# multimodallearning/DG-TTA

Hardware: AMD Instinct MI355X
Metric: TTA-epochs/sec per GPU on 128^3 patch; Dice delta vs reference (higher is better)
Workload: dtype fp16

## Files before the change

dg_tta_amd/_lib.py:

```python
import ctypes as C
import os
from pathlib import Path

LIB_PATH = Path(__file__).resolve().parent / "libdgtta_hip.so"

_c_float_p = C.POINTER(C.c_float)
P, I, I64, U64, F, SZ = C.c_void_p, C.c_int, C.c_int64, C.c_uint64, C.c_float, C.c_size_t

SIGNATURES = {
    "dgtta_version": (I, []),
    "dgtta_last_error": (C.c_char_p, []),
    "dgtta_reload_env": (I, []),
    "dgtta_mind3d_ws_bytes": (SZ, [I, I, I, I]),
    "dgtta_mind3d_fwd": (I, [P, P, F, I, C.POINTER(F), I, P, I, I, I, P, SZ, I, I, I, I, P]),
    "dgtta_mind3d_noise_fill": (I, [P, U64, U64, I, I, I, I, I, P]),
    "dgtta_mind3d_fwd_seeded": (I, [P, U64, U64, I, F, I, C.POINTER(F), I, P, I, I, I, P, SZ, I, I, I, I, P]),
    "dgtta_gin_ws_bytes": (SZ, [I, I, I, I]),
    "dgtta_gin_chain_fwd": (I, [P, P, C.POINTER(I), C.POINTER(P), C.POINTER(P), P, P, SZ, I, I, I, I, P]),
    "dgtta_affine_warp3d_fwd": (I, [P, P, P, I, I, I, I, I, I, I, I, I, I, I, I, I, I, P, P]),
    "dgtta_affine_warp3d_bwd": (I, [P, P, P, I, I, I, I, I, I, I, I, I, I, I, I, I, P]),
    "dgtta_rf_field_ws_bytes": (SZ, [I, I, I, I]),
    "dgtta_rf_field_fwd": (I, [P, P, P, SZ, I, I, I, I, I, I, I, I, P]),
    "dgtta_diffeo_fields_ws_bytes": (SZ, [I, I, I, I]),
    "dgtta_diffeo_fields": (I, [P, F, P, P, P, SZ, I, I, I, I, I, P]),
    "dgtta_dense_warp3d_fwd": (I, [P, P, P, I, I, I, I, I, I, I, I, I, P]),
    "dgtta_dense_warp3d_bwd": (I, [P, P, P, I, I, I, I, I, I, I, I, I, P]),
    "dgtta_softdice_ws_bytes": (SZ, [I, I, I64]),
    "dgtta_softdice_fwd": (I, [P, P, P, P, P, SZ, I, I, I64, I, I, I, P]),
    "dgtta_softdice_bwd": (I, [P, P, P, P, P, F, P, I, I, I64, I, I, P]),
    "dgtta_softdice_bwd_t": (I, [P, P, P, P, P, F, P, I, I, I64, I, I, I, P]),
    "dgtta_softdice_probs_fwd": (I, [P, P, P, P, SZ, I, I, I64, I64, I64, I64, P]),
    "dgtta_softdice_probs_bwd": (I, [P, P, P, P, P, P, I, I, I64, I64, I64, I64, P]),
    "dgtta_dice_ce_ws_bytes": (SZ, [I, I, I64]),
    "dgtta_dice_ce_fwd": (I, [P, I, P, P, P, P, SZ, I, I, I64, F, I, P]),
    "dgtta_dice_ce_bwd": (I, [P, I, P, P, F, P, P, I, I, I, I64, P]),
    "dgtta_dice_ce_ds_ws_bytes": (SZ, [I, I, I, I, I]),
    "dgtta_dice_ce_ds_fwd": (I, [P, I, P, P, P, P, SZ, I, I, I, I, I, I, I, I, F, I, P]),
    "dgtta_dice_ce_ds_bwd": (I, [P, I, P, P, F, P, P, I, I, I, I, I, I, I, I, I, P]),
    "dgtta_adamw_step": (I, [C.POINTER(P), C.POINTER(P), C.POINTER(P), C.POINTER(P), C.POINTER(I64), I, F, F, F, F, F,
                             I, F, P, P]),
    "dgtta_grads_nonfinite": (I, [C.POINTER(P), C.POINTER(I64), I, P, P]),
    "dgtta_grad_sumsq_ws_bytes": (SZ, [I64, I]),
    "dgtta_grad_sumsq": (I, [C.POINTER(P), C.POINTER(I64), I, P, P, SZ, P]),
    "dgtta_sgd_step": (I, [C.POINTER(P), C.POINTER(P), C.POINTER(P), C.POINTER(I64), I, F, F, F, I, I, F, P, F, P, P]),
    "dgtta_conv3d_packed_bytes": (SZ, [I, I, I]),
    "dgtta_conv3d_pack_weights": (I, [P, P, I, I, I, I, I, P]),
    "dgtta_conv3d_stats_bytes": (SZ, [I, I, I, I, I]),
    "dgtta_conv3d_k3_fwd": (I, [P, I, P, P, P, I, P, I, I, I, I, I, I, I, I, I, I, I, P]),
    "dgtta_conv3d_k3_dgrad": (I, [P, I, P, P, I, I, I, I, I, I, I, I, I, I, I, I, I, P]),
    "dgtta_conv3d_wgrad_ws_bytes": (SZ, [I, I, I, I, I, I]),
    "dgtta_conv3d_wgrad_split_ws_bytes": (SZ, [I, I, I, I, I, I, I]),
    "dgtta_conv3d_k3_wgrad": (I, [P, I, P, I, P, P, P, SZ, I, I, I, I, I, I, I, I, I, I, P]),
    "dgtta_conv3d_k3_blocked_supported": (I, [I, I, I, I, I, I, I]),
    "dgtta_conv3d_k3_fwd_blocked": (I, [P, I64, P, P, P, I, P, I, I, I, I, I, I, I, I, I, P]),
    "dgtta_conv3d_k3_wgrad_blocked": (I, [P, I64, P, I, P, P, P, SZ, I, I, I, I, I, I, I, I, P]),
    "dgtta_instnorm_ws_bytes": (SZ, [I, I, I64]),
    "dgtta_instnorm_lrelu_fwd": (I, [P, I, P, P, P, P, P, I, P, SZ, I, I, I64, F, F, I, P]),
    "dgtta_instnorm_lrelu_bwd": (I, [P, I, P, I, P, P, P, P, I, P, P, P, SZ, I, I, I64, F, I, I, P]),
    "dgtta_conv3d_k3_dgrad_gstats": (I, [P, I, P, P, I, I, I, I, I, I, I, I, I, P, I, P, P, P, F, P, SZ, C.POINTER(I), I, I, P]),
    "dgtta_instnorm_lrelu_bwd_gstats": (I, [P, I, P, I, P, P, P, P, I, P, P, P, P, SZ, I, I, I64, F, I, I, P]),
    "dgtta_convT3d_fwd_ws_bytes": (SZ, [I, I, I]),
    "dgtta_convT3d_k2s2_fwd": (I, [P, I, P, P, P, I, P, SZ, I, I, I, I, I, I, I, I, P]),
    "dgtta_convT3d_bwd_ws_bytes": (SZ, [I, I, I, I, I, I]),
    "dgtta_convT3d_bwd_split_ws_bytes": (SZ, [I, I, I, I, I, I]),
    "dgtta_convT3d_k2s2_bwd": (I, [P, I, P, I, P, P, I, P, P, P, SZ, I, I, I, I, I, I, I, I, I, P]),
    "dgtta_conv3d_kpacked_bytes": (SZ, [I, I, I, I]),
    "dgtta_conv3d_kpack_weights": (I, [P, P, I, I, I, I, I, I, I, I, P]),
    "dgtta_conv3d_fwd": (I, [P, I, P, P, P, I, P, I, I, I, I, I, I, I, I, I, I, I, I, I, P]),
    "dgtta_conv3d_dgrad": (I, [P, I, P, P, I, I, I, I, I, I, I, I, I, I, I, I, I, I, I, P]),
    "dgtta_conv3d_kwgrad_ws_bytes": (SZ, [I, I, I, I, I, I, I, I, I, I]),
    "dgtta_conv3d_wgrad": (I, [P, I, P, I, P, P, P, SZ, I, I, I, I, I, I, I, I, I, I, I, I, P]),
    "dgtta_convT3d_s_fwd_ws_bytes": (SZ, [I, I, I, I, I, I]),
    "dgtta_convT3d_s_fwd": (I, [P, I, P, P, P, I, P, SZ, I, I, I, I, I, I, I, I, I, I, P]),
    "dgtta_convT3d_s_bwd_ws_bytes": (SZ, [I, I, I, I, I, I, I, I, I]),
    "dgtta_convT3d_s_bwd": (I, [P, I, P, I, P, P, I, P, P, P, SZ, I, I, I, I, I, I, I, I, I, I, I, P]),
    "dgtta_seghead_fwd": (I, [P, I, P, P, P, I, P, I, I, I, I, I64, I, P]),
    "dgtta_seghead_bwd_ws_bytes": (SZ, [I, I, I, I64]),
    "dgtta_seghead_bwd": (I, [P, I, P, I, P, P, I, P, I, P, P, P, SZ, I, I, I64, I, I, P]),
    "dgtta_seghead_bwd_acc": (I, [P, I, P, I, P, P, I, P, I, P, P, P, SZ, I, I, I64, I, I, I, P]),
    "dgtta_seghead_warp_supported": (I, [P, I, I, I, I, I, I, I]),
    "dgtta_seghead_warp_bwd_ws_bytes": (SZ, [I, I, I, I, I, I]),
    "dgtta_seghead_warp_fwd": (I, [P, P, P, P, I, P, P, I, I, I, I, I, I, I, P]),
    "dgtta_seghead_warp_bwd": (I, [P, P, P, P, P, P, I, P, P, P, P, SZ, I, I, I, I, I, I, I, I, P]),
    "dgtta_seghead_warp_bwd_g16": (I, [P, P, P, P, P, P, I, P, P, P, P, SZ, I, I, I, I, I, I, I, I, P]),
    "dgtta_ncdhw_to_ndhwc": (I, [P, P, I, I, I64, I, I, P]),
    "dgtta_ndhwc_to_ncdhw": (I, [P, P, I, I, I64, I, I, P]),
    "dgtta_argmax_dice": (I, [P, I, I, P, P, P, I, I64, P]),
    "dgtta_resample_axis_ws_bytes": (SZ, [I64, I, I64, I]),
    "dgtta_resample_axis": (I, [P, P, P, SZ, I64, I, I, I64, I, P]),
    "dgtta_window_accumulate": (I, [P, P, P, P, I, I, I, I, I, I, I, I, I, I, P]),
    "dgtta_seghead_window_accumulate": (I, [P, P, P, P, P, P, I, I, I, I, I, I, I, I, I, I, I, I, P]),
    "dgtta_logits_chunk_f64": (I, [P, P, P, I, I, I, I, I, I, I, I, I, I, I, I, P]),
    "dgtta_window_accumulate_t": (I, [P, P, P, P, I, I, I, I, I, I, I, I, I, I, I, P]),
    "dgtta_seghead_window_accumulate_t": (I, [P, P, P, P, P, P, I, I, I, I, I, I, I, I, I, I, I, I, I, P]),
    "dgtta_argmax_rows": (I, [P, I, I, I64, P, P]),
    "dgtta_feature_window_accumulate": (I, [P, P, P, P, I, I, I, I, I, I, I, I, I, I, I, P]),
    "dgtta_feature_window_accumulate_norm": (I, [P, P, P, P, F, P, P, P, I, I, I, I, I, I, I, I, I, I, I, P]),
    "dgtta_feature_window_accumulate_multi": (I, [P, P, P, I, P, P, F, P, P, P, I, I, I, I, I, I, I, I, I, I, I, I, P]),
    "dgtta_feature_head_argmax": (I, [P, I64, P, P, P, I, I, I, I64, P, P]),
    "dgtta_feature_logits_chunk_f64": (I, [P, I64, P, P, P, P, I, I, I, I, I, I, I, I, I, I, I, I, I, I, P]),
    "dgtta_logits_chunk_f64_t": (I, [P, P, P, I, I, I, I, I, I, I, I, I, I, I, I, I, P]),
    "dgtta_argmax_merge_f64": (I, [P, I64, I, I, P, P, I, P]),
    "dgtta_feature_head_softmax": (I, [P, I64, P, P, P, I, I, I, I64, C.POINTER(I), I, I, P, P, P, P, P]),
    "dgtta_softmax_merge_f64": (I, [P, I64, I, I, C.c_double, P, P, P, C.POINTER(I), I, P, I, P]),
    "dgtta_softmax_finalize_f64": (I, [P, P, P, P, I64, I, I, P, P, P, P]),
    "dgtta_label_bboxes": (I, [P, P, I, I, I, I, P, P]),
    "dgtta_label_surface": (I, [P, I, I, I, I64, I, I, I, I, I, I, P, P]),
    "dgtta_edt_ws_bytes": (SZ, [I, I, I]),
    "dgtta_edt_sq": (I, [P, P, P, SZ, I, I, I, F, F, F, P]),
    "dgtta_cc_ws_bytes": (SZ, [I, I, I]),
    "dgtta_cc_label": (I, [P, P, I, I, I, I, I, P, P, SZ, P]),
    "dgtta_cc_sizes": (I, [P, I64, P, P]),
    "dgtta_cc_filter": (I, [P, P, I, P, P, I64, I, I, I64, P, P, P, SZ, P]),
    "dgtta_holes_ws_bytes": (SZ, [I, I, I]),
    "dgtta_holes_fill": (I, [P, I, I, I, I, P, P, P, P, SZ, P]),
    "dgtta_holes_member": (I, [P, I, I, I, P, I, I, I, I, I, I, I, P, P]),
    "dgtta_holes_apply": (I, [P, I, I, I, P, P, I, I, I, I, I, I, I64, I64, P, P]),
    "dgtta_nonzero_mask": (I, [P, I, I64, P, P]),
    "dgtta_bspline3_prefilter": (I, [P, P, I, I, I, P]),
    "dgtta_patch_sample_aug": (I, [P, I, I, I, I, I, P, P, P]),
    "dgtta_intensity_stats_ws_bytes": (SZ, [I, I64]),
    "dgtta_intensity_stats": (I, [P, I, I64, C.POINTER(I), I, P, P, SZ, P]),
    "dgtta_intensity_map": (I, [P, P, I, I64, P, I, P, P, P]),
    "dgtta_gauss_blur3": (I, [P, P, P, I, I, I, I, P, I, P]),
}



class PatchItem(C.Structure):
    _fields_ = [("image", P), ("label", P), ("D", I), ("H", I), ("W", I), ("map", F * 12)]


PATCH_MAX_ITEMS = 16


class IntensityItem(C.Structure):
    _fields_ = [("item", I), ("mode", I), ("negate", I), ("noise_b", I), ("a", F), ("s", F), ("seed_lo", C.c_uint32),
                ("seed_hi", C.c_uint32), ("off_lo", C.c_uint32), ("off_hi", C.c_uint32)]


class BlurItem(C.Structure):
    _fields_ = [("item", I), ("radius", I), ("taps", F * 9)]


INTENSITY_MAX_ITEMS = 16
IMAP_LINEAR, IMAP_CONTRAST, IMAP_GAMMA, IMAP_RESTORE = 0, 1, 2, 3

_lib = None
_load_error = None


class DgttaError(RuntimeError):
    pass


def load():
    global _lib, _load_error
    if _lib is not None:
        return _lib
    if _load_error is not None:
        raise DgttaError(_load_error)
    path = os.environ.get("DGTTA_LIB", str(LIB_PATH))
    import torch
    try:
        lib = C.CDLL(path)
    except OSError as e:
        _load_error = (f"libdgtta_hip.so could not be loaded from {path} ({e}). Build it with "
                       f"`python dg_tta_amd/build.py`; dg_tta_amd has no CPU fallback.")
        raise DgttaError(_load_error) from e
    for name, (res, args) in SIGNATURES.items():
        fn = getattr(lib, name)
        fn.restype = res
        fn.argtypes = args
    _lib = lib
    return lib


def check(rc, what):
    if rc != 0:
        msg = load().dgtta_last_error().decode(errors="replace")
        raise DgttaError(f"{what} failed (code {rc}): {msg}")


def ptr(t):
    return None if t is None else t.data_ptr()


def stream_of(device=None):
    import torch
    return torch.cuda.current_stream(device).cuda_stream


def require_cuda(*tensors):
    for t in tensors:
        if t is not None and not t.is_cuda:
            raise DgttaError("dg_tta_amd ops run on the MI355X only: got a CPU tensor (there is no CPU fallback)")
```

dg_tta_amd/csrc/common.h:

```cpp
#pragma once
#include <hip/hip_runtime.h>
#include <hip/hip_bf16.h>
#include <hip/hip_fp16.h>
#include <stdint.h>
#include <stdio.h>
#include <stdarg.h>

#include "../../include/dgtta.h"

#define WAVE 64

#include <atomic>

void dgtta_set_error(const char *fmt, ...);

struct DgttaSwitches {
  int conv_rows, conv_s2, dgrad_s2_allcls, wgrad_tr, wgrad_tr8, wgrad_s2_onepass, convt_wgrad_onepass;
  int convt_gemm, rows_order, in_nt, wgrad_upw, wgrad_xcd, in_gstats, softdice16, conv_ring, wgrad_ring, ha_mfma, wgrad_f32_split, feature_head_mfma, headwarp_mfma, wgrad_flat, wgrad_reduce_taps;
};
const DgttaSwitches &dgtta_switches();

struct DynLdsOnce {
  std::atomic<unsigned long long> mask{0};
};
static inline hipError_t ensure_dyn_lds(DynLdsOnce &o, const void *fn, int bytes) {
  int dev = 0;
  (void)hipGetDevice(&dev);
  const unsigned long long bit = 1ull << (dev & 63);
  if (o.mask.load(std::memory_order_acquire) & bit) return hipSuccess;
  const hipError_t e = hipFuncSetAttribute(fn, hipFuncAttributeMaxDynamicSharedMemorySize, bytes);
  if (e == hipSuccess) o.mask.fetch_or(bit, std::memory_order_release);
  return e;
}

struct RowsGstCtx {
  const void *y;
  long long ldy;
  const float *mr, *gamma, *beta;
  float slope;
  double *out;
  int produced;
};

#define DG_REQUIRE(cond, code, ...)      \
  do {                                   \
    if (!(cond)) {                       \
      dgtta_set_error(__VA_ARGS__);      \
      return (code);                     \
    }                                    \
  } while (0)

#define DG_CHECK_LAUNCH(name)                                                     \
  do {                                                                            \
    hipError_t e__ = hipGetLastError();                                           \
    if (e__ != hipSuccess) {                                                      \
      dgtta_set_error("%s: launch failed: %s", name, hipGetErrorString(e__));     \
      return DGTTA_ERR_LAUNCH;                                                    \
    }                                                                             \
  } while (0)

__host__ __device__ static inline int64_t cdiv64(int64_t a, int64_t b) { return (a + b - 1) / b; }
__host__ __device__ static inline int cdiv(int a, int b) { return (a + b - 1) / b; }
static inline size_t align_up(size_t x, size_t a) { return (x + a - 1) / a * a; }
static inline int grid_for(int64_t total) {
  const int64_t b = (total + 255) / 256;
  return (int)(b < 8192 ? b : 8192);
}

typedef unsigned short bf16_t;

__device__ __forceinline__ float bf16_to_f32(bf16_t h) { return __uint_as_float(((unsigned)h) << 16); }
__device__ __forceinline__ bf16_t f32_to_bf16(float f) {
  __hip_bfloat16 b = __float2bfloat16(f);
  return *reinterpret_cast<bf16_t *>(&b);
}

struct f16_t {
  unsigned short v;
};
__device__ __forceinline__ float f16_to_f32(unsigned short h) {
  return __half2float(__ushort_as_half(h));
}
__device__ __forceinline__ unsigned short f32_to_f16(float f) { return __half_as_ushort(__float2half_rn(f)); }

template <typename T>
__device__ __forceinline__ unsigned short f32_to_16(float f);
template <>
__device__ __forceinline__ unsigned short f32_to_16<bf16_t>(float f) { return f32_to_bf16(f); }
template <>
__device__ __forceinline__ unsigned short f32_to_16<f16_t>(float f) { return f32_to_f16(f); }
template <typename T>
__device__ __forceinline__ float from16(unsigned short h);
template <>
__device__ __forceinline__ float from16<bf16_t>(unsigned short h) { return bf16_to_f32(h); }
template <>
__device__ __forceinline__ float from16<f16_t>(unsigned short h) { return f16_to_f32(h); }
template <typename T>
__device__ __forceinline__ unsigned pack2_16(float lo, float hi) {
  return (unsigned)f32_to_16<T>(lo) | ((unsigned)f32_to_16<T>(hi) << 16);
}
template <typename T>
__device__ __forceinline__ void unpack2_16(unsigned w, float &lo, float &hi);
template <>
__device__ __forceinline__ void unpack2_16<bf16_t>(unsigned w, float &lo, float &hi) {
  lo = __uint_as_float(w << 16);
  hi = __uint_as_float(w & 0xffff0000u);
}
template <>
__device__ __forceinline__ void unpack2_16<f16_t>(unsigned w, float &lo, float &hi) {
  lo = f16_to_f32((unsigned short)(w & 0xffffu));
  hi = f16_to_f32((unsigned short)(w >> 16));
}

template <typename T>
__device__ __forceinline__ float ld_f(const T *p);
template <>
__device__ __forceinline__ float ld_f<float>(const float *p) { return *p; }
template <>
__device__ __forceinline__ float ld_f<bf16_t>(const bf16_t *p) { return bf16_to_f32(*p); }
template <>
__device__ __forceinline__ float ld_f<f16_t>(const f16_t *p) { return f16_to_f32(p->v); }

template <typename T>
__device__ __forceinline__ void st_f(T *p, float v);
template <>
__device__ __forceinline__ void st_f<float>(float *p, float v) { *p = v; }
template <>
__device__ __forceinline__ void st_f<bf16_t>(bf16_t *p, float v) { *p = f32_to_bf16(v); }
template <>
__device__ __forceinline__ void st_f<f16_t>(f16_t *p, float v) { p->v = f32_to_f16(v); }

template <typename T>
__device__ __forceinline__ void unpack16(const uint4 &v, float *f);
template <>
__device__ __forceinline__ void unpack16<float>(const uint4 &v, float *f) {
  f[0] = __uint_as_float(v.x);
  f[1] = __uint_as_float(v.y);
  f[2] = __uint_as_float(v.z);
  f[3] = __uint_as_float(v.w);
}
template <>
__device__ __forceinline__ void unpack16<bf16_t>(const uint4 &v, float *f) {
  const unsigned w[4] = {v.x, v.y, v.z, v.w};
#pragma unroll
  for (int i = 0; i < 4; ++i) {
    f[2 * i] = __uint_as_float(w[i] << 16);
    f[2 * i + 1] = __uint_as_float(w[i] & 0xffff0000u);
  }
}
template <>
__device__ __forceinline__ void unpack16<f16_t>(const uint4 &v, float *f) {
  const unsigned w[4] = {v.x, v.y, v.z, v.w};
#pragma unroll
  for (int i = 0; i < 4; ++i) unpack2_16<f16_t>(w[i], f[2 * i], f[2 * i + 1]);
}

template <typename T>
__device__ __forceinline__ uint4 pack16(const float *f);
template <>
__device__ __forceinline__ uint4 pack16<float>(const float *f) {
  return make_uint4(__float_as_uint(f[0]), __float_as_uint(f[1]), __float_as_uint(f[2]), __float_as_uint(f[3]));
}
template <>
__device__ __forceinline__ uint4 pack16<bf16_t>(const float *f) {
  unsigned w[4];
#pragma unroll
  for (int i = 0; i < 4; ++i) w[i] = (unsigned)f32_to_bf16(f[2 * i]) | ((unsigned)f32_to_bf16(f[2 * i + 1]) << 16);
  return make_uint4(w[0], w[1], w[2], w[3]);
}
template <>
__device__ __forceinline__ uint4 pack16<f16_t>(const float *f) {
  return make_uint4(pack2_16<f16_t>(f[0], f[1]), pack2_16<f16_t>(f[2], f[3]), pack2_16<f16_t>(f[4], f[5]),
                    pack2_16<f16_t>(f[6], f[7]));
}

__device__ __forceinline__ float wave_sum(float v) {
#pragma unroll
  for (int o = 32; o > 0; o >>= 1) v += __shfl_xor(v, o, 64);
  return v;
}
__device__ __forceinline__ double wave_sum_d(double v) {
#pragma unroll
  for (int o = 32; o > 0; o >>= 1) v += __shfl_xor(v, o, 64);
  return v;
}
__device__ __forceinline__ float wave_min(float v) {
#pragma unroll
  for (int o = 32; o > 0; o >>= 1) v = fminf(v, __shfl_xor(v, o, 64));
  return v;
}

__device__ __forceinline__ float block_sum(float v, float *red) {
  v = wave_sum(v);
  const int lane = threadIdx.x & 63, w = threadIdx.x >> 6, nw = (blockDim.x + 63) >> 6;
  __syncthreads();
  if (lane == 0) red[w] = v;
  __syncthreads();
  float r = 0.f;
  for (int i = 0; i < nw; ++i) r += red[i];
  return r;
}

__device__ __forceinline__ float lrelu(float a, float slope) { return a > 0.f ? a : a * slope; }
```

dg_tta_amd/csrc/conv_dispatch.hip:

```cpp
#include "conv_api.h"

static int wgrad_splits(int64_t nvox) {
  int64_t s = cdiv64(nvox, 4096);
  return (int)(s < 64 ? (s > 0 ? s : 1) : 64);
}

static const void *wb_of(const void *wpack, int CinP, int CoutP, int dtype) {
  return (const char *)wpack + (size_t)27 * CinP * CoutP * esize(dtype);
}

static const void *img_of(const void *wpack, int CinP, int CoutP, int dtype) {
  return (const char *)wpack + (size_t)2 * 27 * CinP * CoutP * esize(dtype);
}
static const void *imgB_of(const void *wpack, int CinP, int CoutP, int dtype) {
  return (const char *)img_of(wpack, CinP, CoutP, dtype) + conv_imgB_offset_bytes(CinP, CoutP, dtype);
}

extern "C" size_t dgtta_conv3d_packed_bytes(int CinP, int CoutP, int dtype) {
  if (CinP <= 0 || CoutP <= 0) return 0;
  return (size_t)2 * 27 * CinP * CoutP * esize(dtype) + conv_image_bytes(CinP, CoutP, dtype);
}

extern "C" int dgtta_conv3d_pack_weights(const float *w_t, void *wpack, int Cin, int Cout, int CinP, int CoutP,
                                         int dtype, void *stream) {
  DG_REQUIRE(w_t && wpack, DGTTA_ERR_BADARG, "pack_weights: null pointer");
  void *wf = wpack;
  void *wb = const_cast<void *>(wb_of(wpack, CinP, CoutP, dtype));
  DG_REQUIRE(Cin > 0 && Cout > 0 && CinP >= Cin && CoutP >= Cout, DGTTA_ERR_BADARG, "pack_weights: bad channel counts");
  const int rc = conv3_pack_weights_ref(w_t, wf, wb, Cin, Cout, CinP, CoutP, dtype, (hipStream_t)stream);
  if (rc != DGTTA_OK) return rc;
  if (CinP % conv_granule(dtype) == 0 && CoutP % conv_granule(dtype) == 0)
    return conv_pack_images(w_t, const_cast<void *>(img_of(wpack, CinP, CoutP, dtype)), 27, Cin, Cout, CinP, CoutP, dtype,
                            (hipStream_t)stream);
  return DGTTA_OK;
}

extern "C" size_t dgtta_conv3d_stats_bytes(int B, int Cout, int Do, int Ho, int Wo) {
  if (B <= 0 || Cout <= 0 || Do <= 0 || Ho <= 0 || Wo <= 0) return 0;
  int64_t nb = conv3_mfma_max_tiles(Do, Ho, Wo);
  const int64_t rb = reduce_blocks((int64_t)Do * Ho * Wo, B);
  if (rb > nb) nb = rb;
  return 256 + (size_t)B * nb * Cout * 2 * sizeof(double);
}

static int k3_fwd(const void *x, int ldx, long long x_block_stride, const void *wpack, const float *bias, void *y, int ldy,
                  void *stats, int B, int Cin, int Cout, int CinP, int CoutP, int Di, int Hi, int Wi, int stride, int dtype, int impl,
                  void *stream) {
  DG_REQUIRE(x && wpack && y, DGTTA_ERR_BADARG, "conv3d_k3_fwd: null pointer");
  const void *wf = wpack;
  DG_REQUIRE(B > 0 && Cin > 0 && Cout > 0 && CinP >= Cin && CoutP >= Cout && Di > 0 && Hi > 0 && Wi > 0,
             DGTTA_ERR_BADARG, "conv3d_k3_fwd: bad dims");
  DG_REQUIRE(stride == 1 || stride == 2, DGTTA_ERR_UNSUPPORTED, "conv3d_k3_fwd: stride %d", stride);
  DG_REQUIRE((x_block_stride ? 2 * ldx : ldx) >= Cin && ldy >= Cout, DGTTA_ERR_BADARG, "conv3d_k3_fwd: ld < C");
  hipStream_t st = (hipStream_t)stream;
  if (impl != 1) {
    int rc = conv3_fwd_mfma(x, ldx, img_of(wpack, CinP, CoutP, dtype), 0, bias, y, ldy, B, Cin, Cout, CinP, CoutP, Di, Hi,
                            Wi, stride, dtype, st, (double *)stats, nullptr, x_block_stride, false);
    if (rc != DGTTA_ERR_UNSUPPORTED) return rc;
    DG_REQUIRE(x_block_stride == 0, DGTTA_ERR_UNSUPPORTED,
               "conv3d_k3_fwd_blocked: only the D-ring kernel reads x as 32-channel planes (ask dgtta_conv3d_k3_blocked_supported)");
    DG_REQUIRE(impl == 0, DGTTA_ERR_UNSUPPORTED, "conv3d_k3_fwd: shape not covered by the MFMA kernel");
  }
  int rc = conv3_fwd_ref(x, ldx, wf, bias, y, ldy, B, Cin, Cout, CinP, CoutP, Di, Hi, Wi, stride, dtype, st);
  if (rc != DGTTA_OK) return rc;
  if (stats) {
    const int64_t V = (int64_t)out_dim(Di, stride) * out_dim(Hi, stride) * out_dim(Wi, stride);
    return conv_stats_ref(y, ldy, stats, B, Cout, V, dtype, st);
  }
  return DGTTA_OK;
}

extern "C" int dgtta_conv3d_k3_fwd(const void *x, int ldx, const void *wpack, const float *bias, void *y, int ldy,
                                   void *stats, int B, int Cin, int Cout, int CinP, int CoutP, int Di, int Hi, int Wi,
                                   int stride, int dtype, int impl, void *stream) {
  return k3_fwd(x, ldx, 0, wpack, bias, y, ldy, stats, B, Cin, Cout, CinP, CoutP, Di, Hi, Wi, stride, dtype, impl, stream);
}

extern "C" int dgtta_conv3d_k3_blocked_supported(int B, int Cin, int Cout, int D, int H, int W, int dtype) {
  if (B <= 0 || Cin != 64 || Cout <= 0 || Cout % 32 || D <= 0 || H <= 0 || W <= 0) return 0;
  if (dtype != DGTTA_BF16 && dtype != DGTTA_F16) return 0;
  const int rc = conv3_fwd_mfma((const void *)16, 32, (const void *)16, 0, nullptr, (void *)16, Cout, B, Cin, Cout, Cin, Cout, D, H, W, 1,
                                dtype, nullptr, nullptr, nullptr, (long long)B * D * H * W * 32, true);
  return rc == DGTTA_OK && conv3_wgrad_blocked_ok(B, Cin, Cout, D, H, W, dtype);
}

extern "C" int dgtta_conv3d_k3_fwd_blocked(const void *x, long long x_block_stride, const void *wpack, const float *bias, void *y,
                                           int ldy, void *stats, int B, int Cin, int Cout, int CinP, int CoutP, int Di, int Hi,
                                           int Wi, int dtype, void *stream) {
  DG_REQUIRE(x_block_stride > 0 && x_block_stride % 8 == 0, DGTTA_ERR_BADARG, "conv3d_k3_fwd_blocked: block stride must be a positive multiple of 8 elements");
  return k3_fwd(x, 32, x_block_stride, wpack, bias, y, ldy, stats, B, Cin, Cout, CinP, CoutP, Di, Hi, Wi, 1, dtype, 0, stream);
}

static int k3_dgrad(const void *dy, int lddy, const void *wpack, void *dx, int lddx, int B, int Cin, int Cout, int CinP, int CoutP,
                    int Di, int Hi, int Wi, int stride, int accumulate, int dtype, int impl, void *stream, RowsGstCtx *gst) {
  DG_REQUIRE(dy && wpack && dx, DGTTA_ERR_BADARG, "conv3d_k3_dgrad: null pointer");
  const void *wb = wb_of(wpack, CinP, CoutP, dtype);
  DG_REQUIRE(B > 0 && Cin > 0 && Cout > 0 && CinP >= Cin && CoutP >= Cout && Di > 0 && Hi > 0 && Wi > 0,
             DGTTA_ERR_BADARG, "conv3d_k3_dgrad: bad dims");
  DG_REQUIRE(stride == 1 || stride == 2, DGTTA_ERR_UNSUPPORTED, "conv3d_k3_dgrad: stride %d", stride);
  DG_REQUIRE(lddx >= Cin && lddy >= Cout, DGTTA_ERR_BADARG, "conv3d_k3_dgrad: ld < C");
  hipStream_t st = (hipStream_t)stream;
  if (impl != 1 && stride == 1 && !accumulate) {
    int rc = conv3_fwd_mfma(dy, lddy, imgB_of(wpack, CinP, CoutP, dtype), 1, nullptr, dx, lddx, B, Cout, Cin, CoutP, CinP, Di,
                            Hi, Wi, 1, dtype, st, nullptr, gst, 0, false);
    if (rc != DGTTA_ERR_UNSUPPORTED) return rc;
    DG_REQUIRE(impl == 0, DGTTA_ERR_UNSUPPORTED, "conv3d_k3_dgrad: shape not covered by the MFMA kernel");
  }
  if (impl != 1 && stride == 2 && !((Di | Hi | Wi) & 1)) {
    int rc = conv3_dgrad_s2_mfma(dy, lddy, imgB_of(wpack, CinP, CoutP, dtype), dx, lddx, B, Cin, Cout, CinP, CoutP, Di, Hi, Wi,
                                 accumulate, dtype, st);
    if (rc != DGTTA_ERR_UNSUPPORTED) return rc;
    DG_REQUIRE(impl == 0, DGTTA_ERR_UNSUPPORTED, "conv3d_k3_dgrad: shape not covered by the MFMA kernel");
  }
  return conv3_dgrad_ref(dy, lddy, wb, dx, lddx, B, Cin, Cout, CinP, CoutP, Di, Hi, Wi, stride, accumulate, dtype, st);
}

extern "C" int dgtta_conv3d_k3_dgrad(const void *dy, int lddy, const void *wpack, void *dx, int lddx, int B, int Cin,
                                     int Cout, int CinP, int CoutP, int Di, int Hi, int Wi, int stride, int accumulate,
                                     int dtype, int impl, void *stream) {
  return k3_dgrad(dy, lddy, wpack, dx, lddx, B, Cin, Cout, CinP, CoutP, Di, Hi, Wi, stride, accumulate, dtype, impl, stream, nullptr);
}

extern "C" int dgtta_conv3d_k3_dgrad_gstats(const void *dy, int lddy, const void *wpack, void *dx, int lddx, int B, int Cin,
                                            int Cout, int CinP, int CoutP, int Di, int Hi, int Wi, const void *y_prev,
                                            int ldy_prev, const float *mean_rstd_prev, const float *gamma_prev,
                                            const float *beta_prev, float slope, void *gstats, size_t gstats_bytes,
                                            int *h_produced, int dtype, int impl, void *stream) {
  DG_REQUIRE(y_prev && mean_rstd_prev && gamma_prev && beta_prev && gstats && h_produced, DGTTA_ERR_BADARG,
             "conv3d_k3_dgrad_gstats: null pointer");
  DG_REQUIRE(ldy_prev >= Cin, DGTTA_ERR_BADARG, "conv3d_k3_dgrad_gstats: ldy_prev < Cin");
  DG_REQUIRE(B > 0 && Cin > 0 && Di > 0 && Hi > 0 && Wi > 0 && gstats_bytes >= dgtta_conv3d_stats_bytes(B, Cin, Di, Hi, Wi),
             DGTTA_ERR_WORKSPACE, "conv3d_k3_dgrad_gstats: statistics buffer too small");
  RowsGstCtx ctx{y_prev, ldy_prev, mean_rstd_prev, gamma_prev, beta_prev, slope, (double *)gstats, 0};
  const bool fuse = dtype != DGTTA_F32 && impl != 1 && dgtta_switches().in_gstats != '0';
  const int rc = k3_dgrad(dy, lddy, wpack, dx, lddx, B, Cin, Cout, CinP, CoutP, Di, Hi, Wi, 1, 0, dtype, impl, stream,
                          fuse ? &ctx : nullptr);
  *h_produced = rc == DGTTA_OK ? ctx.produced : 0;
  return rc;
}

static size_t wgrad_bias_bytes(int B, int Cout, int Do, int Ho, int Wo) {
  return align_up((size_t)B * reduce_blocks((int64_t)Do * Ho * Wo, B) * Cout * 2 * sizeof(double), 256);
}

extern "C" size_t dgtta_conv3d_wgrad_ws_bytes(int B, int Cin, int Cout, int Do, int Ho, int Wo) {
  if (B <= 0 || Cin <= 0 || Cout <= 0 || Do <= 0 || Ho <= 0 || Wo <= 0) return 0;
  const int64_t nvox = (int64_t)B * Do * Ho * Wo;
  size_t a = align_up((size_t)wgrad_splits(nvox) * Cout * Cin * 27 * sizeof(float), 256);
  size_t c = align_up(conv3_wgrad_mfma_ws_bytes(B, Cin, Cout, Do, Ho, Wo), 256);
  return wgrad_bias_bytes(B, Cout, Do, Ho, Wo) + (a > c ? a : c);
}

extern "C" size_t dgtta_conv3d_wgrad_split_ws_bytes(int B, int Cin, int Cout, int Do, int Ho, int Wo, int stride) {
  if (B <= 0 || Cin <= 0 || Cout <= 0 || Do <= 0 || Ho <= 0 || Wo <= 0 || (stride != 1 && stride != 2)) return 0;
  const size_t base = dgtta_conv3d_wgrad_ws_bytes(B, Cin, Cout, Do, Ho, Wo);
  return base + 256 + conv3_wgrad_split_extra_bytes(B, Cin, Cout, Do, Ho, Wo, stride);
}

static int k3_wgrad(const void *x, int ldx, long long x_block_stride, const void *dy, int lddy, float *dw_t, float *db, void *ws,
                    size_t ws_bytes, int B, int Cin, int Cout, int Di, int Hi, int Wi, int stride, int accumulate, int dtype, int impl,
                    void *stream) {
  DG_REQUIRE(x && dy && dw_t && ws, DGTTA_ERR_BADARG, "conv3d_k3_wgrad: null pointer");
  DG_REQUIRE(B > 0 && Cin > 0 && Cout > 0 && Di > 0 && Hi > 0 && Wi > 0, DGTTA_ERR_BADARG, "conv3d_k3_wgrad: bad dims");
  DG_REQUIRE(stride == 1 || stride == 2, DGTTA_ERR_UNSUPPORTED, "conv3d_k3_wgrad: stride %d", stride);
  const int Do = out_dim(Di, stride), Ho = out_dim(Hi, stride), Wo = out_dim(Wi, stride);
  DG_REQUIRE(ws_bytes >= dgtta_conv3d_wgrad_ws_bytes(B, Cin, Cout, Do, Ho, Wo), DGTTA_ERR_WORKSPACE,
             "conv3d_k3_wgrad: workspace too small");
  hipStream_t st = (hipStream_t)stream;
  const int64_t nvox = (int64_t)B * Do * Ho * Wo;
  const int nsplit = wgrad_splits(nvox);
  const size_t bias_bytes = wgrad_bias_bytes(B, Cout, Do, Ho, Wo);
  void *ws2 = ws;
  float *part = (float *)((char *)ws + bias_bytes);
  bool done = false;
  if (impl != 1) {
    int rc = conv3_wgrad_mfma(x, ldx, dy, lddy, dw_t, part, ws_bytes - bias_bytes, B, Cin, Cout, Di, Hi, Wi,
                              stride, accumulate, dtype, st, x_block_stride);
    if (rc == DGTTA_OK) done = true;
    else if (rc != DGTTA_ERR_UNSUPPORTED) return rc;
    else DG_REQUIRE(impl == 0 && x_block_stride == 0, DGTTA_ERR_UNSUPPORTED,
                    "conv3d_k3_wgrad: shape not covered by the MFMA kernel (x as 32-channel planes: only the ring sweep, ask dgtta_conv3d_k3_blocked_supported)");
  }
  if (!done) {
    const int rc = conv3_wgrad_ref(x, ldx, dy, lddy, part, nsplit, dw_t, B, Cin, Cout, Di, Hi, Wi, stride, accumulate, dtype, st);
    if (rc != DGTTA_OK) return rc;
  }
  if (db) return conv_bias_grad(dy, lddy, db, ws2, B, Cout, (int64_t)Do * Ho * Wo, accumulate, dtype, st);
  return DGTTA_OK;
}

extern "C" int dgtta_conv3d_k3_wgrad(const void *x, int ldx, const void *dy, int lddy, float *dw_t, float *db, void *ws,
                                     size_t ws_bytes, int B, int Cin, int Cout, int Di, int Hi, int Wi, int stride,
                                     int accumulate, int dtype, int impl, void *stream) {
  return k3_wgrad(x, ldx, 0, dy, lddy, dw_t, db, ws, ws_bytes, B, Cin, Cout, Di, Hi, Wi, stride, accumulate, dtype, impl, stream);
}

extern "C" int dgtta_conv3d_k3_wgrad_blocked(const void *x, long long x_block_stride, const void *dy, int lddy, float *dw_t, float *db,
                                             void *ws, size_t ws_bytes, int B, int Cin, int Cout, int Di, int Hi, int Wi,
                                             int accumulate, int dtype, void *stream) {
  DG_REQUIRE(x_block_stride > 0 && x_block_stride % 8 == 0, DGTTA_ERR_BADARG, "conv3d_k3_wgrad_blocked: block stride must be a positive multiple of 8 elements");
  return k3_wgrad(x, 32, x_block_stride, dy, lddy, dw_t, db, ws, ws_bytes, B, Cin, Cout, Di, Hi, Wi, 1, accumulate, dtype, 0, stream);
}

extern "C" size_t dgtta_convT3d_fwd_ws_bytes(int Cin, int Cout, int dtype) {
  if (Cin <= 0 || Cout <= 0) return 0;
  return convT_pack_region(Cin, Cout, dtype);
}

extern "C" int dgtta_convT3d_k2s2_fwd(const void *x, int ldx, const float *w_t, const float *bias, void *out, int ldo,
                                      void *ws, size_t ws_bytes, int B, int Cin, int Cout, int Di, int Hi, int Wi,
                                      int dtype, int impl, void *stream) {
  DG_REQUIRE(x && w_t && out, DGTTA_ERR_BADARG, "convT3d_k2s2_fwd: null pointer");
  DG_REQUIRE(B > 0 && Cin > 0 && Cout > 0 && Di > 0 && Hi > 0 && Wi > 0 && ldx >= Cin && ldo >= Cout, DGTTA_ERR_BADARG,
             "convT3d_k2s2_fwd: bad dims");
  hipStream_t st = (hipStream_t)stream;
  if (impl != 1 && ws && ws_bytes >= convT_pack_region(Cin, Cout, dtype)) {
    int rc = convT_fwd_mfma(x, ldx, w_t, bias, out, ldo, ws, B, Cin, Cout, Di, Hi, Wi, dtype, st);
    if (rc != DGTTA_ERR_UNSUPPORTED) return rc;
  }
  DG_REQUIRE(impl != 2, DGTTA_ERR_UNSUPPORTED, "convT3d_k2s2_fwd: shape not covered by the MFMA kernel");
  return convT_fwd_ref(x, ldx, w_t, bias, out, ldo, B, Cin, Cout, Di, Hi, Wi, dtype, st);
}

static size_t convT_bias_region(int B, int Cout, int Di, int Hi, int Wi) {
  return align_up((size_t)B * reduce_blocks((int64_t)Di * Hi * Wi * 8, B) * Cout * 2 * sizeof(double), 256);
}

extern "C" size_t dgtta_convT3d_bwd_ws_bytes(int B, int Cin, int Cout, int Di, int Hi, int Wi) {
  if (B <= 0 || Cin <= 0 || Cout <= 0 || Di <= 0 || Hi <= 0 || Wi <= 0) return 0;
  const int64_t nvox = (int64_t)B * Di * Hi * Wi;
  size_t a = align_up((size_t)wgrad_splits(nvox) * Cin * Cout * 8 * sizeof(float), 256);
  size_t c = align_up(conv3_wgrad_mfma_ws_bytes(B, Cin, Cout, Di, Hi, Wi), 256);
  return convT_bias_region(B, Cout, Di, Hi, Wi) + convT_pack_region(Cin, Cout, DGTTA_F32) + (a > c ? a : c);
}

extern "C" size_t dgtta_convT3d_bwd_split_ws_bytes(int B, int Cin, int Cout, int Di, int Hi, int Wi) {
  if (B <= 0 || Cin <= 0 || Cout <= 0 || Di <= 0 || Hi <= 0 || Wi <= 0) return 0;
  const int64_t nvox = (int64_t)B * Di * Hi * Wi;
  size_t a = align_up((size_t)wgrad_splits(nvox) * Cin * Cout * 8 * sizeof(float), 256);
  size_t c = align_up(conv3_wgrad_mfma_ws_bytes(B, Cin, Cout, Di, Hi, Wi), 256) + convT_wgrad_split_extra_bytes(B, Cin, Cout, Di, Hi, Wi);
  return convT_bias_region(B, Cout, Di, Hi, Wi) + convT_pack_region(Cin, Cout, DGTTA_F32) + (a > c ? a : c);
}

extern "C" int dgtta_convT3d_k2s2_bwd(const void *x, int ldx, const void *dout, int lddo, const float *w_t, void *dx,
                                      int lddx, float *dw_t, float *db, void *ws, size_t ws_bytes, int B, int Cin,
                                      int Cout, int Di, int Hi, int Wi, int accumulate, int dtype, int impl,
                                      void *stream) {
  DG_REQUIRE(x && dout && w_t && ws, DGTTA_ERR_BADARG, "convT3d_k2s2_bwd: null pointer");
  DG_REQUIRE(B > 0 && Cin > 0 && Cout > 0 && Di > 0 && Hi > 0 && Wi > 0 && ldx >= Cin && lddo >= Cout,
             DGTTA_ERR_BADARG, "convT3d_k2s2_bwd: bad dims");
  DG_REQUIRE(ws_bytes >= dgtta_convT3d_bwd_ws_bytes(B, Cin, Cout, Di, Hi, Wi), DGTTA_ERR_WORKSPACE,
             "convT3d_k2s2_bwd: workspace too small");
  hipStream_t st = (hipStream_t)stream;
  const int64_t nvox = (int64_t)B * Di * Hi * Wi;
  void *ws_bias = ws;
  void *ws_pack = (char *)ws + convT_bias_region(B, Cout, Di, Hi, Wi);
  void *ws_main = (char *)ws_pack + convT_pack_region(Cin, Cout, DGTTA_F32);
  const size_t main_bytes = ws_bytes - ((char *)ws_main - (char *)ws);
  int bias_units = 0;
  if (dx) {
    DG_REQUIRE(lddx >= Cin, DGTTA_ERR_BADARG, "convT3d_k2s2_bwd: lddx < Cin");
    int rc = DGTTA_ERR_UNSUPPORTED;
    if (impl != 1) rc = convT_dgrad_mfma(dout, lddo, w_t, dx, lddx, ws_pack, B, Cin, Cout, Di, Hi, Wi, dtype, st);
    if (rc == DGTTA_ERR_UNSUPPORTED) {
      DG_REQUIRE(impl != 2, DGTTA_ERR_UNSUPPORTED, "convT3d_k2s2_bwd: dgrad shape not covered by the MFMA kernel");
      rc = convT_dgrad_ref(dout, lddo, w_t, dx, lddx, B, Cin, Cout, Di, Hi, Wi, dtype, st);
      if (rc != DGTTA_OK) return rc;
    } else if (rc != DGTTA_OK) {
      return rc;
    }
  }
  if (dw_t) {
    int rc = DGTTA_ERR_UNSUPPORTED;
    if (impl != 1)
      rc = convT_wgrad_mfma(x, ldx, dout, lddo, dw_t, ws_main, main_bytes, B, Cin, Cout, Di, Hi, Wi, accumulate, dtype, st,
                            db ? (float *)ws_bias : nullptr, convT_bias_region(B, Cout, Di, Hi, Wi), &bias_units);
    if (rc == DGTTA_ERR_UNSUPPORTED) {
      DG_REQUIRE(impl != 2, DGTTA_ERR_UNSUPPORTED, "convT3d_k2s2_bwd: wgrad shape not covered by the MFMA kernel");
      rc = convT_wgrad_ref(x, ldx, dout, lddo, (float *)ws_main, wgrad_splits(nvox), dw_t, B, Cin, Cout, Di, Hi, Wi, accumulate,
                           dtype, st);
      if (rc != DGTTA_OK) return rc;
    } else if (rc != DGTTA_OK) {
      return rc;
    }
  }
  if (db && bias_units > 0) {
    DG_REQUIRE(convT_bias_finalize((const float *)ws_bias, bias_units, Cout, db, accumulate, st) == DGTTA_OK, DGTTA_ERR_LAUNCH,
               "convT3d_k2s2_bwd: bias finalize launch failed");
    return DGTTA_OK;
  }
  if (db) return conv_bias_grad(dout, lddo, db, ws_bias, B, Cout, (int64_t)Di * Hi * Wi * 8, accumulate, dtype, st);
  return DGTTA_OK;
}
```

dg_tta_amd/csrc/conv_mfma.hip:

```cpp
#include "conv_common.h"
#include <stdlib.h>
#include <type_traits>

namespace {

template <typename T, int MBW, int MBH, int MBD, int S, int NB, int KSPC, int NW = 4, bool AC = false>
__global__ __launch_bounds__(NW * 64) void conv3_mfma_kernel(const T *__restrict__ x, View xv, const T *__restrict__ w,
                                                         ConvClasses cs, const float *__restrict__ bias,
                                                         T *__restrict__ y, View yv, int Cin, int Cout, int CinP,
                                                         int CoutP, int tilesW, int tilesH, int tilesD,
                                                         double *__restrict__ stats, int ntaps_src) {
  const int cls = blockIdx.z;
  x += cs.xoff[cls];
  if (!AC) y += cs.yoff[cls];
  const Taps &taps = cs.taps[cls];
  const int accumulate = cs.acc[cls];
  const int Di = xv.D, Hi = xv.H, Wi = xv.W, Do = yv.D, Ho = yv.H, Wo = yv.W;
  typedef ConvCfg<T, MBW, MBH, MBD, S, NB, KSPC> Cfg;
  typedef typename Cfg::G G;
  constexpr int EPV = Cfg::EPV, NG = Cfg::NG, CK = Cfg::CK, NC = Cfg::NC, NV = G::NV, MPW = G::MB / NW, NT = NW * 64;
  extern __shared__ __attribute__((aligned(16))) unsigned char smem[];
  uint4 *sA = reinterpret_cast<uint4 *>(smem);
  uint4 *sB = reinterpret_cast<uint4 *>(smem + Cfg::A_BYTES);

  const int tid = threadIdx.x, lane = tid & 63, wave = tid >> 6;
  const int r = lane & 31, h = lane >> 5;

  int tlin = blockIdx.x;
  if ((gridDim.x & 7) == 0) tlin = (tlin & 7) * (int)(gridDim.x >> 3) + (tlin >> 3);
  int t = tlin;
  const int tw = t % tilesW;
  t /= tilesW;
  const int th = t % tilesH;
  t /= tilesH;
  const int td = t % tilesD;
  const int b = t / tilesD;
  const int n0 = blockIdx.y * NC;
  constexpr int SE = G::SE, NTAP = G::NTAP;
  const int od0 = td * G::TD, oh0 = th * G::TH, ow0 = tw * G::TW;
  const int id0 = od0 * SE - G::HALO, ih0 = oh0 * SE - G::HALO, iw0 = ow0 * SE - G::HALO;

  int a_off[MPW];
#pragma unroll
  for (int i = 0; i < MPW; ++i) {
    const int mb = wave * MPW + i;
    const int mbd = mb / MBH, mbh = mb % MBH;
    const int row = mbh * G::RPM + r / MBW, col = r % MBW;
    a_off[i] = ((mbd * SE) * G::IH + row * SE) * G::ROW + col;
  }

  constexpr int NACC = AC ? 8 : NB;
  f32x16_t acc[MPW][NACC];
#pragma unroll
  for (int i = 0; i < MPW; ++i)
#pragma unroll
    for (int j = 0; j < NACC; ++j)
#pragma unroll
      for (int q = 0; q < 16; ++q) acc[i][j][q] = 0.f;

  const T *xbp = x + (int64_t)b * xv.sb;
  const int cin_lim = (Cin + EPV - 1) / EPV * EPV;

  constexpr int NA = (NV * NG + NT - 1) / NT, NBL = (NTAP * NC * NG + NT - 1) / NT;
  uint4 ra[NA], rb[NBL];
  __shared__ signed char s_wt[32];
  if (tid < 27) s_wt[tid] = AC ? (signed char)tid : taps.wt[tid];
  __syncthreads();
  int wslot[NBL];
#pragma unroll
  for (int i = 0; i < NBL; ++i) {
    const int idx = tid + i * NT;
    const int n = idx % NC, g = (idx / NC) % NG, tap = (S == 0) ? 13 : (idx / (NG * NC)) % 27;
    const int wt = s_wt[tap];
    const bool ok = idx < NTAP * NC * NG && wt >= 0;
    const int off = ((((n0 + n) / 32) * (CinP / (2 * EPV)) + g / 2) * ntaps_src + wt) * 64 + (g & 1) * 32 + (n0 + n) % 32;
    wslot[i] = ok ? off : -1;
  }
  auto load_chunk = [&](int kc) {
#pragma unroll
    for (int i = 0; i < NA; ++i) {
      const int idx = tid + i * NT;
      const int g = idx % NG, v = idx / NG;
      const int wx_l = v % G::ROW, hy = (v / G::ROW) % G::IH, dz = v / (G::ROW * G::IH);
      int wx = wx_l;
      if (S == 2) wx = (wx_l >= G::IWH) ? 2 * (wx_l - G::IWH) + 1 : 2 * wx_l;
      const int gd = id0 + dz, gh = ih0 + hy, gw = iw0 + wx;
      int c = kc + g * EPV;
      long long soff = 0;
      if (S == 0 && cs.kseg > 0) {
        const int seg = c / cs.kseg;
        c -= seg * cs.kseg;
        soff = cs.segoff[seg];
      }
      const bool ok = idx < NV * NG && (S != 2 || wx < G::IW) && (unsigned)gd < (unsigned)Di &&
                      (unsigned)gh < (unsigned)Hi && (unsigned)gw < (unsigned)Wi && c < cin_lim;
      const T *p = ok ? xbp + soff + gd * xv.sd + gh * xv.sh + gw * xv.sw + c : x;
      const uint4 val = *reinterpret_cast<const uint4 *>(p);
      ra[i] = ok ? val : make_uint4(0, 0, 0, 0);
    }
    const int kterm = (kc / (2 * EPV)) * ntaps_src * 64;
#pragma unroll
    for (int i = 0; i < NBL; ++i) {
      const bool ok = wslot[i] >= 0;
      const T *p = w + (int64_t)(ok ? wslot[i] + kterm : 0) * EPV;
      const uint4 val = *reinterpret_cast<const uint4 *>(p);
      rb[i] = ok ? val : make_uint4(0, 0, 0, 0);
    }
  };
  auto store_chunk = [&]() {
#pragma unroll
    for (int i = 0; i < NA; ++i) {
      const int idx = tid + i * NT;
      if (idx < NV * NG) sA[(idx % NG) * NV + idx / NG] = ra[i];
    }
#pragma unroll
    for (int i = 0; i < NBL; ++i) {
      const int idx = tid + i * NT;
      if (idx < NTAP * NC * NG) sB[idx] = rb[i];
    }
  };

  load_chunk(0);
  for (int kc = 0; kc < CinP; kc += CK) {
    __syncthreads();
    store_chunk();
    __syncthreads();
    if (kc + CK < CinP) load_chunk(kc + CK);
    if (AC) {
#pragma unroll
      for (int ks = 0; ks < KSPC; ++ks) {
        const int g = 2 * ks + h;
#pragma unroll
        for (int sh8 = 0; sh8 < 8; ++sh8) {
          const int sd = sh8 >> 2, shh = (sh8 >> 1) & 1, sw = sh8 & 1;
          const int tap_off = ((1 + sd) * G::IH + (1 + shh)) * G::ROW + G::lds_col(1 + sw);
          uint4 af[MPW];
#pragma unroll
          for (int i = 0; i < MPW; ++i) af[i] = sA[g * NV + a_off[i] + tap_off];
#pragma unroll
          for (int od = 0; od < 2 - sd; ++od)
#pragma unroll
            for (int oh = 0; oh < 2 - shh; ++oh)
#pragma unroll
              for (int ow = 0; ow < 2 - sw; ++ow) {
                const int pd = sd ? 1 : od, ph = shh ? 1 : oh, pw = sw ? 1 : ow;
                const int td = sd ? 0 : 1 + od, th = shh ? 0 : 1 + oh, tw = sw ? 0 : 1 + ow;
                const int tap = td * 9 + th * 3 + tw, c8 = pd * 4 + ph * 2 + pw;
                const uint4 bfr = sB[(tap * NG + g) * NC + r];
#pragma unroll
                for (int i = 0; i < MPW; ++i) mfma_step<T>(af[i], bfr, acc[i][c8]);
              }
        }
      }
    } else
#pragma unroll
    for (int tap = (S == 0 ? 13 : 0); tap < (S == 0 ? 14 : 27); ++tap) {
      if (taps.wt[tap] < 0) continue;
      const int kd = tap / 9, kh = (tap / 3) % 3, kw = tap % 3;
      const int tap_off = (S == 0) ? 0 : (kd * G::IH + kh) * G::ROW + G::lds_col(kw);
      const int tb = (S == 0) ? 0 : tap;
#pragma unroll
      for (int ks = 0; ks < KSPC; ++ks) {
        const int g = 2 * ks + h;
        uint4 bf[NB];
#pragma unroll
        for (int j = 0; j < NB; ++j) bf[j] = uint4(sB[(tb * NG + g) * NC + j * 32 + r]);
#pragma unroll
        for (int i = 0; i < MPW; ++i) {
          const uint4 af = sA[g * NV + a_off[i] + tap_off];
#pragma unroll
          for (int j = 0; j < NB; ++j) mfma_step<T>(af, bf[j], acc[i][j]);
        }
      }
    }
  }

  float st1[NB], st2[NB];
#pragma unroll
  for (int j = 0; j < NB; ++j) st1[j] = st2[j] = 0.f;
  if (AC) {
    const bool vec = Cout % 8 == 0 && (reinterpret_cast<uintptr_t>(y) & 15) == 0 && yv.sw % 8 == 0 && yv.sh % 8 == 0 &&
                     yv.sd % 8 == 0 && yv.sb % 8 == 0;
    __syncthreads();
    float *slab = reinterpret_cast<float *>(smem) + wave * (32 * 36);
#pragma unroll
    for (int i = 0; i < MPW; ++i) {
      const int mb = wave * MPW + i;
      const int mbd = mb / MBH, mbh = mb % MBH;
      const int co = n0 + r;
      uint4 olds[8][2];
      if constexpr (sizeof(T) == 2) {
        if (vec && accumulate) {
#pragma unroll
          for (int c8 = 0; c8 < 8; ++c8)
#pragma unroll
            for (int t = 0; t < 2; ++t) {
              const int m = t * 16 + (lane >> 2), cq = (lane & 3) * 8;
              const int od = od0 + mbd, oh = oh0 + mbh * G::RPM + m / MBW, ow = ow0 + m % MBW;
              olds[c8][t] = make_uint4(0u, 0u, 0u, 0u);
              if (n0 + cq < Cout && od < Do && oh < Ho && ow < Wo)
                olds[c8][t] = *reinterpret_cast<const uint4 *>(y + cs.yoff[c8] + b * yv.sb + od * yv.sd + oh * yv.sh + ow * yv.sw + n0 + cq);
            }
        }
      }
#pragma unroll
      for (int c8 = 0; c8 < 8; ++c8) {
        if (!vec) {
#pragma unroll
          for (int q = 0; q < 16; ++q) {
            const int m = (q & 3) + 8 * (q >> 2) + 4 * h;
            const int od = od0 + mbd, oh = oh0 + mbh * G::RPM + m / MBW, ow = ow0 + m % MBW;
            if (co < Cout && od < Do && oh < Ho && ow < Wo) {
              T *o = y + cs.yoff[c8] + b * yv.sb + od * yv.sd + oh * yv.sh + ow * yv.sw + co;
              float v = acc[i][c8][q];
              if (accumulate) v += ld_f<T>(o);
              st_f<T>(o, v);
            }
          }
          continue;
        }
#pragma unroll
        for (int q = 0; q < 16; ++q) slab[((q & 3) + 8 * (q >> 2) + 4 * h) * 36 + r] = acc[i][c8][q];
#pragma unroll
        for (int t = 0; t < 2; ++t) {
          const int m = t * 16 + (lane >> 2), cq = (lane & 3) * 8;
          const float4 v0 = *reinterpret_cast<const float4 *>(slab + m * 36 + cq);
          const float4 v1 = *reinterpret_cast<const float4 *>(slab + m * 36 + cq + 4);
          float v[8] = {v0.x, v0.y, v0.z, v0.w, v1.x, v1.y, v1.z, v1.w};
          const int od = od0 + mbd, oh = oh0 + mbh * G::RPM + m / MBW, ow = ow0 + m % MBW;
          if (n0 + cq < Cout && od < Do && oh < Ho && ow < Wo) {
            T *o = y + cs.yoff[c8] + b * yv.sb + od * yv.sd + oh * yv.sh + ow * yv.sw + n0 + cq;
            if constexpr (sizeof(T) == 2) {
              uint4 *o4 = reinterpret_cast<uint4 *>(o);
              if (accumulate) {
                const uint4 old = olds[c8][t];
                const unsigned wv[4] = {old.x, old.y, old.z, old.w};
#pragma unroll
                for (int e = 0; e < 4; ++e) {
                  float lo, hi;
                  unpack2_16<T>(wv[e], lo, hi);
                  v[2 * e] += lo;
                  v[2 * e + 1] += hi;
                }
              }
              uint4 pk;
              pk.x = pack2_16<T>(v[0], v[1]);
              pk.y = pack2_16<T>(v[2], v[3]);
              pk.z = pack2_16<T>(v[4], v[5]);
              pk.w = pack2_16<T>(v[6], v[7]);
              *o4 = pk;
            } else {
              float4 *o4 = reinterpret_cast<float4 *>(o);
              if (accumulate) {
                const float4 a0 = o4[0], a1 = o4[1];
                v[0] += a0.x; v[1] += a0.y; v[2] += a0.z; v[3] += a0.w;
                v[4] += a1.x; v[5] += a1.y; v[6] += a1.z; v[7] += a1.w;
              }
              o4[0] = make_float4(v[0], v[1], v[2], v[3]);
              o4[1] = make_float4(v[4], v[5], v[6], v[7]);
            }
          }
        }
      }
    }
    return;
  }
#pragma unroll
  for (int i = 0; i < MPW; ++i) {
    const int mb = wave * MPW + i;
    const int mbd = mb / MBH, mbh = mb % MBH;
#pragma unroll
    for (int j = 0; j < NB; ++j) {
      const int co = n0 + j * 32 + r;
      const float bv = (bias && co < Cout) ? bias[co] : 0.f;
#pragma unroll
      for (int q = 0; q < 16; ++q) {
        const int m = (q & 3) + 8 * (q >> 2) + 4 * h;
        const int od = od0 + mbd, oh = oh0 + mbh * G::RPM + m / MBW, ow = ow0 + m % MBW;
        if (co < Cout && od < Do && oh < Ho && ow < Wo) {
          T *o = y + b * yv.sb + od * yv.sd + oh * yv.sh + ow * yv.sw + co;
          float v = acc[i][j][q] + bv;
          if (accumulate) v += ld_f<T>(o);
          st_f<T>(o, v);
          st1[j] += v;
          st2[j] += v * v;
        }
      }
    }
  }
  if (stats) {
    __syncthreads();
    float *red = reinterpret_cast<float *>(smem);
#pragma unroll
    for (int j = 0; j < NB; ++j) {
      const float a = st1[j] + __shfl_xor(st1[j], 32, 64), c = st2[j] + __shfl_xor(st2[j], 32, 64);
      if (h == 0) {
        red[(wave * NC + j * 32 + r) * 2 + 0] = a;
        red[(wave * NC + j * 32 + r) * 2 + 1] = c;
      }
    }
    __syncthreads();
    const int tiles_per_b = tilesW * tilesH * tilesD;
    if (tid < NC && n0 + tid < Cout) {
      double s = 0.0, ss = 0.0;
#pragma unroll
      for (int wv = 0; wv < NW; ++wv) {
        s += (double)red[(wv * NC + tid) * 2 + 0];
        ss += (double)red[(wv * NC + tid) * 2 + 1];
      }
      double *p = stats + 32 + (((int64_t)b * tiles_per_b + (tlin % tiles_per_b)) * Cout + n0 + tid) * 2;
      p[0] = s;
      p[1] = ss;
    }
    if (blockIdx.x == 0 && blockIdx.y == 0 && tid == 0) reinterpret_cast<long long *>(stats)[0] = tiles_per_b;
  }
}

template <typename T, int MBW, int MBH, int MBD, int S, int NB, int KSPC, int NW = 4, bool AC = false>
int launch_conv(const ConvLaunch &L, const ConvClasses &cs) {
  typedef ConvCfg<T, MBW, MBH, MBD, S, NB, KSPC> Cfg;
  typedef typename Cfg::G G;
  auto kern = conv3_mfma_kernel<T, MBW, MBH, MBD, S, NB, KSPC, NW, AC>;
  static DynLdsOnce lds_once;
  DG_REQUIRE(ensure_dyn_lds(lds_once, reinterpret_cast<const void *>(kern), (int)Cfg::LDS_BYTES) == hipSuccess,
             DGTTA_ERR_LAUNCH, "conv3_mfma: cannot raise the dynamic LDS limit to %zu", (size_t)Cfg::LDS_BYTES);
  const int tW = cdiv(L.yv.W, G::TW), tH = cdiv(L.yv.H, G::TH), tD = cdiv(L.yv.D, G::TD);
  const int64_t tiles = (int64_t)tW * tH * tD * L.B;
  DG_REQUIRE(tiles < (1ll << 31), DGTTA_ERR_UNSUPPORTED, "conv3_mfma: too many tiles");
  dim3 grid((unsigned)tiles, (unsigned)cdiv(L.CoutP, Cfg::NC), AC ? 1u : (unsigned)cs.n);
  hipLaunchKernelGGL(kern, grid, dim3(NW * 64), Cfg::LDS_BYTES, L.st, (const T *)L.x, L.xv, (const T *)L.w, cs, L.bias, (T *)L.y,
                     L.yv, L.Cin, L.Cout, L.CinP, L.CoutP, tW, tH, tD, L.stats, L.ntaps_src);
  DG_CHECK_LAUNCH(AC ? "conv3_mfma_kernel<all classes>" : "conv3_mfma_kernel");
  return DGTTA_OK;
}

template <typename T>
int dispatch_conv_classes(const ConvLaunch &L, const ConvClasses &cs, int stride) {
  const View &yv = L.yv;
  const bool ring_only = L.xkh || L.dry;
  const long long vox = (long long)yv.D * yv.H * yv.W * L.B;
  if (ring_only && stride != 1) return DGTTA_ERR_UNSUPPORTED;
  if (stride == 0) {
    if (yv.W >= 32) return launch_conv<T, 32, 4, 4, 0, 1, 1, 8>(L, cs);
    if (yv.W >= 16) return launch_conv<T, 16, 4, 4, 0, 1, 1, 8>(L, cs);
    if (vox <= 4096) return launch_conv<T, 8, 2, 2, 0, 1, 1>(L, cs);
    return launch_conv<T, 8, 2, 8, 0, 1, 1, 8>(L, cs);
  }
  if (stride == 1 && sizeof(T) == 2 && yv.W >= 32 && cs.n == 1 && cs.acc[0] == 0 && cs.kseg == 0 && cs.xoff[0] == 0 &&
      cs.yoff[0] == 0) {
    const int rows = dgtta_switches().conv_rows;
    const int is_f16 = (int)std::is_same<T, f16_t>::value;
    bool all_taps = true;
    for (int t = 0; t < 27; ++t) all_taps = all_taps && cs.taps[0].wt[t] >= 0;
    const bool vec_out = L.Cout % 8 == 0 && ((uintptr_t)L.y & 15) == 0 && yv.sw % 8 == 0 && yv.sh % 8 == 0 &&
                         yv.sd % 8 == 0 && yv.sb % 8 == 0;
    const long long njobs = (long long)cdiv(yv.W, 32) * cdiv(yv.H, 8) * cdiv(yv.D, 4) * cdiv(L.CoutP, 32) * L.B;
    if (all_taps && vec_out && ((L.Cin == 32 && L.CinP == 32) || (L.Cin == 64 && L.CinP == 64)) &&
        (njobs >= 512 || dgtta_switches().conv_ring == '1') && dgtta_switches().conv_ring != '0' && rows != '1') {
      const int rc = conv3_ring_launch(L, cs.taps[0], conv3_mfma_max_tiles(yv.D, yv.H, yv.W), is_f16);
      if (rc != DGTTA_ERR_UNSUPPORTED || ring_only) return rc;
    }
    if (ring_only) return DGTTA_ERR_UNSUPPORTED;
    if (all_taps && vec_out && (njobs >= 256 || rows == '1') && rows != '0') return conv3_rows_launch(L, cs.taps[0], is_f16);
  }
  if (ring_only) return DGTTA_ERR_UNSUPPORTED;
  if (stride == 1) {
    if (yv.W >= 32) return launch_conv<T, 32, 4, 4, 1, 1, 1, 8>(L, cs);
    const bool k2 = L.CinP % (4 * Elem<T>::EPV) == 0;
    if (yv.W >= 16) return launch_conv<T, 16, 4, 4, 1, 1, 1, 8>(L, cs);
    if (vox <= 4096 && k2) return launch_conv<T, 8, 2, 2, 1, 1, 2>(L, cs);
    if (vox <= 4096) return launch_conv<T, 8, 2, 2, 1, 1, 1>(L, cs);
    return launch_conv<T, 8, 2, 8, 1, 1, 1, 8>(L, cs);
  }
  if (stride == 2) {
    if (dgtta_switches().conv_s2 == '4') {
      if (yv.W >= 16) return launch_conv<T, 16, 2, 4, 2, 1, 1>(L, cs);
      return launch_conv<T, 8, 2, 4, 2, 1, 1>(L, cs);
    }
    if (dgtta_switches().conv_s2 != '1' && yv.W >= 32 && L.CoutP % 64 == 0) return launch_conv<T, 32, 4, 2, 2, 2, 1, 8>(L, cs);
    if (yv.W >= 32) return launch_conv<T, 32, 4, 2, 2, 1, 1, 8>(L, cs);
    if (yv.W >= 16) return launch_conv<T, 16, 2, 4, 2, 1, 1, 8>(L, cs);
    return launch_conv<T, 8, 2, 4, 2, 1, 1, 8>(L, cs);
  }
  return DGTTA_ERR_UNSUPPORTED;
}

template <typename T>
int dispatch_conv(const ConvLaunch &L, const Taps &taps, int stride, int accumulate) {
  return dispatch_conv_classes<T>(L, single_class(taps, accumulate), stride);
}

template <typename T>
int dgrad_s2_allcls(const ConvLaunch &L, const ConvClasses &cs) {
  if (L.yv.W >= 32) return launch_conv<T, 32, 4, 2, 1, 1, 1, 8, true>(L, cs);
  if (L.yv.W >= 16) return launch_conv<T, 16, 2, 4, 1, 1, 1, 8, true>(L, cs);
  return launch_conv<T, 8, 2, 4, 1, 1, 1, 8, true>(L, cs);
}

template <typename T>
__global__ void conva_pack_kernel(const float *__restrict__ w, T *__restrict__ imgF, T *__restrict__ imgB, int Cin, int Cout,
                                  int CinP, int CoutP, int ntaps) {
  constexpr int EPV = Elem<T>::EPV;
  const int CoutN = (CoutP + 31) / 32 * 32, CinN = (CinP + 31) / 32 * 32;
  const int64_t nf = (int64_t)ntaps * CinP * CoutN, nb = (int64_t)ntaps * CoutP * CinN;
  for (int64_t i = (int64_t)blockIdx.x * blockDim.x + threadIdx.x; i < (nf > nb ? nf : nb); i += (int64_t)gridDim.x * blockDim.x) {
    if (i < nf) {
      const int ci = (int)(i % CinP), co = (int)((i / CinP) % CoutN), tap = (int)(i / ((int64_t)CinP * CoutN));
      st_f<T>(imgF + conv_weight_image_index(co, ci, tap, CinP, ntaps, EPV),
              (ci < Cin && co < Cout) ? w[((int64_t)co * Cin + ci) * ntaps + tap] : 0.f);
    }
    if (i < nb) {
      const int co = (int)(i % CoutP), ci = (int)((i / CoutP) % CinN), tap = (int)(i / ((int64_t)CoutP * CinN));
      st_f<T>(imgB + conv_weight_image_index(ci, co, tap, CoutP, ntaps, EPV),
              (ci < Cin && co < Cout) ? w[((int64_t)co * Cin + ci) * ntaps + tap] : 0.f);
    }
  }
}

}

int64_t conv3_mfma_max_tiles(int Do, int Ho, int Wo) {
  const int shapes[6][3] = {{4, 4, 32}, {4, 8, 16}, {2, 8, 8}, {8, 8, 8}, {4, 4, 16}, {4, 8, 8}};
  int64_t best = 0;
  for (auto &t : shapes) {
    int64_t n = (int64_t)cdiv(Do, t[0]) * cdiv(Ho, t[1]) * cdiv(Wo, t[2]);
    best = n > best ? n : best;
  }
  return best;
}

int conv3_fwd_mfma(const void *x, int ldx, const void *w_kmajor, int mirror, const float *bias, void *y, int ldy, int B,
                   int Cin, int Cout, int CinP, int CoutP, int Di, int Hi, int Wi, int stride, int dtype,
                   hipStream_t st, double *stats, RowsGstCtx *gst, long long xkh, bool dry) {
  if ((xkh || dry) && (stride != 1 || dtype == DGTTA_F32)) return DGTTA_ERR_UNSUPPORTED;
  const int Do = (Di - 1) / stride + 1, Ho = (Hi - 1) / stride + 1, Wo = (Wi - 1) / stride + 1;
  const ConvLaunch L{x, dense_view(B, Di, Hi, Wi, ldx), w_kmajor, bias, y, dense_view(B, Do, Ho, Wo, ldy), B, Cin, Cout, CinP, CoutP,
                     stats, 27, st, gst, xkh, dry};
  if (stride == 2 && !mirror && dtype != DGTTA_F32 && dgtta_switches().conv_s2 != '1' && dgtta_switches().conv_s2 != '4') {
    const int rc = conv3_s2_regs(L, conv3_mfma_max_tiles(Do, Ho, Wo), dtype);
    if (rc != DGTTA_ERR_UNSUPPORTED) return rc;
  }
  if (!dtype_ok(dtype) || !operand_ok(epv_of(dtype), x, xkh ? 2 * ldx : ldx, Cin, CinP)) return DGTTA_ERR_UNSUPPORTED;
  DISPATCH_T(dtype, return dispatch_conv<T>(L, identity_taps(mirror), stride, 0));
}

int conv3_dgrad_s2_mfma(const void *dy, int lddy, const void *w_kmajor, void *dx, int lddx, int B, int Cin, int Cout,
                        int CinP, int CoutP, int Di, int Hi, int Wi, int accumulate, int dtype, hipStream_t st) {
  if (!dtype_ok(dtype) || !operand_ok(epv_of(dtype), dy, lddy, Cout, CoutP)) return DGTTA_ERR_UNSUPPORTED;
  const int Do = (Di - 1) / 2 + 1, Ho = (Hi - 1) / 2 + 1, Wo = (Wi - 1) / 2 + 1;
  View yv;
  const ConvClasses cs = dgrad_parity_classes(3, 2, 2, 2, Di, Hi, Wi, lddx, accumulate, &yv);
  const ConvLaunch L{dy, dense_view(B, Do, Ho, Wo, lddy), w_kmajor, nullptr, dx, yv, B, Cout, Cin, CoutP, CinP, nullptr, 27, st};
  const bool allcls = dgtta_switches().dgrad_s2_allcls != '0' && CinP % 8 == 0;
  DISPATCH_T(dtype, return allcls ? dgrad_s2_allcls<T>(L, cs) : dispatch_conv_classes<T>(L, cs, 1));
}

size_t convT_packed_bytes(int CinP, int CoutP, int dtype) {
  return (size_t)8 * (CinP * n32(CoutP) + CoutP * n32(CinP)) * esize(dtype);
}
size_t conv_image_bytes(int CinP, int CoutP, int dtype) {
  return (size_t)27 * (CinP * n32(CoutP) + CoutP * n32(CinP)) * esize(dtype);
}
size_t conv_imgB_offset_bytes(int CinP, int CoutP, int dtype) {
  return (size_t)27 * CinP * n32(CoutP) * esize(dtype);
}
int conv_pack_images(const float *w_t, void *img, int ntaps, int Cin, int Cout, int CinP, int CoutP, int dtype, hipStream_t st) {
  const int cmax = CinP > CoutP ? CinP : CoutP;
  const int64_t n = (int64_t)ntaps * cmax * n32(cmax);
  const unsigned blocks = (unsigned)((n + 255) / 256 < 2048 ? (n + 255) / 256 : 2048);
  void *imgB = (char *)img + (size_t)ntaps * CinP * n32(CoutP) * esize(dtype);
  DISPATCH_T(dtype, hipLaunchKernelGGL((conva_pack_kernel<T>), dim3(blocks), dim3(256), 0, st, w_t, (T *)img, (T *)imgB, Cin, Cout,
                                       CinP, CoutP, ntaps));
  DG_CHECK_LAUNCH("conva_pack_kernel");
  return DGTTA_OK;
}

namespace {
template <typename T>
__global__ void convTa_pack_kernel(const float *__restrict__ w, T *__restrict__ wf, T *__restrict__ wb, int Cin, int Cout, int CinP,
                                   int CoutP, int no) {
  constexpr int EPV = Elem<T>::EPV;
  const int CoutN = (CoutP + 31) / 32 * 32, CinN = (CinP + 31) / 32 * 32;
  const int64_t nf = (int64_t)no * CinP * CoutN, nb = (int64_t)no * CoutP * CinN;
  for (int64_t i = (int64_t)blockIdx.x * blockDim.x + threadIdx.x; i < (nf > nb ? nf : nb); i += (int64_t)gridDim.x * blockDim.x) {
    if (i < nf) {
      int ci = (int)(i % CinP), co = (int)((i / CinP) % CoutN), o = (int)(i / ((int64_t)CinP * CoutN));
      st_f<T>(wf + conv_weight_image_index(co, ci, o, CinP, no, EPV), (ci < Cin && co < Cout) ? w[((int64_t)ci * Cout + co) * no + o] : 0.f);
    }
    if (i < nb) {
      int co = (int)(i % CoutP), ci = (int)((i / CoutP) % CinN), o = (int)(i / ((int64_t)CoutP * CinN));
      st_f<T>(wb + conv_weight_image_index(ci, o * CoutP + co, 0, no * CoutP, 1, EPV),
              (ci < Cin && co < Cout) ? w[((int64_t)ci * Cout + co) * no + o] : 0.f);
    }
  }
}

template <typename T>
int convTa_run_t(int mode, const void *in, int ldin, const float *w_t, const float *bias, void *out, int ldout, void *ws, int B, int Cin,
                 int Cout, int Di, int Hi, int Wi, int sd, int sh, int sw, hipStream_t st) {
  constexpr int EPV = Elem<T>::EPV;
  const int CinP = (Cin + 2 * EPV - 1) / (2 * EPV) * (2 * EPV), CoutP = (Cout + 2 * EPV - 1) / (2 * EPV) * (2 * EPV);
  const int no = sd * sh * sw;
  if (mode == 0 ? !operand_ok(EPV, in, ldin, Cin, CinP) : !operand_ok(EPV, in, ldin, Cout, CoutP)) return DGTTA_ERR_UNSUPPORTED;
  T *wf = (T *)ws, *wb = wf + (size_t)no * CinP * n32(CoutP);
  const int64_t n = (int64_t)no * (CinP > CoutP ? CinP : CoutP) * n32(CinP > CoutP ? CinP : CoutP);
  hipLaunchKernelGGL((convTa_pack_kernel<T>), dim3((unsigned)((n + 255) / 256 < 1024 ? (n + 255) / 256 : 1024)), dim3(256), 0, st,
                     w_t, wf, wb, Cin, Cout, CinP, CoutP, no);
  DG_CHECK_LAUNCH("convTa_pack_kernel");
  const int Do = sd * Di, Ho = sh * Hi, Wo = sw * Wi;
  Taps taps;
  for (int t = 0; t < 27; ++t) taps.wt[t] = -1;
  taps.wt[13] = 0;
  if (mode == 0) {
    ConvClasses cs{};
    cs.n = no;
    View yv{};
    for (int o = 0; o < no; ++o) {
      yv = lattice_view(Do, Ho, Wo, ldout, sd, sh, sw, sd == 2 ? (o / (sh * sw)) % 2 : 0, sh == 2 ? (o / sw) % 2 : 0,
                        sw == 2 ? o % 2 : 0, &cs.yoff[o]);
      cs.taps[o] = taps;
      cs.taps[o].wt[13] = (signed char)o;
    }
    const ConvLaunch L{in, dense_view(B, Di, Hi, Wi, ldin), wf, bias, out, yv, B, Cin, Cout, CinP, CoutP, nullptr, no, st};
    return dispatch_conv_classes<T>(L, cs, 0);
  }
  ConvClasses cs = single_class(taps, 0);
  cs.kseg = CoutP;
  View xv{};
  for (int o = 0; o < no; ++o)
    xv = lattice_view(Do, Ho, Wo, ldin, sd, sh, sw, sd == 2 ? (o / (sh * sw)) % 2 : 0, sh == 2 ? (o / sw) % 2 : 0, sw == 2 ? o % 2 : 0,
                      &cs.segoff[o]);
  const ConvLaunch L{in, xv, wb, nullptr, out, dense_view(B, Di, Hi, Wi, ldout), B, Cout, Cin, no * CoutP, CinP, nullptr, 1, st};
  return dispatch_conv_classes<T>(L, cs, 0);
}
}

int convTa_run(int mode, const void *in, int ldin, const float *w_t, const float *bias, void *out, int ldout, void *ws, int B, int Cin,
               int Cout, int Di, int Hi, int Wi, int sd, int sh, int sw, int dtype, hipStream_t st) {
  if (!dtype_ok(dtype)) return DGTTA_ERR_UNSUPPORTED;
  DISPATCH_T(dtype, return convTa_run_t<T>(mode, in, ldin, w_t, bias, out, ldout, ws, B, Cin, Cout, Di, Hi, Wi, sd, sh, sw, st));
}

int convT_fwd_mfma(const void *x, int ldx, const float *w_t, const float *bias, void *out, int ldo, void *ws, int B, int Cin,
                   int Cout, int Di, int Hi, int Wi, int dtype, hipStream_t st) {
  if (ldx >= Cin && ldo >= Cout && convT_gemm_eligible(0, x, ldx, out, ldo, Cin, Cout, Wi, dtype))
    return convT_gemm_run(0, x, ldx, w_t, bias, out, ldo, ws, B, Cin, Cout, Di, Hi, Wi, dtype, st);
  return convTa_run(0, x, ldx, w_t, bias, out, ldo, ws, B, Cin, Cout, Di, Hi, Wi, 2, 2, 2, dtype, st);
}
int convT_dgrad_mfma(const void *dout, int lddo, const float *w_t, void *dx, int lddx, void *ws, int B, int Cin, int Cout,
                     int Di, int Hi, int Wi, int dtype, hipStream_t st) {
  if (lddo >= Cout && lddx >= Cin && convT_gemm_eligible(1, dout, lddo, dx, lddx, Cin, Cout, Wi, dtype))
    return convT_gemm_run(1, dout, lddo, w_t, nullptr, dx, lddx, ws, B, Cin, Cout, Di, Hi, Wi, dtype, st);
  return convTa_run(1, dout, lddo, w_t, nullptr, dx, lddx, ws, B, Cin, Cout, Di, Hi, Wi, 2, 2, 2, dtype, st);
}
```

dg_tta_amd/csrc/conv_ring.hip:

```cpp
#include "conv_common.h"
#include <stdlib.h>
#include <type_traits>

namespace {

template <int KH>
struct RingCfgT {
  static constexpr int TH = 8 / KH, TW = 32;
  static constexpr int IH = TH + 2, IW = TW + 2;
  static constexpr int VB = 64;
  static constexpr int ROWB = IW * VB;
  static constexpr int SUB_PIECES = (IH * ROWB + 1023) / 1024;
  static constexpr int SUB = SUB_PIECES * 1024;
  static constexpr int PIECES = KH * SUB_PIECES, PLANE = PIECES * 1024;
  static constexpr int NVOX = IH * IW;
  static constexpr int NSLOT = 6;
  static constexpr int NW = 8 / KH, NT = NW * 64;
  static constexpr int NPW = (2 * PIECES + NW - 1) / NW;
  static constexpr int RED_BYTES = NW * 16 * 2 * (int)sizeof(float) + 32 * 2 * (int)sizeof(float);
  static constexpr int LDS_BYTES = NSLOT * PLANE + RED_BYTES;
};
typedef RingCfgT<1> RingCfg;
static_assert(RingCfgT<2>::LDS_BYTES <= 160 * 1024 && RingCfgT<1>::LDS_BYTES <= 160 * 1024, "ring does not fit the LDS");

template <int NM, int NR>
__device__ __forceinline__ void ring_sched_interleave() {
  if constexpr (NM > 0) {
    __builtin_amdgcn_sched_group_barrier(0x008, 1, 0);
    constexpr int r = NR > 0 ? 1 : 0;
    if constexpr (r > 0) __builtin_amdgcn_sched_group_barrier(0x100, 1, 0);
    ring_sched_interleave<NM - 1, NR - r>();
  }
}

template <typename T16>
__device__ __forceinline__ unsigned pack2_pk(float lo, float hi);
template <>
__device__ __forceinline__ unsigned pack2_pk<f16_t>(float lo, float hi) {
  return __builtin_bit_cast(unsigned, __builtin_convertvector(f32x2_t{lo, hi}, f16x2_t));
}
template <>
__device__ __forceinline__ unsigned pack2_pk<bf16_t>(float lo, float hi) {
  return __builtin_bit_cast(unsigned, __builtin_convertvector(f32x2_t{lo, hi}, bf16x2_t));
}

__device__ __forceinline__ void store16_buf(u32x4_t rsrc, unsigned voff, unsigned soff, u32x4_t val) {
  asm volatile("buffer_store_dwordx4 %0, %1, %2, %3 offen" ::"v"(val), "v"(voff), "s"(rsrc), "s"(soff) : "memory");
}

__device__ __forceinline__ void ring_wait_all_but(int n) { vm_wait_all_but<40>(min(n, 40)); }

struct RingGst {
  const bf16_t *y;
  View v;
  const float *mr, *gamma, *beta;
  float slope;
  unsigned bytes;
};

template <typename T16, bool GST = false, int KH = 1>
__global__ __launch_bounds__(RingCfgT<KH>::NT) void conv3_ring_kernel(const bf16_t *__restrict__ x, View xv, const bf16_t *__restrict__ w,
                                                                 Taps taps, const float *__restrict__ bias, bf16_t *__restrict__ y,
                                                                 View yv, int Cout, int tilesW, int tilesH, int nblkN, int nseg,
                                                                 int steps_per_seg, int njobs, double *__restrict__ stats,
                                                                 int ntaps_src, unsigned x_bytes, unsigned y_bytes, RingGst gst,
                                                                 long long xkh) {
  typedef RingCfgT<KH> C;
  extern __shared__ __attribute__((aligned(16))) unsigned char smem[];
  float *red = reinterpret_cast<float *>(smem + C::NSLOT * C::PLANE);
  float *gcst = red + C::NW * 16 * 2;
  const unsigned lds0 = lds_addr_of(smem);

  const int tid = threadIdx.x, lane = tid & 63, wave = __builtin_amdgcn_readfirstlane(tid >> 6);
  const int v = lane & 15, q = lane >> 4;
  const int chalf = wave & 1, ws = wave >> 1;
  const int D = xv.D, H = xv.H, W = xv.W;
  const int steps_total = (D + 1) / 2;

  int aoff[3];
#pragma unroll
  for (int kw = 0; kw < 3; ++kw) {
    const int u = v + kw;
    aoff[kw] = (2 * ws) * C::ROWB + u * C::VB + ((q ^ (((u >> 2) & 1) << 1)) << 4);
  }

  uint4 wreg[KH][27];
  int nb_loaded = -1;
  const int G = gridDim.x;
  const bool xcd_order = (G % 8) == 0;
  const int rounds = (njobs + G - 1) / G;
  for (int rd = 0; rd < rounds; ++rd) {
    int j = xcd_order ? (rd * 8 + (int)(blockIdx.x % 8)) * (G / 8) + (int)(blockIdx.x / 8) : rd * G + (int)blockIdx.x;
    if (j >= njobs) continue;
    const int nb = j % nblkN;
    j /= nblkN;
    const int th = j % tilesH;
    j /= tilesH;
    const int tw = j % tilesW;
    j /= tilesW;
    const int seg = j % nseg;
    const int b = j / nseg;
    const int oh0 = th * C::TH, ow0 = tw * C::TW, n0 = nb * 32;
    const int s_beg = seg * steps_per_seg;
    const int s_end = (s_beg + steps_per_seg < steps_total) ? s_beg + steps_per_seg : steps_total;
    const int nsteps = s_end - s_beg;
    const int d0 = 2 * s_beg;
    const u32x4_t rx = make_rsrc(x + (long long)b * xv.sb, x_bytes), ry = make_rsrc(y + (long long)b * yv.sb, y_bytes);
    const u32x4_t rx1 = (KH == 2 && xkh) ? make_rsrc(x + xkh + (long long)b * xv.sb, x_bytes) : rx;
    const int khoff = (KH == 2 && xkh) ? 0 : 32;

    if (nb != nb_loaded) {
#pragma unroll
      for (int t = 0; t < 27; ++t) {
        const int wt = taps.wt[t];
#pragma unroll
        for (int kh = 0; kh < KH; ++kh) {
          const long long idx = ((((long long)nb * (2 * KH) + 2 * kh + (q >> 1)) * ntaps_src + wt) * 2 + (q & 1)) * 32 + chalf * 16 + v;
          wreg[kh][t] = *reinterpret_cast<const uint4 *>(w + idx * 8);
        }
      }
      nb_loaded = nb;
    }
    float bv[4];
#pragma unroll
    for (int r = 0; r < 4; ++r) bv[r] = (!GST && bias) ? bias[n0 + chalf * 16 + 4 * q + r] : 0.f;
    const __amdgpu_buffer_rsrc_t rg =
        __builtin_amdgcn_make_buffer_rsrc((void *)(gst.y + (long long)b * gst.v.sb), (short)0, (int)gst.bytes, 0x00020000);
    if (GST) {
      if (tid < 32) {
        const int c = n0 + tid;
        const float mu = gst.mr[((long long)b * Cout + c) * 2], rs = gst.mr[((long long)b * Cout + c) * 2 + 1];
        const float a = gst.gamma[c] * rs;
        gcst[tid * 2] = a;
        gcst[tid * 2 + 1] = gst.beta[c] - mu * a;
      }
    }
#pragma unroll
    for (int t = 0; t < 27; ++t)
#pragma unroll
      for (int kh = 0; kh < KH; ++kh) asm volatile("" ::"v"(wreg[kh][t].x), "v"(wreg[kh][t].w));
#pragma unroll
    for (int r = 0; r < 4; ++r) asm volatile("" ::"v"(bv[r]));

    auto piece_off = [&](int i) -> unsigned {
      const int idx = wave + C::NW * i;
      const int P = idx % C::SUB_PIECES, kh = (idx / C::SUB_PIECES) % KH;
      const int e = P * 16 + (lane >> 2), row = e / C::IW, u = e - row * C::IW;
      const int g = (lane & 3) ^ (((u >> 2) & 1) << 1);
      const int gh = oh0 - 1 + row, gw = ow0 - 1 + u;
      const bool ok = idx < 2 * C::PIECES && e < C::NVOX && (unsigned)gh < (unsigned)H && (unsigned)gw < (unsigned)W;
      return ok ? (unsigned)((gh * xv.sh + gw * xv.sw + kh * khoff + g * 8) * 2) : RSRC_OOB;
    };
    unsigned poff[KH == 1 ? C::NPW : 1];
    if (KH == 1) {
#pragma unroll
      for (int i = 0; i < C::NPW; ++i) poff[i] = piece_off(i);
    }
    const int ovox = v + 16 * (q & 1);
    const unsigned ooff = (ow0 + ovox < W) ? (unsigned)((ovox * yv.sw + chalf * 16 + (q >> 1) * 8) * 2) : RSRC_OOB;
    const unsigned goff = (GST && ow0 + ovox < W) ? (unsigned)((ovox * gst.v.sw + chalf * 16 + (q >> 1) * 8) * 2) : RSRC_OOB;
    const bool wv0 = ow0 + v < W, wv1 = ow0 + 16 + v < W;
    const bool full_w = ow0 + 32 <= W;

    auto issue_piece = [&](int i, int pr, int ip) -> int {
      const int idx = wave + C::NW * i;
      if (C::NW * i + C::NW - 1 < 2 * C::PIECES || idx < 2 * C::PIECES) {
        const int gd = d0 - 1 + ip + idx / C::PIECES;
        const bool dok = (unsigned)gd < (unsigned)D;
        const unsigned soff = dok ? (unsigned)(gd * xv.sd * 2) : 0u;
        const unsigned voff = (KH == 1 ? poff[KH == 1 ? i : 0] : piece_off(i)) | (dok ? 0u : RSRC_OOB);
        const bool half1 = KH == 2 && ((idx / C::SUB_PIECES) % KH) == 1;
        dma16_buf_to_lds(half1 ? rx1 : rx, voff, soff, lds0 + pr * (2 * C::PLANE) + idx * 1024);
        return 1;
      }
      return 0;
    };

    f32x4_t acc[2][2][2];
    f32x2_t s1[2] = {{0.f, 0.f}, {0.f, 0.f}}, s2[2] = {{0.f, 0.f}, {0.f, 0.f}};
    f32x2_t gs1[4], gs2[4];
#pragma unroll
    for (int t = 0; t < 4; ++t) gs1[t] = gs2[t] = f32x2_t{0.f, 0.f};
    u32x4_t gy[2];
    int issued = 0;

    auto load_gy = [&](int k, int od) {
#pragma unroll
      for (int oh = 0; oh < 2; ++oh) {
        const int odg = d0 + 2 * k + od, ohg = oh0 + 2 * ws + oh;
        if (odg < D && ohg < H) {
          const unsigned soff = (unsigned)(((long long)odg * gst.v.sd + (long long)ohg * gst.v.sh + (long long)ow0 * gst.v.sw + n0) * 2);
          gy[oh] = __builtin_amdgcn_raw_buffer_load_b128(rg, goff, soff, 0);
          ++issued;
        }
      }
    };

    auto epilogue_row = [&](int k, int od, int oh) {
      const int odg = d0 + 2 * k + od, ohg = oh0 + 2 * ws + oh;
      if (odg < D && ohg < H) {
        const f32x4_t a0 = acc[od][oh][0], a1 = acc[od][oh][1];
        if (!GST) {
          auto sums = [&](const f32x2_t l0, const f32x2_t h0, const f32x2_t l1, const f32x2_t h1) {
            s1[0] += l0 + l1;
            s1[1] += h0 + h1;
            s2[0] = __builtin_elementwise_fma(l0, l0, __builtin_elementwise_fma(l1, l1, s2[0]));
            s2[1] = __builtin_elementwise_fma(h0, h0, __builtin_elementwise_fma(h1, h1, s2[1]));
          };
          const f32x2_t z2 = {0.f, 0.f};
          if (full_w)
            sums(__builtin_shufflevector(a0, a0, 0, 1), __builtin_shufflevector(a0, a0, 2, 3),
                 __builtin_shufflevector(a1, a1, 0, 1), __builtin_shufflevector(a1, a1, 2, 3));
          else
            sums(wv0 ? __builtin_shufflevector(a0, a0, 0, 1) : z2, wv0 ? __builtin_shufflevector(a0, a0, 2, 3) : z2,
                 wv1 ? __builtin_shufflevector(a1, a1, 0, 1) : z2, wv1 ? __builtin_shufflevector(a1, a1, 2, 3) : z2);
        }
        const unsigned x0 = pack2_pk<T16>(a0[0], a0[1]), x1 = pack2_pk<T16>(a0[2], a0[3]);
        const unsigned y0 = pack2_pk<T16>(a1[0], a1[1]), y1 = pack2_pk<T16>(a1[2], a1[3]);
        const auto p0 = __builtin_amdgcn_permlane16_swap(x0, y0, false, false);
        const auto p1 = __builtin_amdgcn_permlane16_swap(x1, y1, false, false);
        const u32x4_t val = {p0[0], p1[0], p0[1], p1[1]};
        const unsigned soff = (unsigned)(((long long)odg * yv.sd + (long long)ohg * yv.sh + (long long)ow0 * yv.sw + n0) * 2);
        store16_buf(ry, ooff, soff, val);
        ++issued;
        if (GST && goff != RSRC_OOB) {
          const u32x4_t yq = gy[oh];
#pragma unroll
          for (int t = 0; t < 4; ++t) {
            const float4 c4 = *reinterpret_cast<const float4 *>(gcst + (chalf * 16 + (q >> 1) * 8 + 2 * t) * 2);
            const f32x2_t gA = {c4.x, c4.z}, gB = {c4.y, c4.w};
            float g0, g1, yy0, yy1;
            unpack2_16<T16>(val[t], g0, g1);
            unpack2_16<T16>(yq[t], yy0, yy1);
            const f32x2_t g2 = {g0, g1}, y2 = {yy0, yy1};
            const f32x2_t a2 = __builtin_elementwise_fma(gA, y2, gB);
            const f32x2_t gsl = g2 * gst.slope;
            const f32x2_t q2 = {a2[0] > 0.f ? g2[0] : gsl[0], a2[1] > 0.f ? g2[1] : gsl[1]};
            gs1[t] += q2;
            gs2[t] = __builtin_elementwise_fma(q2, y2, gs2[t]);
          }
        }
      }
    };

    uint4 fr[2][6 * KH];
    auto load_row = [&](int rs, int kkv, uint4(&f)[6 * KH]) {
      const int dz = rs >> 2, hy = rs & 3;
      int slot = 2 * kkv + dz;
      slot = slot >= 6 ? slot - 6 : slot;
      const int sb = slot * C::PLANE;
#pragma unroll
      for (int kw = 0; kw < 3; ++kw)
#pragma unroll
        for (int hf = 0; hf < 2; ++hf)
#pragma unroll
          for (int kh = 0; kh < KH; ++kh)
            f[(kw * 2 + hf) * KH + kh] = *reinterpret_cast<const uint4 *>(smem + (aoff[kw] + sb) + kh * C::SUB + hy * C::ROWB + hf * 1024);
    };
    auto init_acc = [&]() {
#pragma unroll
      for (int od = 0; od < 2; ++od)
#pragma unroll
        for (int oh = 0; oh < 2; ++oh)
#pragma unroll
          for (int hf = 0; hf < 2; ++hf)
#pragma unroll
            for (int r = 0; r < 4; ++r) acc[od][oh][hf][r] = bv[r];
    };
    int mark_cur = 0, mark_nxt = 0;
    auto issue_group = [&](int pr, int ip) __attribute__((always_inline)) {
#pragma unroll
      for (int i = 0; i < C::NPW; ++i) issued += issue_piece(i, pr, ip);
      return issued;
    };
    auto rows = [&](auto rs0c, auto rs1c, auto bar7c, auto dma0c, int k, int kkv, bool more) {
      constexpr int RS0 = decltype(rs0c)::value, RS1 = decltype(rs1c)::value, DMA0 = decltype(dma0c)::value;
      constexpr bool BAR7 = decltype(bar7c)::value;
      const int prn = kkv == 0 ? 2 : kkv - 1;
#pragma unroll
      for (int rs = RS0; rs < RS1; ++rs) {
        const int dz = rs >> 2, hy = rs & 3;
        if (BAR7 && rs == 7) {
          ring_wait_all_but(issued - mark_cur);
          lds_barrier();
        }
        if (DMA0 >= 0 && more && rs >= DMA0 && rs < DMA0 + C::NPW) {
          issued += issue_piece(rs - DMA0, prn, 2 * k + 4);
          if (rs == DMA0 + C::NPW - 1) mark_nxt = issued;
        }
        if (GST && rs == 8) load_gy(k, 0);
        if (GST && rs == 12) load_gy(k, 1);
        __builtin_amdgcn_sched_barrier(0);
        if (rs + 1 < 16) load_row(rs + 1, kkv, fr[(rs + 1) & 1]);
#pragma unroll
        for (int kw = 0; kw < 3; ++kw)
#pragma unroll
          for (int hf = 0; hf < 2; ++hf)
#pragma unroll
            for (int kd = 0; kd < 3; ++kd)
#pragma unroll
              for (int kh = 0; kh < 3; ++kh) {
                const int od = dz - kd, oh = hy - kh;
                if (od >= 0 && od < 2 && oh >= 0 && oh < 2) {
#pragma unroll
                  for (int kq = 0; kq < KH; ++kq)
                    mfma16<T16>(wreg[kq][(kd * 3 + kh) * 3 + kw], fr[rs & 1][(kw * 2 + hf) * KH + kq], acc[od][oh][hf]);
                }
              }
        if (rs + 1 < 16) {
          const int nm = ((dz == 1 || dz == 2) ? 2 : 1) * ((hy == 1 || hy == 2) ? 2 : 1);
          if (nm == 1) ring_sched_interleave<6 * KH, 6 * KH>();
          else if (nm == 2) ring_sched_interleave<12 * KH, 6 * KH>();
          else ring_sched_interleave<24 * KH, 6 * KH>();
        }
        __builtin_amdgcn_sched_barrier(0);
        if (rs == 10 || rs == 11 || rs == 14 || rs == 15) epilogue_row(k, (rs >> 2) - 2, (rs & 3) - 2);
      }
    };
    typedef std::integral_constant<int, 0> I0;
    typedef std::integral_constant<int, 16> I16;

    lds_barrier();
    const int mark_p = issue_group(0, 0);
    mark_cur = issue_group(1, 2);
    ring_wait_all_but(issued - mark_p);
    lds_barrier();
    int kk = 0;
    {
      for (int k = 0; k < nsteps; ++k) {
        const bool more = k + 1 < nsteps;
        mark_nxt = issued;
        init_acc();
        load_row(0, kk, fr[0]);
        rows(I0{}, I16{}, std::true_type{}, I0{}, k, kk, more);
        mark_cur = mark_nxt;
        kk = kk == 2 ? 0 : kk + 1;
      }
    }

    if (stats && GST) {
#pragma unroll
      for (int e = 0; e < 8; ++e) {
        float a = gs1[e >> 1][e & 1], c2 = gs2[e >> 1][e & 1];
#pragma unroll
        for (int m = 1; m < 32; m <<= 1) {
          a += __shfl_xor(a, m, 64);
          c2 += __shfl_xor(c2, m, 64);
        }
        if ((lane & 31) == 0) {
          red[(wave * 16 + (q >> 1) * 8 + e) * 2 + 0] = a;
          red[(wave * 16 + (q >> 1) * 8 + e) * 2 + 1] = c2;
        }
      }
    }
    if (stats) {
#pragma unroll
      for (int r = 0; r < 4 && !GST; ++r) {
        float a = s1[r >> 1][r & 1], c2 = s2[r >> 1][r & 1];
#pragma unroll
        for (int m = 1; m < 16; m <<= 1) {
          a += __shfl_xor(a, m, 64);
          c2 += __shfl_xor(c2, m, 64);
        }
        if (v == 0) {
          red[(wave * 16 + 4 * q + r) * 2 + 0] = a;
          red[(wave * 16 + 4 * q + r) * 2 + 1] = c2;
        }
      }
      lds_barrier();
      const int nblk = tilesH * tilesW * nseg;
      if (tid < 32 && n0 + tid < Cout) {
        const int ch = tid >> 4, cc = tid & 15;
        double s = 0.0, ss = 0.0;
#pragma unroll
        for (int wq = 0; wq < C::NW / 2; ++wq) {
          s += (double)red[((wq * 2 + ch) * 16 + cc) * 2 + 0];
          ss += (double)red[((wq * 2 + ch) * 16 + cc) * 2 + 1];
        }
        const int slot = (seg * tilesW + tw) * tilesH + th;
        double *pp = stats + 32 + (((int64_t)b * nblk + slot) * Cout + n0 + tid) * 2;
        pp[0] = s;
        pp[1] = ss;
      }
      if (blockIdx.x == 0 && tid == 0 && rd == 0) reinterpret_cast<long long *>(stats)[0] = nblk;
    }
  }
}

}

namespace {

template <int KH>
int ring_launch_kh(const ConvLaunch &L, const Taps &taps, int64_t stats_cap_slots, int is_f16) {
  typedef RingCfgT<KH> C;
  const void *x = L.x, *w = L.w;
  void *y = L.y;
  const View &xv = L.xv, &yv = L.yv;
  const int B = L.B, Cout = L.Cout, ntaps_src = L.ntaps_src;
  const float *bias = L.bias;
  double *stats = L.stats;
  hipStream_t st = L.st;
  RowsGstCtx *gctx = L.gst;
  const long long xkh = L.xkh;
  const bool dry = L.dry;
  if (xkh && (KH != 2 || xkh % 8 || xv.sw != 32)) return DGTTA_ERR_UNSUPPORTED;
  const long long xb = ((long long)(xv.D - 1) * xv.sd + (long long)(xv.H - 1) * xv.sh + (long long)(xv.W - 1) * xv.sw + (xkh ? 32 : 32 * KH)) * 2;
  const long long yb = ((long long)(yv.D - 1) * yv.sd + (long long)(yv.H - 1) * yv.sh + (long long)(yv.W - 1) * yv.sw + Cout) * 2;
  if (xb >= (1ll << 31) || yb >= (1ll << 31)) return DGTTA_ERR_UNSUPPORTED;
  if (xv.sw % 8 || xv.sh % 8 || xv.sd % 8 || xv.sb % 8 || yv.sw % 8 || yv.sh % 8 || yv.sd % 8 || yv.sb % 8 || ((uintptr_t)x & 15) ||
      ((uintptr_t)y & 15))
    return DGTTA_ERR_UNSUPPORTED;
  static int ncu = [] {
    int dev = 0, n = 256;
    if (hipGetDevice(&dev) == hipSuccess) (void)hipDeviceGetAttribute(&n, hipDeviceAttributeMultiprocessorCount, dev);
    return n > 0 ? n : 256;
  }();
  const int tW = cdiv(yv.W, C::TW), tH = cdiv(yv.H, C::TH), nblkN = Cout / 32;
  const int steps_total = (yv.D + 1) / 2;
  const long long ncol = (long long)B * nblkN * tW * tH;
  int nseg = 1;
  {
    double best = 1e300;
    for (int s = 1; s <= 32 && s <= steps_total; s *= 2) {
      const int sps = cdiv(steps_total, s);
      const int ns = cdiv(steps_total, sps);
      const double t = (double)cdiv64(ncol * ns, ncu) * (sps + 1.5);
      if (t < best * 0.97) best = t, nseg = ns;
    }
  }
  const int sps = cdiv(steps_total, nseg);
  nseg = cdiv(steps_total, sps);
  if (stats && (int64_t)tW * tH * nseg > stats_cap_slots) return DGTTA_ERR_UNSUPPORTED;
  const long long njobs = ncol * nseg;
  if (njobs >= (1ll << 31)) return DGTTA_ERR_UNSUPPORTED;
  RingGst ga{};
  const long long gb = gctx ? ((long long)(yv.D - 1) * yv.H * yv.W * gctx->ldy + (long long)(yv.H - 1) * yv.W * gctx->ldy +
                               (long long)(yv.W - 1) * gctx->ldy + Cout) * 2 : 0;
  const bool gst_on = gctx && !stats && !bias && gctx->ldy % 8 == 0 && ((uintptr_t)gctx->y & 15) == 0 && gb < (1ll << 31) &&
                      (int64_t)tW * tH * nseg <= stats_cap_slots;
  if (gst_on) {
    ga.y = (const bf16_t *)gctx->y;
    ga.v = dense_view(B, yv.D, yv.H, yv.W, (int)gctx->ldy);
    ga.mr = gctx->mr;
    ga.gamma = gctx->gamma;
    ga.beta = gctx->beta;
    ga.slope = gctx->slope;
    ga.bytes = (unsigned)gb;
    stats = gctx->out;
    if (!dry) gctx->produced = 1;
  }
  if (dry) return DGTTA_OK;
  const int grid = (int)(njobs < ncu ? njobs : ncu);
#define RING_LAUNCH(T16, GSTV)                                                                                                \
  do {                                                                                                                        \
    auto kern = conv3_ring_kernel<T16, GSTV, KH>;                                                                             \
    static DynLdsOnce once;                                                                                                   \
    DG_REQUIRE(ensure_dyn_lds(once, reinterpret_cast<const void *>(kern), C::LDS_BYTES) == hipSuccess, DGTTA_ERR_LAUNCH,      \
               "conv3_ring: cannot raise the dynamic LDS limit to %d", C::LDS_BYTES);                                         \
    hipLaunchKernelGGL(kern, dim3(grid), dim3(C::NT), C::LDS_BYTES, st, (const bf16_t *)x, xv, (const bf16_t *)w, taps, bias, \
                       (bf16_t *)y, yv, Cout, tW, tH, nblkN, nseg, sps, (int)njobs, stats, ntaps_src, (unsigned)xb,           \
                       (unsigned)yb, ga, xkh);                                                                                \
  } while (0)
  if (gst_on) {
    if (is_f16) RING_LAUNCH(f16_t, true);
    else RING_LAUNCH(bf16_t, true);
  } else if (is_f16) {
    RING_LAUNCH(f16_t, false);
  } else {
    RING_LAUNCH(bf16_t, false);
  }
#undef RING_LAUNCH
  DG_CHECK_LAUNCH("conv3_ring_kernel");
  return DGTTA_OK;
}

}

int conv3_ring_launch(const ConvLaunch &L, const Taps &taps, int64_t stats_cap_slots, int is_f16) {
  if (L.Cin != L.CinP || (L.Cin != 32 && L.Cin != 64) || L.Cout % 32 != 0 || L.CoutP != L.Cout) return DGTTA_ERR_UNSUPPORTED;
  if (L.xv.D != L.yv.D || L.xv.H != L.yv.H || L.xv.W != L.yv.W) return DGTTA_ERR_UNSUPPORTED;
  if (L.Cin == 64) {
    if (dgtta_switches().conv_ring == '3') return DGTTA_ERR_UNSUPPORTED;
    return ring_launch_kh<2>(L, taps, stats_cap_slots, is_f16);
  }
  return ring_launch_kh<1>(L, taps, stats_cap_slots, is_f16);
}
```

dg_tta_amd/csrc/conv_rows.hip:

```cpp
#include "conv_common.h"
#include <stdlib.h>

namespace {

template <int PD, int PH, int WD, int WH>
struct RowsCfg {
  static constexpr int NW = WD * WH, NT = NW * 64;
  static constexpr int TD = PD * WD, TH = PH * WH, TW = 32;
  static constexpr int ID = TD + 2, IH = TH + 2, ROW = TW + 2;
  static constexpr int NROW = ID * IH, RB = 68;
  static constexpr size_t A_BYTES = ((size_t)NROW * RB * 16 + 1023) / 1024 * 1024;
  static constexpr size_t B_BYTES = 27 * 1024;
  static constexpr size_t RED_BYTES = (size_t)NW * 32 * 2 * sizeof(float) + 32 * 2 * sizeof(float);
  static constexpr size_t LDS_BYTES = 2 * A_BYTES + B_BYTES + RED_BYTES;
};

struct GstArgs {
  const bf16_t *y;
  View v;
  const float *mr, *gamma, *beta;
  float slope;
};

template <int PD, int PH, int WD, int WH, typename T16 = bf16_t, bool GST = false>
__global__ __launch_bounds__(WD *WH * 64) void conv3_rows_kernel(const bf16_t *__restrict__ x, View xv,
                                                                 const bf16_t *__restrict__ w, Taps taps,
                                                                 const float *__restrict__ bias, bf16_t *__restrict__ y,
                                                                 View yv, int Cin, int Cout, int CinP, int tilesW,
                                                                 int tilesH, int tilesD, int nblkN, int njobs,
                                                                 double *__restrict__ stats, int ntaps_src, int order,
                                                                 GstArgs gst) {
  typedef RowsCfg<PD, PH, WD, WH> Cfg;
  constexpr int NW = Cfg::NW, IH = Cfg::IH;
  extern __shared__ __attribute__((aligned(16))) unsigned char smem[];
  unsigned char *sAb = smem;
  unsigned char *sBb = smem + 2 * Cfg::A_BYTES;
  float *red = reinterpret_cast<float *>(smem + 2 * Cfg::A_BYTES + Cfg::B_BYTES);
  float *gcst = red + NW * 32 * 2;
  bool gst_newrun = true;

  const int tid = threadIdx.x, lane = tid & 63, wave = __builtin_amdgcn_readfirstlane(tid >> 6);
  const int r = lane & 31, h = lane >> 5;
  const int wd = wave / WH, wh = wave % WH;
  const int Di = xv.D, Hi = xv.H, Wi = xv.W, Do = yv.D, Ho = yv.H, Wo = yv.W;
  const int nk = CinP / 16;
  const int cin_lim = (Cin + 7) / 8 * 8;

  const int G = gridDim.x;
  int jbeg, jstep, jend;
  if (order == 0) {
    const int lw = (G % 8 == 0) ? (int)(blockIdx.x % 8) * (G / 8) + (int)(blockIdx.x / 8) : (int)blockIdx.x;
    jbeg = (int)(((long long)njobs * lw) / G), jend = (int)(((long long)njobs * (lw + 1)) / G), jstep = 1;
  } else if (G % 8 == 0) {
    const int xcd = (int)(blockIdx.x % 8), nl = G / 8;
    jbeg = (int)(((long long)njobs * xcd) / 8) + (int)(blockIdx.x / 8);
    jend = (int)(((long long)njobs * (xcd + 1)) / 8);
    jstep = nl;
  } else {
    jbeg = (int)blockIdx.x, jend = njobs, jstep = G;
  }
  const int nmine = jbeg < jend ? (jend - jbeg + jstep - 1) / jstep : 0;
  const int nph = nmine * nk;
  if (nph == 0) return;
  const int NBL = (order != 0 && (nblkN == 2 || nblkN == 4)) ? nblkN : 1;
  int TDL = NBL == 1 ? 8 : 4, THL = NBL == 4 ? 2 : 4;
  while (tilesD % TDL) TDL >>= 1;
  while (tilesH % THL) THL >>= 1;
  if (order == 0) TDL = tilesD, THL = 1;
  const int nbH = nblkN / NBL, tdH = tilesD / TDL, thH = tilesH / THL;
  struct Job {
    int b, n0, od0, oh0, ow0, tile;
  };
  auto decode = [&](int j) {
    Job q;
    const int nb_lo = j % NBL;
    j /= NBL;
    const int td_lo = j % TDL;
    j /= TDL;
    const int th_lo = j % THL;
    j /= THL;
    const int td = (j % tdH) * TDL + td_lo;
    j /= tdH;
    int th, nb;
    if (order == 0) {
      nb = j % nblkN;
      j /= nblkN;
      th = j % tilesH;
      j /= tilesH;
    } else {
      th = (j % thH) * THL + th_lo;
      j /= thH;
      nb = (j % nbH) * NBL + nb_lo;
      j /= nbH;
    }
    const int tw = j % tilesW;
    q.b = j / tilesW;
    q.n0 = nb * 32;
    q.od0 = td * Cfg::TD;
    q.oh0 = th * Cfg::TH;
    q.ow0 = tw * 32;
    q.tile = (tw * tilesH + th) * tilesD + td;
    return q;
  };

  int my_wt[(27 + NW - 1) / NW];
#pragma unroll
  for (int i = 0; i < (27 + NW - 1) / NW; ++i) {
    const int tap = wave + i * NW;
    my_wt[i] = __builtin_amdgcn_readfirstlane(tap < 27 ? (int)taps.wt[tap] : -1);
  }

  constexpr int NPR = (Cfg::NROW + NW - 1) / NW, NPB = (27 + NW - 1) / NW, NPIECE = 2 * NPR + NPB;
  const int m_g = lane >> 5, m_wx = lane & 31, t_g = (lane >> 1) & 1, t_wx = 32 + (lane & 1);
  auto issue_piece = [&](const Job &q, int kc, int buf, int i) {
    if (i < 2 * NPR) {
      const int row = wave + (i >> 1) * NW;
      const bool tail = i & 1;
      if (row < Cfg::NROW && (!tail || lane < 4)) {
        const int dz = row / IH, hy = row % IH;
        const int gd = q.od0 - 1 + dz, gh = q.oh0 - 1 + hy;
        const int g = tail ? t_g : m_g, gw = q.ow0 - 1 + (tail ? t_wx : m_wx);
        const int c = kc * 16 + g * 8;
        const bool ok = (unsigned)gd < (unsigned)Di && (unsigned)gh < (unsigned)Hi && (unsigned)gw < (unsigned)Wi &&
                        c < cin_lim;
        const bf16_t *rowp = x + (long long)q.b * xv.sb + gd * xv.sd + gh * xv.sh;
        const void *src = ok ? (const void *)(rowp + gw * xv.sw + c) : (const void *)&g_zero16;
        dma16_to_lds(src, lds_addr_of(sAb + (size_t)buf * Cfg::A_BYTES + (row * Cfg::RB + (tail ? 64 : 0)) * 16));
      }
    } else {
      const int tap = wave + (i - 2 * NPR) * NW;
      if (tap < 27) {
        const int wt = my_wt[i - 2 * NPR];
        const void *src = wt >= 0 ? (const void *)(w + ((((long long)(q.n0 / 32) * nk + kc) * ntaps_src + wt) * 64 + lane) * 8)
                                  : (const void *)&g_zero16;
        dma16_to_lds(src, lds_addr_of(sBb + tap * 1024));
      }
    }
  };

  f32x16_t acc[PD][PH];
  int abase[3];
#pragma unroll
  for (int kw = 0; kw < 3; ++kw) {
    const int col = r + kw;
    abase[kw] = ((wd * PD) * IH + wh * PH) * Cfg::RB + (col < 32 ? h * 32 + col : 64 + h * 2 + (col - 32));
  }

  int dg[8], sdg[8];
  const int rad[7] = {NBL, TDL, THL, tdH, thH, nbH, tilesW};
  {
    int a = jbeg, c = jstep;
#pragma unroll
    for (int k = 0; k < 7; ++k) {
      dg[k] = a % rad[k];
      a /= rad[k];
      sdg[k] = c % rad[k];
      c /= rad[k];
    }
    dg[7] = a;
    sdg[7] = c;
  }
  auto advance = [&]() {
    int carry = 0;
#pragma unroll
    for (int k = 0; k < 7; ++k) {
      const int v = dg[k] + sdg[k] + carry;
      carry = v >= rad[k] ? 1 : 0;
      dg[k] = carry ? v - rad[k] : v;
    }
    dg[7] += sdg[7] + carry;
    Job q;
    const int nb = dg[5] * NBL + dg[0], td = dg[3] * TDL + dg[1], th = dg[4] * THL + dg[2], tw = dg[6];
    q.b = dg[7];
    q.n0 = nb * 32;
    q.od0 = td * Cfg::TD;
    q.oh0 = th * Cfg::TH;
    q.ow0 = tw * 32;
    q.tile = (tw * tilesH + th) * tilesD + td;
    return q;
  };
  Job cur = decode(jbeg);
  float bv = 0.f;
  float st1 = 0.f, st2 = 0.f;
#pragma unroll
  for (int i = 0; i < NPIECE; ++i) issue_piece(cur, 0, 0, i);
  int kc = 0, jn = jbeg;
  for (int p = 0; p < nph; ++p) {
    dma_wait_all();
    lds_barrier();
    uint4 breg[27];
    const uint4 *sB = reinterpret_cast<const uint4 *>(sBb);
    auto load_b = [&](int kd, int kh) {
#pragma unroll
      for (int kw = 0; kw < 3; ++kw) breg[(kd * 3 + kh) * 3 + kw] = sB[((kd * 3 + kh) * 3 + kw) * 64 + lane];
    };
    static_assert(PD == 2 && PH == 2, "the just-in-time weight schedule is written for 2 x 2 patches");
    load_b(0, 0);
    if (kc == 0) {
      const int co = cur.n0 + r;
      bv = (bias && co < Cout) ? bias[co] : 0.f;
      asm volatile("" ::"v"(bv));
      if (GST && gst_newrun) {
        if (tid < 32) {
          const int c = cur.n0 + tid;
          const float mu = gst.mr[((long long)cur.b * Cout + c) * 2], rs = gst.mr[((long long)cur.b * Cout + c) * 2 + 1];
          const float a = gst.gamma[c] * rs;
          gcst[tid * 2] = a;
          gcst[tid * 2 + 1] = gst.beta[c] - mu * a;
        }
        for (int i = tid; i < NW * 32 * 2; i += Cfg::NT) red[i] = 0.f;
        gst_newrun = false;
      }
    }
    Job nxt = cur;
    int kn = kc + 1;
    if (kn == nk) {
      kn = 0;
      if (p + 1 < nph) nxt = order != 0 ? advance() : decode(jn + jstep);
    }
    const bool more = p + 1 < nph;

    if (kc == 0) {
#pragma unroll
      for (int i = 0; i < PD; ++i)
#pragma unroll
        for (int j = 0; j < PH; ++j)
#pragma unroll
          for (int q = 0; q < 16; ++q) acc[i][j][q] = bv;
    }
    {
      const uint4 *sA = reinterpret_cast<const uint4 *>(sAb + (size_t)(p & 1) * Cfg::A_BYTES);
#pragma unroll
      for (int dz = 0; dz < PD + 2; ++dz)
#pragma unroll
        for (int hy = 0; hy < PH + 2; ++hy) {
          const int rs = dz * (PH + 2) + hy;
          constexpr int sched[8][2] = {{0, 1}, {0, 2}, {1, 0}, {1, 1}, {1, 2}, {2, 0}, {2, 1}, {2, 2}};
          if (rs < 8) {
            __builtin_amdgcn_sched_barrier(0);
            load_b(sched[rs][0], sched[rs][1]);
          } else if (rs == 8) {
            __builtin_amdgcn_sched_barrier(0);
            lds_barrier();
          }
#pragma unroll
          for (int kw = 0; kw < 3; ++kw) {
            const uint4 af = sA[abase[kw] + (dz * IH + hy) * Cfg::RB];
            {
              constexpr int NSTEP = (PD + 2) * (PH + 2) * 3;
              static_assert((2 * NPR * NSTEP) / NPIECE + 1 > 24, "weight pieces must follow the mid-loop barrier");
              const int step = (dz * (PH + 2) + hy) * 3 + kw;
#pragma unroll
              for (int i = 0; i < NPIECE; ++i)
                if (step == (i * NSTEP) / NPIECE + 1 && more) issue_piece(nxt, kn, (p + 1) & 1, i);
            }
#pragma unroll
            for (int kd = 0; kd < 3; ++kd)
#pragma unroll
              for (int kh = 0; kh < 3; ++kh) {
                const int od = dz - kd, oh = hy - kh;
                if (od >= 0 && od < PD && oh >= 0 && oh < PH) mfma_step<T16>(af, breg[(kd * 3 + kh) * 3 + kw], acc[od][oh]);
              }
          }
        }
    }

    if (kc == nk - 1) {
      lds_barrier();
      int le = lane;
      asm volatile("" : "+v"(le));
      const int re = le & 31, he = le >> 5;
      const int co = cur.n0 + re;
      unsigned char *slabb = sAb + (size_t)(p & 1) * Cfg::A_BYTES + wave * (PD * PH * 2048);
      const bool full = cur.od0 + Cfg::TD <= Do && cur.oh0 + Cfg::TH <= Ho && cur.ow0 + 32 <= Wo && cur.n0 + 32 <= Cout;
      if (full) {
        const int swz = (re >> 1) & 7;
        const int cq = le >> 4, li = le & 15, rq = li >> 2, rp = li & 3;
        f32x2_t s1v = {0.f, 0.f}, s2v = {0.f, 0.f};
        uint4 gy[GST ? PD * PH * 2 : 1];
        f32x2_t gs1[4], gs2[4], gA[4], gB[4];
        if (GST) {
#pragma unroll
          for (int k = 0; k < PD * PH; ++k) {
            const int od = cur.od0 + wd * PD + k / PH, oh = cur.oh0 + wh * PH + k % PH;
            const bf16_t *yrow = gst.y + (long long)cur.b * gst.v.sb + od * gst.v.sd + oh * gst.v.sh + cur.n0 + cq * 8;
#pragma unroll
            for (int vb = 0; vb < 2; ++vb)
              gy[k * 2 + vb] = *reinterpret_cast<const uint4 *>(yrow + (long long)(cur.ow0 + 16 * vb + li) * gst.v.sw);
          }
#pragma unroll
          for (int t = 0; t < 4; ++t) {
            const float4 c4 = *reinterpret_cast<const float4 *>(gcst + (cq * 8 + 2 * t) * 2);
            gs1[t] = gs2[t] = f32x2_t{0.f, 0.f};
            gA[t] = f32x2_t{c4.x, c4.z};
            gB[t] = f32x2_t{c4.y, c4.w};
          }
        }
        auto part1 = [&](int i, int j) {
          unsigned char *sl = slabb + (i * PH + j) * 2048 + re * 64;
#pragma unroll
          for (int g = 0; g < 4; ++g) {
            const f32x2_t a = {acc[i][j][4 * g], acc[i][j][4 * g + 1]}, c = {acc[i][j][4 * g + 2], acc[i][j][4 * g + 3]};
            s1v += a;
            s1v += c;
            s2v = __builtin_elementwise_fma(a, a, s2v);
            s2v = __builtin_elementwise_fma(c, c, s2v);
            uint2 pk;
            pk.x = pack2_16<T16>(a[0], a[1]);
            pk.y = pack2_16<T16>(c[0], c[1]);
            *reinterpret_cast<uint2 *>(sl + (((2 * g + he) ^ swz) << 3)) = pk;
          }
        };
        auto part2 = [&](int i, int j) {
          const int od = cur.od0 + wd * PD + i, oh = cur.oh0 + wh * PH + j;
          bf16_t *orow = y + (long long)cur.b * yv.sb + od * yv.sd + oh * yv.sh + cur.n0 + cq * 8;
          const unsigned char *sl = slabb + (i * PH + j) * 2048;
#pragma unroll
          for (int vb = 0; vb < 2; ++vb) {
            const int c0 = 8 * cq + rq, c1 = c0 + 4, sidx = 4 * vb + rp;
            const s16x4_t lo = __builtin_amdgcn_ds_read_tr16_b64_v4i16(
                (lds_s16x4_t *)(sl + c0 * 64 + ((sidx ^ ((c0 >> 1) & 7)) << 3)));
            const s16x4_t hi = __builtin_amdgcn_ds_read_tr16_b64_v4i16(
                (lds_s16x4_t *)(sl + c1 * 64 + ((sidx ^ ((c1 >> 1) & 7)) << 3)));
            uint4 val;
            val.x = (unsigned)(unsigned short)lo[0] | ((unsigned)(unsigned short)lo[1] << 16);
            val.y = (unsigned)(unsigned short)lo[2] | ((unsigned)(unsigned short)lo[3] << 16);
            val.z = (unsigned)(unsigned short)hi[0] | ((unsigned)(unsigned short)hi[1] << 16);
            val.w = (unsigned)(unsigned short)hi[2] | ((unsigned)(unsigned short)hi[3] << 16);
            if (GST) {
              const uint4 yq = gy[(i * PH + j) * 2 + vb];
              const unsigned gw[4] = {val.x, val.y, val.z, val.w}, yw[4] = {yq.x, yq.y, yq.z, yq.w};
#pragma unroll
              for (int t = 0; t < 4; ++t) {
                float g0, g1, y0, y1;
                unpack2_16<T16>(gw[t], g0, g1);
                unpack2_16<T16>(yw[t], y0, y1);
                const f32x2_t g2 = {g0, g1}, y2 = {y0, y1};
                const f32x2_t a2 = __builtin_elementwise_fma(gA[t], y2, gB[t]);
                const f32x2_t gsl = g2 * gst.slope;
                const f32x2_t q2 = {a2[0] > 0.f ? g2[0] : gsl[0], a2[1] > 0.f ? g2[1] : gsl[1]};
                gs1[t] += q2;
                gs2[t] = __builtin_elementwise_fma(q2, y2, gs2[t]);
              }
            }
            const int ow = cur.ow0 + 16 * vb + li;
            st16_nt(orow + ow * yv.sw, val);
          }
        };
#pragma unroll
        for (int k = 0; k <= PD * PH; ++k) {
          if (k < PD * PH) part1(k / PH, k % PH);
          if (k > 0) part2((k - 1) / PH, (k - 1) % PH);
        }
        st1 += s1v[0] + s1v[1];
        st2 += s2v[0] + s2v[1];
        if (GST) {
#pragma unroll
          for (int e = 0; e < 8; ++e) {
            float a = gs1[e >> 1][e & 1], c2 = gs2[e >> 1][e & 1];
            a += __int_as_float(__builtin_amdgcn_update_dpp(0, __float_as_int(a), 0xB1, 0xf, 0xf, false));
            c2 += __int_as_float(__builtin_amdgcn_update_dpp(0, __float_as_int(c2), 0xB1, 0xf, 0xf, false));
            a += __int_as_float(__builtin_amdgcn_update_dpp(0, __float_as_int(a), 0x4E, 0xf, 0xf, false));
            c2 += __int_as_float(__builtin_amdgcn_update_dpp(0, __float_as_int(c2), 0x4E, 0xf, 0xf, false));
            a += __int_as_float(__builtin_amdgcn_update_dpp(0, __float_as_int(a), 0x141, 0xf, 0xf, false));
            c2 += __int_as_float(__builtin_amdgcn_update_dpp(0, __float_as_int(c2), 0x141, 0xf, 0xf, false));
            a += __int_as_float(__builtin_amdgcn_update_dpp(0, __float_as_int(a), 0x140, 0xf, 0xf, false));
            c2 += __int_as_float(__builtin_amdgcn_update_dpp(0, __float_as_int(c2), 0x140, 0xf, 0xf, false));
            if (li == 0) {
              float2 *slot = reinterpret_cast<float2 *>(red + (wave * 32 + cq * 8 + e) * 2);
              float2 cur2 = *slot;
              cur2.x += a;
              cur2.y += c2;
              *slot = cur2;
            }
          }
        }
      } else {
        bf16_t *slab = reinterpret_cast<bf16_t *>(slabb);
#pragma unroll
        for (int i = 0; i < PD; ++i)
#pragma unroll
          for (int j = 0; j < PH; ++j) {
            const int od = cur.od0 + wd * PD + i, oh = cur.oh0 + wh * PH + j;
            const bool row_ok = od < Do && oh < Ho;
#pragma unroll
            for (int q = 0; q < 16; ++q) {
              const int m = (q & 3) + 8 * (q >> 2) + 4 * he;
              const float v = acc[i][j][q];
              slab[(i * PH + j) * 1024 + m * 32 + re] = f32_to_16<T16>(v);
              if (row_ok && co < Cout && cur.ow0 + m < Wo) {
                st1 += v;
                st2 += v * v;
              }
            }
          }
#pragma unroll
        for (int i = 0; i < PD; ++i)
#pragma unroll
          for (int j = 0; j < PH; ++j) {
            const int od = cur.od0 + wd * PD + i, oh = cur.oh0 + wh * PH + j;
            bf16_t *orow = y + (long long)cur.b * yv.sb + od * yv.sd + oh * yv.sh + cur.n0;
#pragma unroll
            for (int t = 0; t < 2; ++t) {
              const int m = t * 16 + (le >> 2), cq = (le & 3) * 8;
              const uint4 val = *reinterpret_cast<const uint4 *>(slab + (i * PH + j) * 1024 + m * 32 + cq);
              const int ow = cur.ow0 + m;
              if (od < Do && oh < Ho && ow < Wo && cur.n0 + cq < Cout)
                *reinterpret_cast<uint4 *>(orow + ow * yv.sw + cq) = val;
            }
          }
      }
      if (stats) {
        const bool flush = !(p + 1 < nph) || nxt.b != cur.b || nxt.n0 != cur.n0;
        const int tiles_per_b = tilesW * tilesH * tilesD;
        double *pp = stats + 32 + (((int64_t)cur.b * tiles_per_b + cur.tile) * Cout + cur.n0 + tid) * 2;
        if (flush) {
          if (!GST) {
            const float a = st1 + __shfl_xor(st1, 32, 64), c2 = st2 + __shfl_xor(st2, 32, 64);
            if (he == 0) {
              red[(wave * 32 + re) * 2 + 0] = a;
              red[(wave * 32 + re) * 2 + 1] = c2;
            }
          } else {
            gst_newrun = true;
          }
          st1 = st2 = 0.f;
          lds_barrier();
          if (tid < 32 && cur.n0 + tid < Cout) {
            double s = 0.0, ss = 0.0;
#pragma unroll
            for (int wv = 0; wv < NW; ++wv) {
              s += (double)red[(wv * 32 + tid) * 2 + 0];
              ss += (double)red[(wv * 32 + tid) * 2 + 1];
            }
            pp[0] = s;
            pp[1] = ss;
          }
        } else if (tid < 32 && cur.n0 + tid < Cout) {
          pp[0] = 0.0;
          pp[1] = 0.0;
        }
        if (blockIdx.x == 0 && tid == 0 && p == nk - 1) reinterpret_cast<long long *>(stats)[0] = tiles_per_b;
      }
    }
    kc = kn;
    if (kn == 0) {
      cur = nxt;
      jn += jstep;
    }
  }
}

}

namespace {

template <int PD, int PH, int WD, int WH, typename T16>
int launch_conv_rows(const ConvLaunch &L, const Taps &taps) {
  typedef RowsCfg<PD, PH, WD, WH> Cfg;
  const View &xv = L.xv, &yv = L.yv;
  const int B = L.B, Cin = L.Cin, Cout = L.Cout, CinP = L.CinP, CoutP = L.CoutP;
  const float *bias = L.bias;
  double *stats = L.stats;
  RowsGstCtx *gctx = L.gst;
  GstArgs ga{};
  const bool gst_on = gctx && !stats && !bias && yv.D % Cfg::TD == 0 && yv.H % Cfg::TH == 0 && yv.W % 32 == 0 && Cout % 32 == 0 &&
                      CoutP == Cout && gctx->ldy % 8 == 0 && ((uintptr_t)gctx->y & 15) == 0;
  if (gst_on) {
    ga.y = (const bf16_t *)gctx->y;
    ga.v = dense_view(B, yv.D, yv.H, yv.W, (int)gctx->ldy);
    ga.mr = gctx->mr;
    ga.gamma = gctx->gamma;
    ga.beta = gctx->beta;
    ga.slope = gctx->slope;
    stats = gctx->out;
    gctx->produced = 1;
  }
  auto kern = conv3_rows_kernel<PD, PH, WD, WH, T16>;
  static DynLdsOnce once_plain, once_gst;
  if (gst_on) kern = conv3_rows_kernel<PD, PH, WD, WH, T16, true>;
  DG_REQUIRE(ensure_dyn_lds(gst_on ? once_gst : once_plain, reinterpret_cast<const void *>(kern), (int)Cfg::LDS_BYTES) == hipSuccess,
             DGTTA_ERR_LAUNCH, "conv3_rows: cannot raise the dynamic LDS limit to %zu", (size_t)Cfg::LDS_BYTES);
  const int tW = cdiv(yv.W, 32), tH = cdiv(yv.H, Cfg::TH), tD = cdiv(yv.D, Cfg::TD), nblkN = cdiv(CoutP, 32);
  const long long njobs = (long long)tW * tH * tD * nblkN * B;
  DG_REQUIRE(njobs < (1ll << 31), DGTTA_ERR_UNSUPPORTED, "conv3_rows: too many tiles");
  static int ncu = [] {
    int dev = 0, n = 256;
    if (hipGetDevice(&dev) == hipSuccess) (void)hipDeviceGetAttribute(&n, hipDeviceAttributeMultiprocessorCount, dev);
    return n > 0 ? n : 256;
  }();
  const int wg_per_cu = (int)((160 * 1024) / Cfg::LDS_BYTES) > 0 ? (int)((160 * 1024) / Cfg::LDS_BYTES) : 1;
  const int grid = (int)(njobs < (long long)ncu * wg_per_cu ? njobs : (long long)ncu * wg_per_cu);
  hipLaunchKernelGGL(kern, dim3(grid), dim3(Cfg::NT), Cfg::LDS_BYTES, L.st, (const bf16_t *)L.x, xv, (const bf16_t *)L.w, taps,
                     bias, (bf16_t *)L.y, yv, Cin, Cout, CinP, tW, tH, tD, nblkN, (int)njobs, stats, L.ntaps_src,
                     dgtta_switches().rows_order == '0' ? 0 : 1, ga);
  DG_CHECK_LAUNCH("conv3_rows_kernel");
  return DGTTA_OK;
}

}

int conv3_rows_launch(const ConvLaunch &L, const Taps &taps, int is_f16) {
  if (is_f16) return launch_conv_rows<2, 2, 2, 4, f16_t>(L, taps);
  return launch_conv_rows<2, 2, 2, 4, bf16_t>(L, taps);
}
```

dg_tta_amd/csrc/lib.hip:

```cpp
#include "common.h"
#include <string.h>

static thread_local char g_err[512] = "";

void dgtta_set_error(const char *fmt, ...) {
  va_list ap;
  va_start(ap, fmt);
  vsnprintf(g_err, sizeof(g_err), fmt, ap);
  va_end(ap);
}

extern "C" int dgtta_version(void) { return 60200;  }
extern "C" const char *dgtta_last_error(void) { return g_err; }

#include <mutex>
#include <stdlib.h>

static std::atomic<const DgttaSwitches *> g_switches{nullptr};
static std::once_flag g_switches_once;


static int env_char(const char *name) {
  const char *v = getenv(name);
  return (v && v[0] && !v[1] && v[0] >= '0' && v[0] <= '9') ? (int)(unsigned char)v[0] : -1;
}

static const DgttaSwitches *read_switches() {
  DgttaSwitches *s = new DgttaSwitches;
  s->conv_rows = env_char("DGTTA_CONV_ROWS");
  s->conv_s2 = env_char("DGTTA_CONV_S2");
  s->convt_gemm = env_char("DGTTA_CONVT_GEMM");
  s->rows_order = env_char("DGTTA_ROWS_ORDER");
  s->wgrad_upw = env_char("DGTTA_WGRAD_UPW");
  s->wgrad_xcd = env_char("DGTTA_WGRAD_XCD");
  s->in_nt = env_char("DGTTA_IN_NT");
  s->in_nt = s->in_nt == '0' ? '0' : '1';
  s->dgrad_s2_allcls = env_char("DGTTA_DGRAD_S2_ALLCLS");
  s->wgrad_tr = env_char("DGTTA_WGRAD_TR");
  s->wgrad_tr8 = env_char("DGTTA_WGRAD_TR8");
  s->wgrad_s2_onepass = env_char("DGTTA_WGRAD_S2_ONEPASS");
  s->convt_wgrad_onepass = env_char("DGTTA_CONVT_WGRAD_ONEPASS");
  s->in_gstats = env_char("DGTTA_IN_GSTATS");
  s->softdice16 = env_char("DGTTA_SOFTDICE16");
  s->conv_ring = env_char("DGTTA_CONV_RING");
  s->wgrad_ring = env_char("DGTTA_WGRAD_RING");
  s->ha_mfma = env_char("DGTTA_HA_MFMA");
  s->wgrad_f32_split = env_char("DGTTA_WGRAD_F32_SPLIT");
  s->feature_head_mfma = env_char("DGTTA_FEATURE_HEAD_MFMA");
  s->headwarp_mfma = env_char("DGTTA_HEADWARP_MFMA");
  s->wgrad_flat = env_char("DGTTA_WGRAD_FLAT");
  s->wgrad_reduce_taps = env_char("DGTTA_WGRAD_REDUCE_TAPS");
  if (s->conv_ring != '0' && s->conv_ring != '1' && s->conv_ring != '3') s->conv_ring = -1;
  if (s->wgrad_ring != '0' && s->wgrad_ring != '1' && s->wgrad_ring != '4' && s->wgrad_ring != '5' && s->wgrad_ring != '6') s->wgrad_ring = -1;
  if (s->convt_gemm != '0' && s->convt_gemm != '1') s->convt_gemm = -1;
  return s;
}

const DgttaSwitches &dgtta_switches() {
  std::call_once(g_switches_once, [] { g_switches.store(read_switches(), std::memory_order_release); });
  return *g_switches.load(std::memory_order_acquire);
}

extern "C" int dgtta_reload_env(void) {
  (void)dgtta_switches();
  g_switches.store(read_switches(), std::memory_order_release);
  return DGTTA_OK;
}
```

dg_tta_amd/unet_exec.py:

```python
import contextlib
import ctypes as C
import os

import torch

from . import _lib
from ._lib import check, ptr, stream_of
from ._state import state_of
from .ops import F32, F16, _ws, dtype_code

EPS, SLOPE = 1e-5, 1e-2


def _wgrad_on_side_stream():
    return os.environ.get("DGTTA_WGRAD_STREAM", "1") != "0"


def _pad(c, m):
    return (c + m - 1) // m * m


def _k3(k):
    return tuple(k) if isinstance(k, (tuple, list)) else (k, k, k)


def _odim(i, s):
    return (i + 2 - 3) // s + 1


def _check_patch_divisible(strides, dims):
    tot = [1, 1, 1]
    for s in strides:
        tot = [a * b for a, b in zip(tot, _k3(s))]
    assert all(d % t == 0 for d, t in zip(dims, tot)), \
        f"patch {dims[0]}x{dims[1]}x{dims[2]} must be divisible by {tot[0]}x{tot[1]}x{tot[2]} (the product of the strides per axis)"


def window_segments(origins, w, max_cover=4):
    launches = []
    k = 0
    while k < len(origins):
        j = k + 1
        while (j < len(origins) and origins[j][:2] == origins[k][:2]
               and origins[j - 1][2] < origins[j][2] < origins[j - 1][2] + w):
            j += 1
        if j - k == 1:
            launches.append(k)
        else:
            sx, sy = origins[k][:2]
            zs = [origins[i][2] for i in range(k, j)]
            cuts = sorted(set(zs + [z + w for z in zs]))
            for a, b in zip(cuts[:-1], cuts[1:]):
                cover = [i for i in range(k, j) if origins[i][2] <= a and b <= origins[i][2] + w]
                for c0 in range(0, len(cover), max_cover):
                    launches.append((sx, sy, a, b, cover[c0:c0 + max_cover]))
        k = j
    return launches


class _Rows:
    __slots__ = ("t", "ptr", "ld")

    def __init__(self, t, ptr_, ld):
        self.t, self.ptr, self.ld = t, ptr_, ld


class _Workspaces:

    def __init__(self, dev):
        self.dev, self.bufs = dev, {}

    def get(self, nbytes, key="ws"):
        nb = int(nbytes)
        t = self.bufs.get(key)
        if t is None or t.numel() < nb:
            t = self.bufs[key] = _ws(nb, self.dev)
        return t


@contextlib.contextmanager
def _timed(probe, where, key, nbatch, stream=None, **info):
    if probe is None or probe["where"] != where:
        yield
        return
    ev0, ev1 = torch.cuda.Event(enable_timing=True), torch.cuda.Event(enable_timing=True)
    ev0.record(stream)
    yield
    ev1.record(stream)
    probe.setdefault(key, []).append((ev0, ev1, nbatch))
    probe.update(info)


class _Pass:

    def __init__(self, net, dev, batch):
        self.lib, self.net, self.dev, self.B = _lib.load(), net, dev, batch
        self.adt, self.impl = net.act_dtype, net.conv_impl
        self.dt = dtype_code(self.adt)
        self.esz = 4 if self.dt == F32 else 2
        self.cp = 8 if self.dt == F32 else 16
        self.st = stream_of(dev)
        self.ws = _Workspaces(dev)
        self.probe = state_of(net).probe

    def empty(self, *shape, dtype=None):
        return torch.empty(shape, dtype=self.adt if dtype is None else dtype, device=self.dev)


class _BackwardPass(_Pass):

    def __init__(self, net, dev, batch):
        super().__init__(net, dev, batch)
        self.grads = {}
        self.inplace = bool(net.accumulate_grads_in_place)
        self.acc = 1 if self.inplace else 0
        self.main_stream = torch.cuda.current_stream(dev)
        self.side = state_of(net).stream("side_stream", dev) if _wgrad_on_side_stream() else None
        if self.side is not None:
            self.side.wait_stream(self.main_stream)

    def gbuf(self, p):
        if self.inplace:
            if p.grad is None:
                p.grad = torch.zeros_like(p, memory_format=torch.contiguous_format)
            return p.grad
        g = self.grads.get(id(p))
        if g is None:
            g = self.grads[id(p)] = torch.zeros_like(p, memory_format=torch.contiguous_format)
        return g

    def scratch_like(self, p):
        if self.side is None:
            return torch.empty_like(p)
        with torch.cuda.stream(self.side):
            return torch.empty_like(p)

    def hand_over(self, nbytes, *reads):
        if self.side is None:
            return self.ws.get(nbytes), self.st
        ev = torch.cuda.Event()
        ev.record(self.main_stream)
        self.side.wait_event(ev)
        for t in reads:
            t.record_stream(self.side)
        with torch.cuda.stream(self.side):
            w = self.ws.get(nbytes, "ws_side")
        return w, self.side.cuda_stream


class _ConvLayer:
    __slots__ = ("mod", "where", "aniso", "halfwise", "cin", "cout", "cinp", "coutp", "stride", "din", "dout", "vout",
                 "x", "xbs", "y", "mr", "z")

    def __init__(self, p, mod, where, cin, din):
        conv = mod.conv
        self.mod, self.where, self.aniso = mod, where, conv.aniso
        self.halfwise = not conv.aniso
        self.cin, self.cout = cin, conv.out_channels
        self.cinp, self.coutp = _pad(cin, p.cp), _pad(self.cout, p.cp)
        self.stride = _k3(conv.stride)
        self.din, self.dout = tuple(din), tuple(_odim(i, s) for i, s in zip(din, self.stride))
        self.vout = self.dout[0] * self.dout[1] * self.dout[2]

    def weights(self, p, cin_slice=None):
        conv = self.mod.conv
        if self.aniso:
            assert cin_slice is None, "the anisotropic kernels have no packed weight slices"
            return p.net.kpacked(conv, p.dt, self.cinp, self.coutp)
        if cin_slice is None:
            return p.net.packed(conv, p.dt, self.cinp, self.coutp)
        return p.net.packed(conv, p.dt, _pad(cin_slice[1] - cin_slice[0], p.cp), self.coutp, cin_slice)

    def forward(self, p, x, xbs=0):
        conv, B, cin, cout = self.mod.conv, p.B, self.cin, self.cout
        self.x, self.xbs = x, xbs
        w = self.weights(p)
        self.y = p.empty(B, *self.dout, cout)
        stats = p.ws.get(p.lib.dgtta_conv3d_stats_bytes(B, cout, *self.dout), "stats")
        with _timed(p.probe, self.where, "events", B, cin=cin, cout=cout, vout=self.vout, batch=B):
            if self.aniso:
                check(p.lib.dgtta_conv3d_fwd(x.ptr, x.ld, ptr(w), ptr(conv.bias), ptr(self.y), cout, ptr(stats), B, cin, cout,
                                             self.cinp, self.coutp, *self.din, conv.kernel_size[0], *self.stride, p.dt, p.st),
                      "dgtta_conv3d_fwd")
            elif xbs:
                check(p.lib.dgtta_conv3d_k3_fwd_blocked(x.ptr, xbs, ptr(w), ptr(conv.bias), ptr(self.y), cout, ptr(stats), B, cin,
                                                        cout, self.cinp, self.coutp, *self.din, p.dt, p.st),
                      "dgtta_conv3d_k3_fwd_blocked")
            else:
                check(p.lib.dgtta_conv3d_k3_fwd(x.ptr, x.ld, ptr(w), ptr(conv.bias), ptr(self.y), cout, ptr(stats), B, cin, cout,
                                                self.cinp, self.coutp, *self.din, self.stride[0], p.dt, p.impl, p.st),
                      "dgtta_conv3d_k3_fwd")
        return stats

    def dgrad(self, p, dy, dst, ld, accumulate=0, cin_slice=None):
        cin = self.cin if cin_slice is None else cin_slice[1] - cin_slice[0]
        w = self.weights(p, cin_slice)
        if self.aniso:
            check(p.lib.dgtta_conv3d_dgrad(ptr(dy), self.cout, ptr(w), dst, ld, p.B, cin, self.cout, self.cinp, self.coutp,
                                           *self.din, self.mod.conv.kernel_size[0], *self.stride, accumulate, p.dt, p.st),
                  "dgtta_conv3d_dgrad")
        else:
            check(p.lib.dgtta_conv3d_k3_dgrad(ptr(dy), self.cout, ptr(w), dst, ld, p.B, cin, self.cout, _pad(cin, p.cp),
                                              self.coutp, *self.din, self.stride[0], accumulate, p.dt, p.impl, p.st),
                  "dgtta_conv3d_k3_dgrad")

    def dgrad_gstats(self, p, dy, gin, prev):
        if self.aniso or self.stride[0] != 1 or p.dt == F32 or prev.cout != self.cin or prev.dout != self.din:
            return self.dgrad(p, dy, ptr(gin), self.cin)
        w, pn, cin = self.weights(p), prev.mod.norm, self.cin
        gbytes = p.lib.dgtta_conv3d_stats_bytes(p.B, cin, *self.din)
        gstats = p.ws.get(gbytes, "gstats")
        produced = C.c_int(0)
        check(p.lib.dgtta_conv3d_k3_dgrad_gstats(ptr(dy), self.cout, ptr(w), ptr(gin), cin, p.B, cin, self.cout, self.cinp,
                                                 self.coutp, *self.din, ptr(prev.y), cin, ptr(prev.mr), ptr(pn.weight),
                                                 ptr(pn.bias), SLOPE, ptr(gstats), gbytes, C.byref(produced), p.dt, p.impl, p.st),
              "dgtta_conv3d_k3_dgrad_gstats")
        return gstats if produced.value else None

    def wgrad_ws_bytes(self, p):
        B, cin, cout, s = p.B, self.cin, self.cout, self.stride[0]
        if self.aniso:
            return p.lib.dgtta_conv3d_kwgrad_ws_bytes(B, cin, cout, *self.din, self.mod.conv.kernel_size[0], *self.stride)
        if p.dt == F32 and p.impl != 1 and (s == 1 or not ((self.din[0] | self.din[1] | self.din[2]) & 1)):
            return p.lib.dgtta_conv3d_wgrad_split_ws_bytes(B, cin, cout, *self.dout, s)
        return p.lib.dgtta_conv3d_wgrad_ws_bytes(B, cin, cout, *self.dout)

    def wgrad(self, p, dy, dw, db, ws, nb, stream):
        x, cin, cout = self.x, self.cin, self.cout
        if self.aniso:
            check(p.lib.dgtta_conv3d_wgrad(x.ptr, x.ld, ptr(dy), cout, ptr(dw), ptr(db), ptr(ws), nb, p.B, cin, cout, *self.din,
                                           self.mod.conv.kernel_size[0], *self.stride, p.acc, p.dt, stream), "dgtta_conv3d_wgrad")
        elif self.xbs:
            check(p.lib.dgtta_conv3d_k3_wgrad_blocked(x.ptr, self.xbs, ptr(dy), cout, ptr(dw), ptr(db), ptr(ws), nb, p.B, cin,
                                                      cout, *self.din, p.acc, p.dt, stream), "dgtta_conv3d_k3_wgrad_blocked")
        else:
            check(p.lib.dgtta_conv3d_k3_wgrad(x.ptr, x.ld, ptr(dy), cout, ptr(dw), ptr(db), ptr(ws), nb, p.B, cin, cout,
                                              *self.din, self.stride[0], p.acc, p.dt, p.impl, stream), "dgtta_conv3d_k3_wgrad")


class _UpLayer:
    __slots__ = ("mod", "aniso", "halfwise", "cin", "cout", "din", "x")

    def __init__(self, mod, cin, cout, din):
        self.mod, self.aniso, self.cin, self.cout, self.din = mod, mod.aniso, cin, cout, tuple(din)
        self.halfwise = not mod.aniso

    def fwd(self, p, x, out):
        m = self.mod
        self.x = x
        if self.aniso:
            nb = p.lib.dgtta_convT3d_s_fwd_ws_bytes(self.cin, self.cout, *m.kernel_size, p.dt)
            ws = p.ws.get(nb)
            check(p.lib.dgtta_convT3d_s_fwd(x.ptr, x.ld, ptr(m.weight), ptr(m.bias), out.ptr, out.ld, ptr(ws), nb, p.B, self.cin,
                                            self.cout, *self.din, *m.kernel_size, p.dt, p.st), "dgtta_convT3d_s_fwd")
        else:
            nb = p.lib.dgtta_convT3d_fwd_ws_bytes(self.cin, self.cout, p.dt)
            ws = p.ws.get(nb)
            check(p.lib.dgtta_convT3d_k2s2_fwd(x.ptr, x.ld, ptr(m.weight), ptr(m.bias), out.ptr, out.ld, ptr(ws), nb, p.B,
                                               self.cin, self.cout, *self.din, p.dt, p.impl, p.st), "dgtta_convT3d_k2s2_fwd")

    def bwd_ws_bytes(self, p):
        if self.aniso:
            return p.lib.dgtta_convT3d_s_bwd_ws_bytes(p.B, self.cin, self.cout, *self.din, *self.mod.kernel_size)
        return (p.lib.dgtta_convT3d_bwd_split_ws_bytes if p.dt == F32 and p.impl != 1 else
                p.lib.dgtta_convT3d_bwd_ws_bytes)(p.B, self.cin, self.cout, *self.din)

    def bwd(self, p, g, dx, dw, db, ws, nb, stream):
        x, m = self.x, self.mod
        if self.aniso:
            check(p.lib.dgtta_convT3d_s_bwd(x.ptr, x.ld, g.ptr, g.ld, ptr(m.weight), dx, self.cin, dw, db, ptr(ws), nb, p.B,
                                            self.cin, self.cout, *self.din, *m.kernel_size, p.acc, p.dt, stream),
                  "dgtta_convT3d_s_bwd")
        else:
            check(p.lib.dgtta_convT3d_k2s2_bwd(x.ptr, x.ld, g.ptr, g.ld, ptr(m.weight), dx, self.cin, dw, db, ptr(ws), nb, p.B,
                                               self.cin, self.cout, *self.din, p.acc, p.dt, p.impl, stream),
                  "dgtta_convT3d_k2s2_bwd")


class _Cat:
    __slots__ = ("buf", "c", "dims", "xbs")

    def __init__(self, p, c, dims, planar):
        self.c, self.dims = c, dims
        if planar:
            self.buf = p.empty(2, p.B, *dims, c)
            self.xbs = p.B * dims[0] * dims[1] * dims[2] * c
        else:
            self.buf = p.empty(p.B, *dims, 2 * c)
            self.xbs = 0

    def rows(self):
        return _Rows(self.buf, self.buf.data_ptr(), self.c if self.xbs else 2 * self.c)

    def skip_rows(self, p):
        if self.xbs:
            return _Rows(self.buf, self.buf[1].data_ptr(), self.c)
        return _Rows(self.buf, self.buf.data_ptr() + self.c * p.esz, 2 * self.c)


def _plan(p, cin, dims):
    enc_mods, dec_mods = p.net.conv_blocks()
    enc, ups, dec = [], [], []
    for si, mods in enumerate(enc_mods):
        enc.append([])
        for bi, mod in enumerate(mods):
            blk = _ConvLayer(p, mod, ("enc", si, bi), cin, dims)
            enc[-1].append(blk)
            cin, dims = blk.cout, blk.dout
    for k, mods in enumerate(dec_mods):
        skip = enc[-(k + 2)][-1]
        ups.append(_UpLayer(p.net.decoder.transpconvs[k], cin, skip.cout, dims))
        cin, dims = 2 * skip.cout, skip.dout
        dec.append([])
        for bi, mod in enumerate(mods):
            blk = _ConvLayer(p, mod, ("dec", k, bi), cin, dims)
            dec[-1].append(blk)
            cin, dims = blk.cout, blk.dout
    return enc, ups, dec


def _input_rows(p, x):
    B, cin, D, H, W = x.shape
    cinp = _pad(cin, p.cp)
    if (x.dtype == p.adt and x.stride(1) == 1 and x.stride(4) == cinp and x.stride(3) == W * cinp
            and x.stride(2) == H * W * cinp and x.stride(0) == D * H * W * cinp):
        xin = x
    else:
        xin = p.empty(B, D, H, W, cinp)
        xs = x.contiguous().float()
        check(p.lib.dgtta_ncdhw_to_ndhwc(ptr(xs), ptr(xin), B, cin, D * H * W, cinp, p.dt, p.st), "dgtta_ncdhw_to_ndhwc")
    return _Rows(xin, xin.data_ptr(), cinp)


def _block_forward(p, blk, x, xbs=0, z=None, stats_only=False):
    B, cout = p.B, blk.cout
    norm = blk.mod.norm
    stats = blk.forward(p, x, xbs)
    blk.mr = p.empty(B, cout, 2, dtype=torch.float32)
    if stats_only:
        z = _Rows(None, None, cout)
    elif z is None:
        zt = p.empty(B, *blk.dout, cout)
        z = _Rows(zt, zt.data_ptr(), cout)
    blk.z = z
    nb = p.lib.dgtta_instnorm_ws_bytes(B, cout, blk.vout)
    ws = p.ws.get(nb)
    check(p.lib.dgtta_instnorm_lrelu_fwd(ptr(blk.y), cout, ptr(stats), ptr(norm.weight), ptr(norm.bias), ptr(blk.mr), z.ptr, z.ld,
                                         ptr(ws), nb, B, cout, blk.vout, EPS, SLOPE, p.dt, p.st), "dgtta_instnorm_lrelu_fwd")
    return z


def _planar_cat(p, skip, readers):
    c = skip.cout
    return (c * p.esz == 64 and p.impl != 1 and os.environ.get("DGTTA_PLANAR_CAT", "1") != "0"
            and all(r.halfwise for r in readers)
            and os.environ.get("DGTTA_SPLIT_CAT_GRAD", "1") != "0"
            and p.lib.dgtta_conv3d_k3_blocked_supported(p.B, 2 * c, c, *skip.dout, p.dt) == 1)


def _encoder_forward(p, enc, ups, dec, x):
    cats = []
    for si, stage in enumerate(enc):
        for blk in stage:
            z = None
            if blk is stage[-1] and si < len(enc) - 1:
                dk = len(enc) - 2 - si
                cats.append(_Cat(p, blk.cout, blk.dout, _planar_cat(p, blk, (enc[si + 1][0], dec[dk][0], ups[dk]))))
                z = cats[-1].skip_rows(p)
            x = _block_forward(p, blk, x, z=z)
    return x, cats


def _decoder_forward(p, ups, dec, cats, x, feat_fold):
    stage_rows = []
    for up, stage, cat in zip(ups, dec, reversed(cats)):
        up.fwd(p, x, cat.rows())
        x = cat.rows()
        for blk in stage:
            fold = feat_fold and blk is dec[-1][-1]
            x = _block_forward(p, blk, x, xbs=cat.xbs if blk is stage[0] else 0, stats_only=fold)
        stage_rows.append(x)
    return stage_rows


def _accumulate_feature_windows(p, wa, last, z, feat_fold, dims):
    lib, dt, st = p.lib, p.dt, p.st
    acc, nsum, gauss, origins = wa[:4]
    X, Y, Z = acc.shape[:3]
    D, H, W = dims
    nrm = last.mod.norm
    src0 = last.y.data_ptr() if feat_fold else z.ptr
    assert (32 if feat_fold else z.ld) == 32
    wbytes = D * H * W * 32 * p.esz
    mrbytes = 32 * 2 * 4
    segments = os.environ.get("DGTTA_FEATURE_SEGMENTS", "1") != "0"
    for launch in window_segments(origins, W) if segments else range(len(origins)):
        if isinstance(launch, int):
            k = launch
            sx, sy, sz = origins[k]
            if feat_fold:
                check(lib.dgtta_feature_window_accumulate_norm(src0 + k * wbytes, last.mr.data_ptr() + k * mrbytes, ptr(nrm.weight),
                                                               ptr(nrm.bias), SLOPE, ptr(gauss), ptr(acc), ptr(nsum), 32, D, H, W,
                                                               X, Y, Z, sx, sy, sz, dt, st), "dgtta_feature_window_accumulate_norm")
            else:
                check(lib.dgtta_feature_window_accumulate(src0 + k * wbytes, ptr(gauss), ptr(acc), ptr(nsum), 32, D, H, W, X, Y, Z,
                                                          sx, sy, sz, dt, st), "dgtta_feature_window_accumulate")
            continue
        sx, sy, a, b, part = launch
        n = len(part)
        srcs = (C.c_void_p * n)(*[src0 + i * wbytes for i in part])
        mrs = (C.c_void_p * n)(*[last.mr.data_ptr() + i * mrbytes for i in part]) if feat_fold else None
        zoffs = (C.c_int * n)(*[a - origins[i][2] for i in part])
        check(lib.dgtta_feature_window_accumulate_multi(srcs, mrs, zoffs, n, ptr(nrm.weight), ptr(nrm.bias), SLOPE, ptr(gauss),
                                                        ptr(acc), ptr(nsum), 32, D, H, W, b - a, X, Y, Z, sx, sy, a, dt, st),
              "dgtta_feature_window_accumulate_multi")


def _accumulate_logit_windows(p, wa, head, z, dims):
    acc, nsum, gauss, origins = wa[:4]
    X, Y, Z = acc.shape[:3]
    D, H, W = dims
    for k, (sx, sy, sz) in enumerate(origins):
        check(p.lib.dgtta_seghead_window_accumulate_t(z.ptr + k * D * H * W * z.ld * p.esz, ptr(head.weight), ptr(head.bias),
                                                      ptr(gauss), ptr(acc), ptr(nsum), head.in_channels, head.out_channels, D, H,
                                                      W, X, Y, Z, sx, sy, sz, p.dt, F32 if acc.dtype == torch.float32 else F16,
                                                      p.st), "dgtta_seghead_window_accumulate_t")


def _head_forward(p, head, z, sel, nsel, fw, dims):
    D, H, W = dims
    out = p.empty(p.B, D, H, W, nsel, dtype=torch.float32)
    if fw is not None:
        assert z.ld == head.in_channels and tuple(fw[0].shape) == (p.B, 3, 4), "fuse_output_warp: shape mismatch"
        check(p.lib.dgtta_seghead_warp_fwd(z.ptr, ptr(head.weight), ptr(head.bias), ptr(sel), nsel, ptr(fw[0]), ptr(out), p.B,
                                           head.in_channels, D, H, W, 1, p.dt, p.st), "dgtta_seghead_warp_fwd")
    else:
        check(p.lib.dgtta_seghead_fwd(z.ptr, z.ld, ptr(head.weight), ptr(head.bias), ptr(sel), nsel, ptr(out), 1, nsel, p.B,
                                      head.in_channels, D * H * W, p.dt, p.st), "dgtta_seghead_fwd")
    return out


def _aux_heads_forward(p, net, dec, stage_rows, sel, nsel):
    return [_head_forward(p, net.decoder.seg_layers[k], stage_rows[k], sel, nsel, None, dec[k][-1].dout)
            for k in range(len(dec) - 2, -1, -1)]


def _scatter_head_grads(p, head, sel, dws, dbs):
    cin = head.in_channels
    gw, gb = p.gbuf(head.weight), p.gbuf(head.bias)
    if sel is None:
        gw.view(-1, cin).add_(dws)
        gb.add_(dbs)
    else:
        gw.view(-1, cin).index_add_(0, sel.long(), dws)
        gb.index_add_(0, sel.long(), dbs)


def _aux_head_backward(p, head, z, sel, nsel, gout, gz, dims):
    D, H, W = dims
    cin = head.in_channels
    assert gz.ld >= cin and z.ld >= cin
    g = gout.contiguous(memory_format=torch.channels_last_3d).float()
    need_hw = head.weight.requires_grad or head.bias.requires_grad
    dws = p.empty(nsel, cin, dtype=torch.float32) if need_hw else None
    dbs = p.empty(nsel, dtype=torch.float32) if need_hw else None
    nb = p.lib.dgtta_seghead_bwd_ws_bytes(p.B, cin, nsel, D * H * W)
    ws = p.ws.get(nb)
    check(p.lib.dgtta_seghead_bwd_acc(z.ptr, z.ld, ptr(g), nsel, ptr(head.weight), ptr(sel), nsel, gz.ptr, gz.ld, ptr(dws), ptr(dbs),
                                      ptr(ws), nb, p.B, cin, D * H * W, 0, 1, p.dt, p.st), "dgtta_seghead_bwd_acc")
    if need_hw:
        _scatter_head_grads(p, head, sel, dws, dbs)


def _head_backward(p, head, z, sel, nsel, fw, g16, gout, dims):
    lib, B, dt, st = p.lib, p.B, p.dt, p.st
    D, H, W = dims
    if g16 is not None and any(gout.stride()):
        gout = gout + g16.permute(0, 4, 1, 2, 3).float()
        g16 = None
    g = None if g16 is not None else gout.contiguous(memory_format=torch.channels_last_3d).float()
    cin = head.in_channels
    gz = p.empty(B, D, H, W, cin)
    need_hw = head.weight.requires_grad or head.bias.requires_grad
    dws = p.empty(nsel, cin, dtype=torch.float32) if need_hw else None
    dbs = p.empty(nsel, dtype=torch.float32) if need_hw else None
    if fw is not None:
        nb = lib.dgtta_seghead_warp_bwd_ws_bytes(B, cin, nsel, D, H, W)
        ws = p.ws.get(nb)
        assert g16 is None or (tuple(g16.shape) == (B, D, H, W, nsel) and g16.dtype == p.adt and g16.is_contiguous())
        bwd = lib.dgtta_seghead_warp_bwd if g16 is None else lib.dgtta_seghead_warp_bwd_g16
        check(bwd(z.ptr, ptr(g if g16 is None else g16), ptr(fw[0]), ptr(fw[1]), ptr(head.weight), ptr(sel), nsel, ptr(gz),
                  ptr(dws), ptr(dbs), ptr(ws), nb, B, cin, D, H, W, 1, 0, dt, st), bwd.__name__)
    else:
        nb = lib.dgtta_seghead_bwd_ws_bytes(B, cin, nsel, D * H * W)
        ws = p.ws.get(nb)
        check(lib.dgtta_seghead_bwd(z.ptr, z.ld, ptr(g), nsel, ptr(head.weight), ptr(sel), nsel, ptr(gz), cin, ptr(dws), ptr(dbs),
                                    ptr(ws), nb, B, cin, D * H * W, 0, dt, st), "dgtta_seghead_bwd")
    if need_hw:
        _scatter_head_grads(p, head, sel, dws, dbs)
    return _Rows(gz, gz.data_ptr(), cin)


def _norm_backward(p, blk, gz, gstats):
    lib, B, cout, v = p.lib, p.B, blk.cout, blk.vout
    norm = blk.mod.norm
    dy = p.empty(B, *blk.dout, cout)
    nb = lib.dgtta_instnorm_ws_bytes(B, cout, v)
    ws = p.ws.get(nb)
    dgam = p.gbuf(norm.weight) if norm.weight.requires_grad else torch.empty_like(norm.weight)
    dbet = p.gbuf(norm.bias) if norm.bias.requires_grad else torch.empty_like(norm.bias)
    if gstats is not None:
        check(lib.dgtta_instnorm_lrelu_bwd_gstats(gz.ptr, gz.ld, ptr(blk.y), cout, ptr(norm.weight), ptr(norm.bias), ptr(blk.mr),
                                                  ptr(dy), cout, ptr(dgam), ptr(dbet), ptr(gstats), ptr(ws), nb, B, cout, v,
                                                  SLOPE, p.acc, p.dt, p.st), "dgtta_instnorm_lrelu_bwd_gstats")
    else:
        check(lib.dgtta_instnorm_lrelu_bwd(gz.ptr, gz.ld, ptr(blk.y), cout, ptr(norm.weight), ptr(norm.bias), ptr(blk.mr), ptr(dy),
                                           cout, ptr(dgam), ptr(dbet), ptr(ws), nb, B, cout, v, SLOPE, p.acc, p.dt, p.st),
              "dgtta_instnorm_lrelu_bwd")
    return dy


def _weight_grad(p, blk, dy):
    conv = blk.mod.conv
    if not (conv.weight.requires_grad or conv.bias.requires_grad):
        return
    nb = blk.wgrad_ws_bytes(p)
    dw = p.gbuf(conv.weight) if conv.weight.requires_grad else p.scratch_like(conv.weight)
    db = p.gbuf(conv.bias) if conv.bias.requires_grad else None
    if p.net.exact_zero_bias_grad:
        db = None
    ws, stream = p.hand_over(nb, dy)
    with _timed(p.probe, blk.where, "wgrad_events", p.B, p.main_stream if p.side is None else p.side):
        blk.wgrad(p, dy, dw, db, ws, nb, stream)


def _concat_grad(p, blk, dy, cat):
    B, c = p.B, cat.c
    if c * p.esz == 64 and blk.halfwise and (cat.xbs or os.environ.get("DGTTA_SPLIT_CAT_GRAD", "1") != "0"):
        halves = [p.empty(B, *cat.dims, c), p.empty(B, *cat.dims, c)]
        for i, dst in enumerate(halves):
            blk.dgrad(p, dy, ptr(dst), c, cin_slice=(i * c, (i + 1) * c))
        return tuple(_Rows(t, t.data_ptr(), c) for t in halves)
    gc = torch.empty_like(cat.buf)
    blk.dgrad(p, dy, ptr(gc), 2 * c)
    return _Rows(gc, gc.data_ptr(), 2 * c), _Rows(gc, gc.data_ptr() + c * p.esz, 2 * c)


def _up_backward(p, up, g):
    m = up.mod
    glow = p.empty(p.B, *up.din, up.cin)
    nb = up.bwd_ws_bytes(p)
    ws = p.ws.get(nb)
    need_w = m.weight.requires_grad or m.bias.requires_grad
    dw = (p.gbuf(m.weight) if m.weight.requires_grad else p.scratch_like(m.weight)) if need_w else None
    db = p.gbuf(m.bias) if m.bias.requires_grad else None
    if p.side is None or not need_w:
        up.bwd(p, g, ptr(glow), ptr(dw), ptr(db), ws, nb, p.st)
    else:
        ws_side, stream = p.hand_over(nb, g.t)
        up.bwd(p, g, ptr(glow), None, None, ws, nb, p.st)
        up.bwd(p, g, None, ptr(dw), ptr(db), ws_side, nb, stream)
    return _Rows(glow, glow.data_ptr(), up.cin)


def _plain_grad(p, blk, dy, prev):
    gin = p.empty(p.B, *blk.din, blk.cin)
    gstats = blk.dgrad_gstats(p, dy, gin, prev)
    return _Rows(gin, gin.data_ptr(), blk.cin), gstats


class _UNetFn(torch.autograd.Function):

    @staticmethod
    def forward(ctx, net, x, sel, need_grad, sink, deep_supervision, *params):
        _lib.require_cuda(x)
        B, cin0, D, H, W = x.shape
        dims = (D, H, W)
        p = _Pass(net, x.device, B)
        cfg = net.cfg
        assert cin0 == cfg["in_channels"], f"expected {cfg['in_channels']} input channels, got {cin0}"
        _check_patch_divisible(cfg["strides"], dims)
        head = net.decoder.seg_layers[-1]
        wa = net._window_acc
        feat_fold = (wa is not None and len(wa) > 4 and not need_grad and os.environ.get("DGTTA_FEATURE_FOLD", "1") != "0" and
                     head.in_channels == cfg["features"][0] == 32)
        enc, ups, dec = _plan(p, cin0, dims)
        z, cats = _encoder_forward(p, enc, ups, dec, _input_rows(p, x))
        stage_rows = _decoder_forward(p, ups, dec, cats, z, feat_fold)
        z = stage_rows[-1]
        if wa is not None:
            assert not need_grad and sel is None and z.ld == head.in_channels and len(wa[3]) == B, "fuse_window_accumulate: misuse"
            if len(wa) > 4:
                _accumulate_feature_windows(p, wa, dec[-1][-1], z, feat_fold, dims)
            else:
                _accumulate_logit_windows(p, wa, head, z, dims)
            return p.empty(B, 0, D, H, W, dtype=torch.float32)
        nsel = head.out_channels if sel is None else int(sel.numel())
        fw = net._fused_warp
        out = _head_forward(p, head, z, sel, nsel, fw, dims)
        aux = _aux_heads_forward(p, net, dec, stage_rows, sel, nsel) if deep_supervision else []
        if need_grad:
            ctx.set_materialize_grads(False)
            ctx.aux = [(stage_rows[k], dec[k][-1].dout) for k in range(len(dec) - 1)] if deep_supervision else None
            ctx.net, ctx.sel, ctx.params = net, sel, params
            ctx.blocks = [blk for stage in enc + dec for blk in stage]
            ctx.ups, ctx.cats = ups, cats
            ctx.meta = (B, dims, nsel, z)
            ctx.fused_warp = fw
            ctx.sink = sink if fw is not None else None
        if deep_supervision:
            return (out.permute(0, 4, 1, 2, 3),) + tuple(a.permute(0, 4, 1, 2, 3) for a in aux)
        return out.permute(0, 4, 1, 2, 3)

    @staticmethod
    def backward(ctx, gout, *gaux):
        net, blocks, ups, cats = ctx.net, ctx.blocks, ctx.ups, ctx.cats
        B, dims, nsel, z = ctx.meta
        if gout is None:
            dev = next(g for g in gaux if g is not None).device
            gout = torch.zeros((B, nsel) + tuple(dims), dtype=torch.float32, device=dev)
        p = _BackwardPass(net, gout.device, B)
        g16 = ctx.sink.take() if ctx.sink is not None else None
        gz = _head_backward(p, net.decoder.seg_layers[-1], z, ctx.sel, nsel, ctx.fused_warp, g16, gout, dims)
        gskip = {}
        gstats = None
        for idx in range(len(blocks) - 1, -1, -1):
            blk = blocks[idx]
            dy = _norm_backward(p, blk, gz, gstats)
            _weight_grad(p, blk, dy)
            if idx == 0:
                break
            kind, sidx, bidx = blk.where
            gstats = None
            if kind == "dec" and bidx == 0:
                gup, gskip[sidx] = _concat_grad(p, blk, dy, cats[-(sidx + 1)])
                gz = _up_backward(p, ups[sidx], gup)
                if sidx > 0 and gaux and gaux[len(ups) - 1 - sidx] is not None:
                    za, adims = ctx.aux[sidx - 1]
                    _aux_head_backward(p, net.decoder.seg_layers[sidx - 1], za, ctx.sel, nsel, gaux[len(ups) - 1 - sidx], gz, adims)
            elif kind == "enc" and bidx == 0:
                gz = gskip[len(ups) - sidx]
                blk.dgrad(p, dy, gz.ptr, gz.ld, accumulate=1)
            else:
                gz, gstats = _plain_grad(p, blk, dy, blocks[idx - 1])
        if p.side is not None:
            p.main_stream.wait_stream(p.side)
        return (None,) * 6 + tuple(p.grads.get(id(q)) if q.requires_grad else None for q in ctx.params)
```

include/dgtta.h:

```cpp
#ifndef DGTTA_H
#define DGTTA_H

#include <stddef.h>
#include <stdint.h>

#ifdef __cplusplus
extern "C" {
#endif

#define DGTTA_OK 0
#define DGTTA_ERR_BADARG (-1)
#define DGTTA_ERR_UNSUPPORTED (-2)
#define DGTTA_ERR_WORKSPACE (-3)
#define DGTTA_ERR_LAUNCH (-4)

#define DGTTA_F32 0
#define DGTTA_BF16 1
#define DGTTA_F16 2

#define DGTTA_PAD_ZEROS 0
#define DGTTA_PAD_BORDER 1
#define DGTTA_INTERP_LINEAR 0
#define DGTTA_INTERP_NEAREST 1

int dgtta_version(void);
const char *dgtta_last_error(void);
int dgtta_reload_env(void);

size_t dgtta_mind3d_ws_bytes(int B, int D, int H, int W);
int dgtta_mind3d_fwd(const float *img, const float *noise, float randn_weighting, int delta, const float *h_taps,
                     int ntaps, void *out, int out_ndhwc, int out_ldc, int out_dtype, void *ws, size_t ws_bytes, int B,
                     int D, int H, int W, void *stream);

int dgtta_mind3d_noise_fill(float *noise, uint64_t seed, uint64_t offset, int b0, int B, int D, int H, int W,
                            void *stream);
int dgtta_mind3d_fwd_seeded(const float *img, uint64_t seed, uint64_t offset, int b0, float randn_weighting, int delta,
                            const float *h_taps, int ntaps, void *out, int out_ndhwc, int out_ldc, int out_dtype,
                            void *ws, size_t ws_bytes, int B, int D, int H, int W, void *stream);

size_t dgtta_gin_ws_bytes(int B, int D, int H, int W);
int dgtta_gin_chain_fwd(const float *x, const float *alpha, const int *h_ksz, const float *const *h_ker,
                        const float *const *h_shift, float *out, void *ws, size_t ws_bytes, int B, int D, int H,
                        int W, void *stream);

int dgtta_affine_warp3d_fwd(const float *src, const float *theta, float *dst, int B, int C, int Ds, int Hs,
                            int Ws, int Dd, int Hd, int Wd, int ndhwc, int src_ldc, int dst_ldc, int pad_mode,
                            int interp_mode, int tta_grid_algebra, const float *sub_const_dev, void *stream);
int dgtta_affine_warp3d_bwd(const float *grad_dst, const float *theta, float *grad_src, int B, int C, int Ds,
                            int Hs, int Ws, int Dd, int Hd, int Wd, int ndhwc, int src_ldc, int dst_ldc,
                            int pad_mode, int tta_grid_algebra, void *stream);

size_t dgtta_rf_field_ws_bytes(int P, int Dl, int Hl, int Wl);
int dgtta_rf_field_fwd(const float *draw, float *field, void *ws, size_t ws_bytes, int P, int k, int Dl, int Hl, int Wl,
                       int D, int H, int W, void *stream);
size_t dgtta_diffeo_fields_ws_bytes(int N, int D, int H, int W);
int dgtta_diffeo_fields(const float *field, float factor, float *disp, float *inverse, void *ws, size_t ws_bytes, int N,
                        int D, int H, int W, int time_steps, void *stream);
int dgtta_dense_warp3d_fwd(const float *src, const float *disp, float *dst, int B, int C, int D, int H, int W, int ndhwc,
                           int src_ldc, int dst_ldc, int pad_mode, void *stream);
int dgtta_dense_warp3d_bwd(const float *grad_dst, const float *disp, float *grad_src, int B, int C, int D, int H, int W,
                           int ndhwc, int src_ldc, int dst_ldc, int pad_mode, void *stream);

size_t dgtta_softdice_ws_bytes(int B, int C, int64_t V);
int dgtta_softdice_fwd(const float *la, const float *lb, float *dice, float *loss, void *ws, size_t ws_bytes,
                       int B, int C, int64_t V, int ldc, int start_class, int guard_items, void *stream);
int dgtta_softdice_bwd(const float *la, const float *lb, float *grad_la, float *grad_lb, const void *ws,
                       float grad_scale, const float *grad_scale_dev, int B, int C, int64_t V, int ldc,
                       int start_class, void *stream);
int dgtta_softdice_bwd_t(const float *la, const float *lb, void *grad_la, void *grad_lb, const void *ws, float grad_scale,
                         const float *grad_scale_dev, int B, int C, int64_t V, int ldc, int start_class, int grad_dtype,
                         void *stream);

int dgtta_softdice_probs_fwd(const float *a, const float *b, float *dice, void *ws, size_t ws_bytes, int B, int C,
                             int64_t V, int64_t stride_b, int64_t stride_c, int64_t stride_v, void *stream);
int dgtta_softdice_probs_bwd(const float *a, const float *b, const float *grad_dice, float *grad_a, float *grad_b,
                             const void *ws, int B, int C, int64_t V, int64_t stride_b, int64_t stride_c,
                             int64_t stride_v, void *stream);

size_t dgtta_dice_ce_ws_bytes(int B, int C, int64_t V);
int dgtta_dice_ce_fwd(const float *logits, int ldc, const int64_t *labels, float *loss3, float *dice, void *ws,
                      size_t ws_bytes, int B, int C, int64_t V, float smooth, int do_bg, void *stream);
int dgtta_dice_ce_bwd(const float *logits, int ldc, const int64_t *labels, const void *ws, float grad_scale,
                      const float *grad_scale_dev, float *grad_logits, int ldg, int B, int C, int64_t V, void *stream);
size_t dgtta_dice_ce_ds_ws_bytes(int B, int C, int d, int h, int w);
int dgtta_dice_ce_ds_fwd(const float *logits, int ldc, const int64_t *labels_full, float *loss3, float *dice, void *ws,
                         size_t ws_bytes, int B, int C, int d, int h, int w, int sd, int sh, int sw, float smooth, int do_bg,
                         void *stream);
int dgtta_dice_ce_ds_bwd(const float *logits, int ldc, const int64_t *labels_full, const void *ws, float grad_scale,
                         const float *grad_scale_dev, float *grad_logits, int ldg, int B, int C, int d, int h, int w, int sd,
                         int sh, int sw, void *stream);

int dgtta_adamw_step(float *const *h_p, const float *const *h_g, float *const *h_m, float *const *h_v,
                     const int64_t *h_n, int ntensors, float lr, float beta1, float beta2, float eps,
                     float weight_decay, int step, float grad_scale, const int *skip_if_nonzero, void *stream);
int dgtta_grads_nonfinite(const float *const *h_g, const int64_t *h_n, int ntensors, int *flag, void *stream);

size_t dgtta_grad_sumsq_ws_bytes(int64_t total_elements, int ntensors);
int dgtta_grad_sumsq(const float *const *h_g, const int64_t *h_n, int ntensors, float *out, void *ws, size_t ws_bytes,
                     void *stream);
int dgtta_sgd_step(float *const *h_p, const float *const *h_g, float *const *h_buf, const int64_t *h_n, int ntensors,
                   float lr, float momentum, float weight_decay, int nesterov, int first_step, float grad_scale,
                   const float *sumsq, float max_norm, const int *skip_if_nonzero, void *stream);


size_t dgtta_conv3d_packed_bytes(int CinP, int CoutP, int dtype);
int dgtta_conv3d_pack_weights(const float *w_t, void *wpack, int Cin, int Cout, int CinP, int CoutP, int dtype,
                              void *stream);

size_t dgtta_conv3d_stats_bytes(int B, int Cout, int Do, int Ho, int Wo);
int dgtta_conv3d_k3_fwd(const void *x, int ldx, const void *wpack, const float *bias, void *y, int ldy, void *stats,
                        int B, int Cin, int Cout, int CinP, int CoutP, int Di, int Hi, int Wi, int stride,
                        int dtype, int impl, void *stream);
int dgtta_conv3d_k3_dgrad(const void *dy, int lddy, const void *wpack, void *dx, int lddx, int B, int Cin, int Cout,
                          int CinP, int CoutP, int Di, int Hi, int Wi, int stride, int accumulate, int dtype,
                          int impl, void *stream);
size_t dgtta_conv3d_wgrad_ws_bytes(int B, int Cin, int Cout, int Do, int Ho, int Wo);
size_t dgtta_conv3d_wgrad_split_ws_bytes(int B, int Cin, int Cout, int Do, int Ho, int Wo, int stride);
int dgtta_conv3d_k3_wgrad(const void *x, int ldx, const void *dy, int lddy, float *dw_t, float *db, void *ws,
                          size_t ws_bytes, int B, int Cin, int Cout, int Di, int Hi, int Wi, int stride,
                          int accumulate, int dtype, int impl, void *stream);
int dgtta_conv3d_k3_blocked_supported(int B, int Cin, int Cout, int D, int H, int W, int dtype);
int dgtta_conv3d_k3_fwd_blocked(const void *x, long long x_block_stride, const void *wpack, const float *bias, void *y, int ldy,
                                void *stats, int B, int Cin, int Cout, int CinP, int CoutP, int Di, int Hi, int Wi, int dtype,
                                void *stream);
int dgtta_conv3d_k3_wgrad_blocked(const void *x, long long x_block_stride, const void *dy, int lddy, float *dw_t, float *db,
                                  void *ws, size_t ws_bytes, int B, int Cin, int Cout, int Di, int Hi, int Wi, int accumulate,
                                  int dtype, void *stream);

size_t dgtta_instnorm_ws_bytes(int B, int C, int64_t V);
int dgtta_instnorm_lrelu_fwd(const void *y, int ldy, const void *stats, const float *gamma, const float *beta,
                             float *mean_rstd, void *z, int ldz, void *ws, size_t ws_bytes, int B, int C,
                             int64_t V, float eps, float slope, int dtype, void *stream);
int dgtta_instnorm_lrelu_bwd(const void *gz, int ldgz, const void *y, int ldy, const float *gamma,
                             const float *beta, const float *mean_rstd, void *dy, int lddy, float *dgamma,
                             float *dbeta, void *ws, size_t ws_bytes, int B, int C, int64_t V, float slope,
                             int accumulate, int dtype, void *stream);

int dgtta_conv3d_k3_dgrad_gstats(const void *dy, int lddy, const void *wpack, void *dx, int lddx, int B, int Cin, int Cout,
                                 int CinP, int CoutP, int Di, int Hi, int Wi, const void *y_prev, int ldy_prev,
                                 const float *mean_rstd_prev, const float *gamma_prev, const float *beta_prev, float slope,
                                 void *gstats, size_t gstats_bytes, int *h_produced, int dtype, int impl, void *stream);
int dgtta_instnorm_lrelu_bwd_gstats(const void *gz, int ldgz, const void *y, int ldy, const float *gamma, const float *beta,
                                    const float *mean_rstd, void *dy, int lddy, float *dgamma, float *dbeta,
                                    const void *gstats, void *ws, size_t ws_bytes, int B, int C, int64_t V, float slope,
                                    int accumulate, int dtype, void *stream);

size_t dgtta_convT3d_fwd_ws_bytes(int Cin, int Cout, int dtype);
int dgtta_convT3d_k2s2_fwd(const void *x, int ldx, const float *w_t, const float *bias, void *out, int ldo, void *ws,
                           size_t ws_bytes, int B, int Cin, int Cout, int Di, int Hi, int Wi, int dtype, int impl,
                           void *stream);
size_t dgtta_convT3d_bwd_ws_bytes(int B, int Cin, int Cout, int Di, int Hi, int Wi);
size_t dgtta_convT3d_bwd_split_ws_bytes(int B, int Cin, int Cout, int Di, int Hi, int Wi);
int dgtta_convT3d_k2s2_bwd(const void *x, int ldx, const void *dout, int lddo, const float *w_t, void *dx, int lddx,
                           float *dw_t, float *db, void *ws, size_t ws_bytes, int B, int Cin, int Cout, int Di,
                           int Hi, int Wi, int accumulate, int dtype, int impl, void *stream);

size_t dgtta_conv3d_kpacked_bytes(int kd, int CinP, int CoutP, int dtype);
int dgtta_conv3d_kpack_weights(const float *w_t, void *wpack, int kd, int kh, int kw, int Cin, int Cout, int CinP, int CoutP,
                               int dtype, void *stream);
int dgtta_conv3d_fwd(const void *x, int ldx, const void *wpack, const float *bias, void *y, int ldy, void *stats, int B, int Cin,
                     int Cout, int CinP, int CoutP, int Di, int Hi, int Wi, int kd, int sd, int sh, int sw, int dtype, void *stream);
int dgtta_conv3d_dgrad(const void *dy, int lddy, const void *wpack, void *dx, int lddx, int B, int Cin, int Cout, int CinP, int CoutP,
                       int Di, int Hi, int Wi, int kd, int sd, int sh, int sw, int accumulate, int dtype, void *stream);
size_t dgtta_conv3d_kwgrad_ws_bytes(int B, int Cin, int Cout, int Di, int Hi, int Wi, int kd, int sd, int sh, int sw);
int dgtta_conv3d_wgrad(const void *x, int ldx, const void *dy, int lddy, float *dw_t, float *db, void *ws, size_t ws_bytes, int B,
                       int Cin, int Cout, int Di, int Hi, int Wi, int kd, int sd, int sh, int sw, int accumulate, int dtype,
                       void *stream);
size_t dgtta_convT3d_s_fwd_ws_bytes(int Cin, int Cout, int sd, int sh, int sw, int dtype);
int dgtta_convT3d_s_fwd(const void *x, int ldx, const float *w_t, const float *bias, void *out, int ldo, void *ws, size_t ws_bytes,
                        int B, int Cin, int Cout, int Di, int Hi, int Wi, int sd, int sh, int sw, int dtype, void *stream);
size_t dgtta_convT3d_s_bwd_ws_bytes(int B, int Cin, int Cout, int Di, int Hi, int Wi, int sd, int sh, int sw);
int dgtta_convT3d_s_bwd(const void *x, int ldx, const void *dout, int lddo, const float *w_t, void *dx, int lddx, float *dw_t,
                        float *db, void *ws, size_t ws_bytes, int B, int Cin, int Cout, int Di, int Hi, int Wi, int sd, int sh,
                        int sw, int accumulate, int dtype, void *stream);

int dgtta_seghead_fwd(const void *x, int ldx, const float *w, const float *bias, const int *sel, int nsel,
                      float *out, int out_ndhwc, int ldo, int B, int Cin, int64_t V, int dtype, void *stream);
size_t dgtta_seghead_bwd_ws_bytes(int B, int Cin, int nsel, int64_t V);
int dgtta_seghead_bwd(const void *x, int ldx, const float *dout, int lddo, const float *w, const int *sel,
                      int nsel, void *dx, int lddx, float *dw_sel, float *db_sel, void *ws, size_t ws_bytes,
                      int B, int Cin, int64_t V, int accumulate, int dtype, void *stream);
int dgtta_seghead_bwd_acc(const void *x, int ldx, const float *dout, int lddo, const float *w, const int *sel,
                          int nsel, void *dx, int lddx, float *dw_sel, float *db_sel, void *ws, size_t ws_bytes,
                          int B, int Cin, int64_t V, int accumulate, int accumulate_dx, int dtype, void *stream);

int dgtta_seghead_warp_supported(const float *h_theta, int B, int Cin, int nsel, int D, int H, int W, int dtype);
size_t dgtta_seghead_warp_bwd_ws_bytes(int B, int Cin, int nsel, int D, int H, int W);
int dgtta_seghead_warp_fwd(const void *z, const float *w, const float *bias, const int *sel, int nsel, const float *theta,
                           float *out, int B, int Cin, int D, int H, int W, int tta_grid_algebra, int dtype, void *stream);
int dgtta_seghead_warp_bwd(const void *z, const float *gout, const float *theta, const float *h_theta, const float *w,
                           const int *sel, int nsel, void *gz, float *dw_sel, float *db_sel, void *ws, size_t ws_bytes, int B,
                           int Cin, int D, int H, int W, int tta_grid_algebra, int accumulate, int dtype, void *stream);
int dgtta_seghead_warp_bwd_g16(const void *z, const void *gout16, const float *theta, const float *h_theta, const float *w,
                               const int *sel, int nsel, void *gz, float *dw_sel, float *db_sel, void *ws, size_t ws_bytes, int B,
                               int Cin, int D, int H, int W, int tta_grid_algebra, int accumulate, int dtype, void *stream);

int dgtta_ncdhw_to_ndhwc(const float *src, void *dst, int B, int C, int64_t V, int ldc, int dtype, void *stream);
int dgtta_ndhwc_to_ncdhw(const void *src, float *dst, int B, int C, int64_t V, int ldc, int dtype, void *stream);

int dgtta_argmax_dice(const float *logits, int ldc, int C, const int64_t *labels, int64_t *argmax_out,
                      int64_t *counts, int B, int64_t V, void *stream);

int dgtta_window_accumulate(const float *patch, const float *gauss, float *acc, float *nsum, int C, int PD, int PH,
                            int PW, int X, int Y, int Z, int x0, int y0, int z0, void *stream);

int dgtta_seghead_window_accumulate(const void *z, const float *w, const float *bias, const float *gauss, float *acc,
                                    float *nsum, int Cin, int C, int PD, int PH, int PW, int X, int Y, int Z, int x0, int y0,
                                    int z0, int dtype, void *stream);

int dgtta_window_accumulate_t(const float *patch, const float *gauss, void *acc, float *nsum, int C, int PD, int PH, int PW,
                              int X, int Y, int Z, int x0, int y0, int z0, int acc_dtype, void *stream);
int dgtta_seghead_window_accumulate_t(const void *z, const float *w, const float *bias, const float *gauss, void *acc,
                                      float *nsum, int Cin, int C, int PD, int PH, int PW, int X, int Y, int Z, int x0, int y0,
                                      int z0, int dtype, int acc_dtype, void *stream);
int dgtta_argmax_rows(const void *logits, int acc_dtype, int C, int64_t rows, int64_t *argmax_out, void *stream);

size_t dgtta_resample_axis_ws_bytes(int64_t outer, int n, int64_t inner, int order);
int dgtta_resample_axis(const double *src, double *dst, void *ws, size_t ws_bytes, int64_t outer, int n, int m,
                        int64_t inner, int order, void *stream);

int dgtta_logits_chunk_f64(const float *acc, const float *nsum, double *dst, int C, int X, int Y, int Z, int x0, int y0,
                           int z0, int xs, int ys, int zs, int c0, int cg, void *stream);
int dgtta_argmax_merge_f64(const double *vals, int64_t V, int cg, int c0, double *best_val, int *best_idx, int first,
                           void *stream);
int dgtta_logits_chunk_f64_t(const void *acc, const float *nsum, double *dst, int C, int X, int Y, int Z, int x0, int y0,
                             int z0, int xs, int ys, int zs, int c0, int cg, int acc_dtype, void *stream);

int dgtta_feature_window_accumulate(const void *z, const float *gauss, float *facc, float *nsum, int Cin, int PD, int PH, int PW, int X,
                                    int Y, int Z, int x0, int y0, int z0, int dtype, void *stream);
int dgtta_feature_window_accumulate_norm(const void *y, const float *mean_rstd, const float *gamma, const float *beta, float slope,
                                         const float *gauss, float *facc, float *nsum, int Cin, int PD, int PH, int PW, int X, int Y,
                                         int Z, int x0, int y0, int z0, int dtype, void *stream);
int dgtta_feature_window_accumulate_multi(const void *const *h_srcs, const float *const *h_mean_rstds, const int *h_zoffs, int nsrc,
                                          const float *gamma, const float *beta, float slope, const float *gauss, float *facc,
                                          float *nsum, int Cin, int PD, int PH, int PW, int seg_len, int X, int Y, int Z, int x0, int y0,
                                          int z0, int dtype, void *stream);
int dgtta_feature_head_argmax(const float *facc, int64_t member_stride, const float *nsum, const float *w, const float *bsum, int M,
                              int Cin, int C, int64_t V, int64_t *argmax_out, void *stream);
int dgtta_feature_logits_chunk_f64(const float *facc, int64_t member_stride, const float *nsum, const float *w, const float *bsum,
                                   double *dst, int M, int Cin, int C, int X, int Y, int Z, int x0, int y0, int z0, int xs, int ys,
                                   int zs, int c0, int cg, void *stream);

int dgtta_feature_head_softmax(const float *facc, int64_t member_stride, const float *nsum, const float *w, const float *bsum, int M,
                               int Cin, int C, int64_t V, const int *h_sel, int K, int prob_dtype, int64_t *label_out, float *conf_out,
                               float *entropy_out, void *probs_out, void *stream);
int dgtta_softmax_merge_f64(const double *vals, int64_t V, int cg, int c0, double scale, double *run_max, double *run_sum,
                            double *run_dot, const int *h_sel, int K, double *stash, int first, void *stream);
int dgtta_softmax_finalize_f64(const double *run_max, const double *run_sum, const double *run_dot, const double *stash, int64_t V,
                               int K, int prob_dtype, float *conf_out, float *entropy_out, void *probs_out, void *stream);

#define DGTTA_EDT_MAX_AXIS 1024
int dgtta_label_bboxes(const int64_t *a, const int64_t *b, int D, int H, int W, int nlab, int *boxes, void *stream);
int dgtta_label_surface(const int64_t *map, int D, int H, int W, int64_t label, int d0, int h0, int w0, int cd, int ch, int cw,
                        uint8_t *surf, void *stream);
size_t dgtta_edt_ws_bytes(int D, int H, int W);
int dgtta_edt_sq(const uint8_t *site, float *dist2, void *ws, size_t ws_bytes, int D, int H, int W, float sd, float sh, float sw,
                 void *stream);

#define DGTTA_CC_MAX_TABLE 1024
size_t dgtta_cc_ws_bytes(int D, int H, int W);
int dgtta_cc_label(const int64_t *map, const int *group, int ntab, int D, int H, int W, int connectivity, int *cc, void *ws,
                   size_t ws_bytes, void *stream);
int dgtta_cc_sizes(const int *cc, int64_t n, int *size, void *stream);
int dgtta_cc_filter(const int64_t *map, const int *group, int ntab, const int *cc, const int *size, int64_t n, int keep_largest,
                    int min_voxels, int64_t background, int64_t *out, int64_t *removed, void *ws, size_t ws_bytes, void *stream);

size_t dgtta_holes_ws_bytes(int D, int H, int W);
int dgtta_holes_fill(const uint8_t *mask, int D, int H, int W, int connectivity, uint8_t *out, int64_t *n_filled, int *box, void *ws,
                     size_t ws_bytes, void *stream);
int dgtta_holes_member(const int64_t *map, int D, int H, int W, const int *group, int ntab, int d0, int h0, int w0, int cd, int ch,
                       int cw, uint8_t *mask, void *stream);
int dgtta_holes_apply(int64_t *map, int D, int H, int W, const uint8_t *mask, const uint8_t *filled, int d0, int h0, int w0, int cd,
                      int ch, int cw, int64_t background, int64_t label, int64_t *count, void *stream);
int dgtta_nonzero_mask(const float *data, int C, int64_t n, uint8_t *mask, void *stream);

#define DGTTA_PATCH_MAX_ITEMS 16
typedef struct DgttaPatchItem {
  const float *image;
  const float *label;
  int D, H, W;
  float map[12];
} DgttaPatchItem;
int dgtta_bspline3_prefilter(const float *src, float *dst, int D, int H, int W, void *stream);
int dgtta_patch_sample_aug(const DgttaPatchItem *items, int n_items, int PD, int PH, int PW, int order, float *image,
                           int64_t *labels, void *stream);

#define DGTTA_INTENSITY_MAX_ITEMS 16
#define DGTTA_IMAP_LINEAR 0
#define DGTTA_IMAP_CONTRAST 1
#define DGTTA_IMAP_GAMMA 2
#define DGTTA_IMAP_RESTORE 3
typedef struct DgttaIntensityItem {
  int item;
  int mode;
  int negate;
  int noise_b;
  float a;
  float s;
  uint32_t seed_lo, seed_hi, off_lo, off_hi;
} DgttaIntensityItem;
typedef struct DgttaBlurItem {
  int item;
  int radius;
  float taps[9];
} DgttaBlurItem;
size_t dgtta_intensity_stats_ws_bytes(int n_items, int64_t V);
int dgtta_intensity_stats(const float *x, int B, int64_t V, const int *h_items, int n_items, double *stats, void *ws,
                          size_t ws_bytes, void *stream);
int dgtta_intensity_map(const float *src, float *dst, int B, int64_t V, const DgttaIntensityItem *h_items, int n_items,
                        const double *stats, const double *stats2, void *stream);
int dgtta_gauss_blur3(const float *src, float *dst, float *scratch, int B, int D, int H, int W, const DgttaBlurItem *h_items,
                      int n_items, void *stream);

#ifdef __cplusplus
}
#endif
#endif
```

Before: 6.471.

## Defer skip-connection dgrad and fuse its accumulation with InstanceNorm backward stats

For large decoder concat blocks, the skip half of the concat gradient is no longer computed immediately. The encoder block's own dgrad writes the skip gradient first, and then the deferred decoder dgrad accumulates into it inside the MFMA ring or rows kernel. That kernel also produces the InstanceNorm backward statistics, which replaces a separate accumulate pass and a later stats pass over a large activation. The cost is an extra buffer load per output tile in the new ADD kernel variants, more template instantiations, and a heuristic gate based on size and shape support.

After: 6.558, median of 6. +1.3%, better.

```diff
diff --git a/dg_tta_amd/_lib.py b/dg_tta_amd/_lib.py
--- a/dg_tta_amd/_lib.py
+++ b/dg_tta_amd/_lib.py
@@ -58,6 +58,8 @@
     "dgtta_instnorm_lrelu_fwd": (I, [P, I, P, P, P, P, P, I, P, SZ, I, I, I64, F, F, I, P]),
     "dgtta_instnorm_lrelu_bwd": (I, [P, I, P, I, P, P, P, P, I, P, P, P, SZ, I, I, I64, F, I, I, P]),
     "dgtta_conv3d_k3_dgrad_gstats": (I, [P, I, P, P, I, I, I, I, I, I, I, I, I, P, I, P, P, P, F, P, SZ, C.POINTER(I), I, I, P]),
+    "dgtta_conv3d_k3_dgrad_gstats_acc": (I, [P, I, P, P, I, I, I, I, I, I, I, I, I, P, I, P, P, P, F, P, SZ, C.POINTER(I), I, I, P]),
+    "dgtta_conv3d_k3_dgrad_gstats_acc_supported": (I, [I, I, I, I, I, I, I]),
     "dgtta_instnorm_lrelu_bwd_gstats": (I, [P, I, P, I, P, P, P, P, I, P, P, P, P, SZ, I, I, I64, F, I, I, P]),
     "dgtta_convT3d_fwd_ws_bytes": (SZ, [I, I, I]),
     "dgtta_convT3d_k2s2_fwd": (I, [P, I, P, P, P, I, P, SZ, I, I, I, I, I, I, I, I, P]),
diff --git a/dg_tta_amd/csrc/common.h b/dg_tta_amd/csrc/common.h
--- a/dg_tta_amd/csrc/common.h
+++ b/dg_tta_amd/csrc/common.h
@@ -40,6 +40,7 @@
   float slope;
   double *out;
   int produced;
+  int add;
 };
 
 #define DG_REQUIRE(cond, code, ...)      \
diff --git a/dg_tta_amd/csrc/conv_dispatch.hip b/dg_tta_amd/csrc/conv_dispatch.hip
--- a/dg_tta_amd/csrc/conv_dispatch.hip
+++ b/dg_tta_amd/csrc/conv_dispatch.hip
@@ -100,11 +100,12 @@
   DG_REQUIRE(stride == 1 || stride == 2, DGTTA_ERR_UNSUPPORTED, "conv3d_k3_dgrad: stride %d", stride);
   DG_REQUIRE(lddx >= Cin && lddy >= Cout, DGTTA_ERR_BADARG, "conv3d_k3_dgrad: ld < C");
   hipStream_t st = (hipStream_t)stream;
-  if (impl != 1 && stride == 1 && !accumulate) {
+  const bool fused_add = accumulate && gst && gst->add;
+  if (impl != 1 && stride == 1 && (!accumulate || fused_add)) {
     int rc = conv3_fwd_mfma(dy, lddy, imgB_of(wpack, CinP, CoutP, dtype), 1, nullptr, dx, lddx, B, Cout, Cin, CoutP, CinP, Di,
                             Hi, Wi, 1, dtype, st, nullptr, gst, 0, false);
     if (rc != DGTTA_ERR_UNSUPPORTED) return rc;
-    DG_REQUIRE(impl == 0, DGTTA_ERR_UNSUPPORTED, "conv3d_k3_dgrad: shape not covered by the MFMA kernel");
+    DG_REQUIRE(impl == 0 || fused_add, DGTTA_ERR_UNSUPPORTED, "conv3d_k3_dgrad: shape not covered by the MFMA kernel");
   }
   if (impl != 1 && stride == 2 && !((Di | Hi | Wi) & 1)) {
     int rc = conv3_dgrad_s2_mfma(dy, lddy, imgB_of(wpack, CinP, CoutP, dtype), dx, lddx, B, Cin, Cout, CinP, CoutP, Di, Hi, Wi,
@@ -137,6 +138,34 @@
                           fuse ? &ctx : nullptr);
   *h_produced = rc == DGTTA_OK ? ctx.produced : 0;
   return rc;
+}
+
+extern "C" int dgtta_conv3d_k3_dgrad_gstats_acc(const void *dy, int lddy, const void *wpack, void *dx, int lddx, int B, int Cin,
+                                                int Cout, int CinP, int CoutP, int Di, int Hi, int Wi, const void *y_prev,
+                                                int ldy_prev, const float *mean_rstd_prev, const float *gamma_prev,
+                                                const float *beta_prev, float slope, void *gstats, size_t gstats_bytes,
+                                                int *h_produced, int dtype, int impl, void *stream) {
+  DG_REQUIRE(y_prev && mean_rstd_prev && gamma_prev && beta_prev && gstats && h_produced, DGTTA_ERR_BADARG,
+             "conv3d_k3_dgrad_gstats_acc: null pointer");
+  DG_REQUIRE(ldy_prev >= Cin, DGTTA_ERR_BADARG, "conv3d_k3_dgrad_gstats_acc: ldy_prev < Cin");
+  DG_REQUIRE(B > 0 && Cin > 0 && Di > 0 && Hi > 0 && Wi > 0 && gstats_bytes >= dgtta_conv3d_stats_bytes(B, Cin, Di, Hi, Wi),
+             DGTTA_ERR_WORKSPACE, "conv3d_k3_dgrad_gstats_acc: statistics buffer too small");
+  RowsGstCtx ctx{y_prev, ldy_prev, mean_rstd_prev, gamma_prev, beta_prev, slope, (double *)gstats, 0, 1};
+  const bool fuse = dtype != DGTTA_F32 && impl != 1 && dgtta_switches().in_gstats != '0';
+  const int rc = k3_dgrad(dy, lddy, wpack, dx, lddx, B, Cin, Cout, CinP, CoutP, Di, Hi, Wi, 1, 1, dtype, impl, stream,
+                          fuse ? &ctx : nullptr);
+  *h_produced = rc == DGTTA_OK ? ctx.produced : 0;
+  return rc;
+}
+
+extern "C" int dgtta_conv3d_k3_dgrad_gstats_acc_supported(int B, int Cin, int Cout, int D, int H, int W, int dtype) {
+  if (B <= 0 || Cin <= 0 || Cout <= 0 || D <= 0 || H <= 0 || W <= 0) return 0;
+  if ((dtype != DGTTA_BF16 && dtype != DGTTA_F16) || dgtta_switches().in_gstats == '0') return 0;
+  const int CinP = (Cin + 15) / 16 * 16, CoutP = (Cout + 15) / 16 * 16;
+  RowsGstCtx ctx{(const void *)16, CinP, nullptr, nullptr, nullptr, 0.f, nullptr, 0, 1};
+  const int rc = conv3_fwd_mfma((const void *)16, CoutP, (const void *)16, 1, nullptr, (void *)16, CinP, B, Cout, Cin, CoutP, CinP, D, H,
+                                W, 1, dtype, nullptr, nullptr, &ctx, 0, true);
+  return rc == DGTTA_OK;
 }
 
 static size_t wgrad_bias_bytes(int B, int Cout, int Do, int Ho, int Wo) {
diff --git a/dg_tta_amd/csrc/conv_mfma.hip b/dg_tta_amd/csrc/conv_mfma.hip
--- a/dg_tta_amd/csrc/conv_mfma.hip
+++ b/dg_tta_amd/csrc/conv_mfma.hip
@@ -337,7 +337,9 @@
 template <typename T>
 int dispatch_conv_classes(const ConvLaunch &L, const ConvClasses &cs, int stride) {
   const View &yv = L.yv;
-  const bool ring_only = L.xkh || L.dry;
+  const bool fused_only = L.gst && L.gst->add;
+  const bool ring_only = L.xkh || (L.dry && !fused_only);
+  if (fused_only && stride != 1) return DGTTA_ERR_UNSUPPORTED;
   const long long vox = (long long)yv.D * yv.H * yv.W * L.B;
   if (ring_only && stride != 1) return DGTTA_ERR_UNSUPPORTED;
   if (stride == 0) {
@@ -363,7 +365,7 @@
     if (ring_only) return DGTTA_ERR_UNSUPPORTED;
     if (all_taps && vec_out && (njobs >= 256 || rows == '1') && rows != '0') return conv3_rows_launch(L, cs.taps[0], is_f16);
   }
-  if (ring_only) return DGTTA_ERR_UNSUPPORTED;
+  if (ring_only || fused_only) return DGTTA_ERR_UNSUPPORTED;
   if (stride == 1) {
     if (yv.W >= 32) return launch_conv<T, 32, 4, 4, 1, 1, 1, 8>(L, cs);
     const bool k2 = L.CinP % (4 * Elem<T>::EPV) == 0;
diff --git a/dg_tta_amd/csrc/conv_ring.hip b/dg_tta_amd/csrc/conv_ring.hip
--- a/dg_tta_amd/csrc/conv_ring.hip
+++ b/dg_tta_amd/csrc/conv_ring.hip
@@ -58,7 +58,7 @@
   unsigned bytes;
 };
 
-template <typename T16, bool GST = false, int KH = 1>
+template <typename T16, bool GST = false, int KH = 1, bool ADD = false>
 __global__ __launch_bounds__(RingCfgT<KH>::NT) void conv3_ring_kernel(const bf16_t *__restrict__ x, View xv, const bf16_t *__restrict__ w,
                                                                  Taps taps, const float *__restrict__ bias, bf16_t *__restrict__ y,
                                                                  View yv, int Cout, int tilesW, int tilesH, int nblkN, int nseg,
@@ -66,6 +66,7 @@
                                                                  int ntaps_src, unsigned x_bytes, unsigned y_bytes, RingGst gst,
                                                                  long long xkh) {
   typedef RingCfgT<KH> C;
+  static_assert(GST || !ADD, "the accumulate form exists with the InstanceNorm backward sums only");
   extern __shared__ __attribute__((aligned(16))) unsigned char smem[];
   float *red = reinterpret_cast<float *>(smem + C::NSLOT * C::PLANE);
   float *gcst = red + C::NW * 16 * 2;
@@ -126,6 +127,8 @@
     for (int r = 0; r < 4; ++r) bv[r] = (!GST && bias) ? bias[n0 + chalf * 16 + 4 * q + r] : 0.f;
     const __amdgpu_buffer_rsrc_t rg =
         __builtin_amdgcn_make_buffer_rsrc((void *)(gst.y + (long long)b * gst.v.sb), (short)0, (int)gst.bytes, 0x00020000);
+    const __amdgpu_buffer_rsrc_t rya =
+        __builtin_amdgcn_make_buffer_rsrc((void *)(y + (long long)b * yv.sb), (short)0, (int)y_bytes, 0x00020000);
     if (GST) {
       if (tid < 32) {
         const int c = n0 + tid;
@@ -182,6 +185,7 @@
 #pragma unroll
     for (int t = 0; t < 4; ++t) gs1[t] = gs2[t] = f32x2_t{0.f, 0.f};
     u32x4_t gy[2];
+    u32x4_t gx[2];
     int issued = 0;
 
     auto load_gy = [&](int k, int od) {
@@ -192,6 +196,11 @@
           const unsigned soff = (unsigned)(((long long)odg * gst.v.sd + (long long)ohg * gst.v.sh + (long long)ow0 * gst.v.sw + n0) * 2);
           gy[oh] = __builtin_amdgcn_raw_buffer_load_b128(rg, goff, soff, 0);
           ++issued;
+          if (ADD) {
+            const unsigned soffy = (unsigned)(((long long)odg * yv.sd + (long long)ohg * yv.sh + (long long)ow0 * yv.sw + n0) * 2);
+            gx[oh] = __builtin_amdgcn_raw_buffer_load_b128(rya, ooff, soffy, 0);
+            ++issued;
+          }
         }
       }
     };
@@ -199,7 +208,21 @@
     auto epilogue_row = [&](int k, int od, int oh) {
       const int odg = d0 + 2 * k + od, ohg = oh0 + 2 * ws + oh;
       if (odg < D && ohg < H) {
-        const f32x4_t a0 = acc[od][oh][0], a1 = acc[od][oh][1];
+        f32x4_t a0 = acc[od][oh][0], a1 = acc[od][oh][1];
+        if (ADD) {
+          const u32x4_t xo = gx[oh];
+          const auto o0 = __builtin_amdgcn_permlane16_swap(xo[0], xo[2], false, false);
+          const auto o1 = __builtin_amdgcn_permlane16_swap(xo[1], xo[3], false, false);
+          float lo, hi;
+          unpack2_16<T16>(o0[0], lo, hi);
+          a0[0] += lo, a0[1] += hi;
+          unpack2_16<T16>(o1[0], lo, hi);
+          a0[2] += lo, a0[3] += hi;
+          unpack2_16<T16>(o0[1], lo, hi);
+          a1[0] += lo, a1[1] += hi;
+          unpack2_16<T16>(o1[1], lo, hi);
+          a1[2] += lo, a1[3] += hi;
+        }
         if (!GST) {
           auto sums = [&](const f32x2_t l0, const f32x2_t h0, const f32x2_t l1, const f32x2_t h1) {
             s1[0] += l0 + l1;
@@ -450,11 +473,13 @@
     stats = gctx->out;
     if (!dry) gctx->produced = 1;
   }
+  const bool add = gctx && gctx->add;
+  if (add && !gst_on) return DGTTA_ERR_UNSUPPORTED;
   if (dry) return DGTTA_OK;
   const int grid = (int)(njobs < ncu ? njobs : ncu);
-#define RING_LAUNCH(T16, GSTV)                                                                                                \
+#define RING_LAUNCH(T16, GSTV, ADDV)                                                                                                \
   do {                                                                                                                        \
-    auto kern = conv3_ring_kernel<T16, GSTV, KH>;                                                                             \
+    auto kern = conv3_ring_kernel<T16, GSTV, KH, ADDV>;                                                                       \
     static DynLdsOnce once;                                                                                                   \
     DG_REQUIRE(ensure_dyn_lds(once, reinterpret_cast<const void *>(kern), C::LDS_BYTES) == hipSuccess, DGTTA_ERR_LAUNCH,      \
                "conv3_ring: cannot raise the dynamic LDS limit to %d", C::LDS_BYTES);                                         \
@@ -462,13 +487,16 @@
                        (bf16_t *)y, yv, Cout, tW, tH, nblkN, nseg, sps, (int)njobs, stats, ntaps_src, (unsigned)xb,           \
                        (unsigned)yb, ga, xkh);                                                                                \
   } while (0)
-  if (gst_on) {
-    if (is_f16) RING_LAUNCH(f16_t, true);
-    else RING_LAUNCH(bf16_t, true);
+  if (add) {
+    if (is_f16) RING_LAUNCH(f16_t, true, true);
+    else RING_LAUNCH(bf16_t, true, true);
+  } else if (gst_on) {
+    if (is_f16) RING_LAUNCH(f16_t, true, false);
+    else RING_LAUNCH(bf16_t, true, false);
   } else if (is_f16) {
-    RING_LAUNCH(f16_t, false);
+    RING_LAUNCH(f16_t, false, false);
   } else {
-    RING_LAUNCH(bf16_t, false);
+    RING_LAUNCH(bf16_t, false, false);
   }
 #undef RING_LAUNCH
   DG_CHECK_LAUNCH("conv3_ring_kernel");
diff --git a/dg_tta_amd/csrc/conv_rows.hip b/dg_tta_amd/csrc/conv_rows.hip
--- a/dg_tta_amd/csrc/conv_rows.hip
+++ b/dg_tta_amd/csrc/conv_rows.hip
@@ -22,7 +22,7 @@
   float slope;
 };
 
-template <int PD, int PH, int WD, int WH, typename T16 = bf16_t, bool GST = false>
+template <int PD, int PH, int WD, int WH, typename T16 = bf16_t, bool GST = false, bool ADD = false>
 __global__ __launch_bounds__(WD *WH * 64) void conv3_rows_kernel(const bf16_t *__restrict__ x, View xv,
                                                                  const bf16_t *__restrict__ w, Taps taps,
                                                                  const float *__restrict__ bias, bf16_t *__restrict__ y,
@@ -278,15 +278,19 @@
         const int cq = le >> 4, li = le & 15, rq = li >> 2, rp = li & 3;
         f32x2_t s1v = {0.f, 0.f}, s2v = {0.f, 0.f};
         uint4 gy[GST ? PD * PH * 2 : 1];
+        uint4 gx[ADD ? PD * PH * 2 : 1];
         f32x2_t gs1[4], gs2[4], gA[4], gB[4];
         if (GST) {
 #pragma unroll
           for (int k = 0; k < PD * PH; ++k) {
             const int od = cur.od0 + wd * PD + k / PH, oh = cur.oh0 + wh * PH + k % PH;
             const bf16_t *yrow = gst.y + (long long)cur.b * gst.v.sb + od * gst.v.sd + oh * gst.v.sh + cur.n0 + cq * 8;
-#pragma unroll
-            for (int vb = 0; vb < 2; ++vb)
+            const bf16_t *xrow = y + (long long)cur.b * yv.sb + od * yv.sd + oh * yv.sh + cur.n0 + cq * 8;
+#pragma unroll
+            for (int vb = 0; vb < 2; ++vb) {
               gy[k * 2 + vb] = *reinterpret_cast<const uint4 *>(yrow + (long long)(cur.ow0 + 16 * vb + li) * gst.v.sw);
+              if (ADD) gx[k * 2 + vb] = *reinterpret_cast<const uint4 *>(xrow + (cur.ow0 + 16 * vb + li) * yv.sw);
+            }
           }
 #pragma unroll
           for (int t = 0; t < 4; ++t) {
@@ -327,6 +331,19 @@
             val.y = (unsigned)(unsigned short)lo[2] | ((unsigned)(unsigned short)lo[3] << 16);
             val.z = (unsigned)(unsigned short)hi[0] | ((unsigned)(unsigned short)hi[1] << 16);
             val.w = (unsigned)(unsigned short)hi[2] | ((unsigned)(unsigned short)hi[3] << 16);
+            if (ADD) {
+              const uint4 xo = gx[(i * PH + j) * 2 + vb];
+              const unsigned cw[4] = {val.x, val.y, val.z, val.w}, ow4[4] = {xo.x, xo.y, xo.z, xo.w};
+              unsigned sw4[4];
+#pragma unroll
+              for (int t = 0; t < 4; ++t) {
+                float c0f, c1f, o0f, o1f;
+                unpack2_16<T16>(cw[t], c0f, c1f);
+                unpack2_16<T16>(ow4[t], o0f, o1f);
+                sw4[t] = pack2_16<T16>(c0f + o0f, c1f + o1f);
+              }
+              val = make_uint4(sw4[0], sw4[1], sw4[2], sw4[3]);
+            }
             if (GST) {
               const uint4 yq = gy[(i * PH + j) * 2 + vb];
               const unsigned gw[4] = {val.x, val.y, val.z, val.w}, yw[4] = {yq.x, yq.y, yq.z, yq.w};
@@ -474,12 +491,16 @@
     ga.beta = gctx->beta;
     ga.slope = gctx->slope;
     stats = gctx->out;
-    gctx->produced = 1;
+    if (!L.dry) gctx->produced = 1;
   }
+  const bool add = gctx && gctx->add;
+  if (add && !gst_on) return DGTTA_ERR_UNSUPPORTED;
+  if (L.dry) return DGTTA_OK;
   auto kern = conv3_rows_kernel<PD, PH, WD, WH, T16>;
-  static DynLdsOnce once_plain, once_gst;
+  static DynLdsOnce once_plain, once_gst, once_add;
   if (gst_on) kern = conv3_rows_kernel<PD, PH, WD, WH, T16, true>;
-  DG_REQUIRE(ensure_dyn_lds(gst_on ? once_gst : once_plain, reinterpret_cast<const void *>(kern), (int)Cfg::LDS_BYTES) == hipSuccess,
+  if (add) kern = conv3_rows_kernel<PD, PH, WD, WH, T16, true, true>;
+  DG_REQUIRE(ensure_dyn_lds(add ? once_add : gst_on ? once_gst : once_plain, reinterpret_cast<const void *>(kern), (int)Cfg::LDS_BYTES) == hipSuccess,
              DGTTA_ERR_LAUNCH, "conv3_rows: cannot raise the dynamic LDS limit to %zu", (size_t)Cfg::LDS_BYTES);
   const int tW = cdiv(yv.W, 32), tH = cdiv(yv.H, Cfg::TH), tD = cdiv(yv.D, Cfg::TD), nblkN = cdiv(CoutP, 32);
   const long long njobs = (long long)tW * tH * tD * nblkN * B;
diff --git a/dg_tta_amd/csrc/lib.hip b/dg_tta_amd/csrc/lib.hip
--- a/dg_tta_amd/csrc/lib.hip
+++ b/dg_tta_amd/csrc/lib.hip
@@ -10,7 +10,7 @@
   va_end(ap);
 }
 
-extern "C" int dgtta_version(void) { return 60200;  }
+extern "C" int dgtta_version(void) { return 60300;  }
 extern "C" const char *dgtta_last_error(void) { return g_err; }
 
 #include <mutex>
diff --git a/dg_tta_amd/unet_exec.py b/dg_tta_amd/unet_exec.py
--- a/dg_tta_amd/unet_exec.py
+++ b/dg_tta_amd/unet_exec.py
@@ -215,6 +215,18 @@
                                                  self.coutp, *self.din, ptr(prev.y), cin, ptr(prev.mr), ptr(pn.weight),
                                                  ptr(pn.bias), SLOPE, ptr(gstats), gbytes, C.byref(produced), p.dt, p.impl, p.st),
               "dgtta_conv3d_k3_dgrad_gstats")
+        return gstats if produced.value else None
+
+    def dgrad_gstats_acc(self, p, dy, dst, prev, cin_slice):
+        cin = cin_slice[1] - cin_slice[0]
+        w, pn = self.weights(p, cin_slice), prev.mod.norm
+        gbytes = p.lib.dgtta_conv3d_stats_bytes(p.B, cin, *self.din)
+        gstats = p.ws.get(gbytes, "gstats")
+        produced = C.c_int(0)
+        check(p.lib.dgtta_conv3d_k3_dgrad_gstats_acc(ptr(dy), self.cout, ptr(w), dst.ptr, dst.ld, p.B, cin, self.cout, _pad(cin, p.cp),
+                                                     self.coutp, *self.din, ptr(prev.y), cin, ptr(prev.mr), ptr(pn.weight),
+                                                     ptr(pn.bias), SLOPE, ptr(gstats), gbytes, C.byref(produced), p.dt, p.impl, p.st),
+              "dgtta_conv3d_k3_dgrad_gstats_acc")
         return gstats if produced.value else None
 
     def wgrad_ws_bytes(self, p):
@@ -534,16 +546,42 @@
         blk.wgrad(p, dy, dw, db, ws, nb, stream)
 
 
-def _concat_grad(p, blk, dy, cat):
+class _DeferredSkip:
+    __slots__ = ("blk", "dy", "rows", "c")
+
+    def __init__(self, blk, dy, rows, c):
+        self.blk, self.dy, self.rows, self.c = blk, dy, rows, c
+
+    def finish(self, p, prev):
+        return self.blk.dgrad_gstats_acc(p, self.dy, self.rows, prev, (self.c, 2 * self.c))
+
+
+SKIP_DEFER_MIN_BYTES = 256 << 20
+
+
+def _defers_skip(p, blk, cat, skip):
+    return (blk.halfwise and all(s == 1 for s in blk.stride) and p.dt != F32 and p.impl != 1 and skip.cout == cat.c
+            and tuple(skip.dout) == tuple(cat.dims) == tuple(blk.din)
+            and p.B * skip.vout * cat.c * p.esz > SKIP_DEFER_MIN_BYTES
+            and p.lib.dgtta_conv3d_k3_dgrad_gstats_acc_supported(p.B, cat.c, blk.cout, *blk.din, p.dt) == 1)
+
+
+def _concat_grad(p, blk, dy, cat, skip):
     B, c = p.B, cat.c
+    defer = _defers_skip(p, blk, cat, skip)
     if c * p.esz == 64 and blk.halfwise and (cat.xbs or os.environ.get("DGTTA_SPLIT_CAT_GRAD", "1") != "0"):
         halves = [p.empty(B, *cat.dims, c), p.empty(B, *cat.dims, c)]
-        for i, dst in enumerate(halves):
+        for i, dst in enumerate(halves[:1] if defer else halves):
             blk.dgrad(p, dy, ptr(dst), c, cin_slice=(i * c, (i + 1) * c))
-        return tuple(_Rows(t, t.data_ptr(), c) for t in halves)
-    gc = torch.empty_like(cat.buf)
-    blk.dgrad(p, dy, ptr(gc), 2 * c)
-    return _Rows(gc, gc.data_ptr(), 2 * c), _Rows(gc, gc.data_ptr() + c * p.esz, 2 * c)
+        gup, gskip = (_Rows(t, t.data_ptr(), c) for t in halves)
+    else:
+        gc = torch.empty_like(cat.buf)
+        if defer:
+            blk.dgrad(p, dy, ptr(gc), 2 * c, cin_slice=(0, c))
+        else:
+            blk.dgrad(p, dy, ptr(gc), 2 * c)
+        gup, gskip = _Rows(gc, gc.data_ptr(), 2 * c), _Rows(gc, gc.data_ptr() + c * p.esz, 2 * c)
+    return gup, (_DeferredSkip(blk, dy, gskip, c) if defer else gskip)
 
 
 def _up_backward(p, up, g):
@@ -633,14 +671,21 @@
             kind, sidx, bidx = blk.where
             gstats = None
             if kind == "dec" and bidx == 0:
-                gup, gskip[sidx] = _concat_grad(p, blk, dy, cats[-(sidx + 1)])
+                skip = next(b for b in reversed(blocks) if b.where[:2] == ("enc", len(ups) - 1 - sidx))
+                gup, gskip[sidx] = _concat_grad(p, blk, dy, cats[-(sidx + 1)], skip)
                 gz = _up_backward(p, ups[sidx], gup)
                 if sidx > 0 and gaux and gaux[len(ups) - 1 - sidx] is not None:
                     za, adims = ctx.aux[sidx - 1]
                     _aux_head_backward(p, net.decoder.seg_layers[sidx - 1], za, ctx.sel, nsel, gaux[len(ups) - 1 - sidx], gz, adims)
             elif kind == "enc" and bidx == 0:
-                gz = gskip[len(ups) - sidx]
-                blk.dgrad(p, dy, gz.ptr, gz.ld, accumulate=1)
+                gz = gskip.pop(len(ups) - sidx)
+                if isinstance(gz, _DeferredSkip):
+                    late, gz = gz, gz.rows
+                    blk.dgrad(p, dy, gz.ptr, gz.ld, accumulate=0)
+                    gstats = late.finish(p, blocks[idx - 1])
+                    del late
+                else:
+                    blk.dgrad(p, dy, gz.ptr, gz.ld, accumulate=1)
             else:
                 gz, gstats = _plain_grad(p, blk, dy, blocks[idx - 1])
         if p.side is not None:
diff --git a/include/dgtta.h b/include/dgtta.h
--- a/include/dgtta.h
+++ b/include/dgtta.h
@@ -140,6 +140,11 @@
                                  int CinP, int CoutP, int Di, int Hi, int Wi, const void *y_prev, int ldy_prev,
                                  const float *mean_rstd_prev, const float *gamma_prev, const float *beta_prev, float slope,
                                  void *gstats, size_t gstats_bytes, int *h_produced, int dtype, int impl, void *stream);
+int dgtta_conv3d_k3_dgrad_gstats_acc(const void *dy, int lddy, const void *wpack, void *dx, int lddx, int B, int Cin, int Cout,
+                                     int CinP, int CoutP, int Di, int Hi, int Wi, const void *y_prev, int ldy_prev,
+                                     const float *mean_rstd_prev, const float *gamma_prev, const float *beta_prev, float slope,
+                                     void *gstats, size_t gstats_bytes, int *h_produced, int dtype, int impl, void *stream);
+int dgtta_conv3d_k3_dgrad_gstats_acc_supported(int B, int Cin, int Cout, int D, int H, int W, int dtype);
 int dgtta_instnorm_lrelu_bwd_gstats(const void *gz, int ldgz, const void *y, int ldy, const float *gamma, const float *beta,
                                     const float *mean_rstd, void *dy, int lddy, float *dgamma, float *dbeta,
                                     const void *gstats, void *ws, size_t ws_bytes, int B, int C, int64_t V, float slope,
```
